# sec-bit/ckb-zkp

Hardware: AMD Instinct MI355X
Metric: Groth16 proofs/sec (2^20 constraints, BN256) (higher is better)
Workload: dtype u32 limbs (256-bit Montgomery integers); 1 GPU; Groth16 prove, MiMC-chain R1CS, 1048570 constraints (domain 2^20), 1258284 aux, bn254, G1 x4 + G2 x1 MSM + 4 NTT (7 in the reference: evaluation-form key); curve=bn254, log_domain=20, parallelism=independent proofs x1

## Files before the change

### ckb_zkp_amd/_lib.py

```python
from __future__ import annotations

import ctypes as C
import os
from pathlib import Path

LIB_PATH = Path(os.environ.get("ZKP_ACCEL_LIB") or Path(__file__).resolve().parent / "lib" / "libzkp_accel.so")

u64p = C.POINTER(C.c_uint64)
u32p = C.POINTER(C.c_uint32)
u8p = C.POINTER(C.c_uint8)
vp = C.c_void_p


class ZkpError(RuntimeError):
    def __init__(self, status: int, where: str, text: str):
        super().__init__(f"{where}: status {status} ({text})")
        self.status = status


class Csr(C.Structure):
    _fields_ = [("row_ptr", vp), ("col", vp), ("coeff", vp)]


class Groth16PkDesc(C.Structure):
# ... 106 lines not shown
    "zkp_bases_upload_g2": (C.c_int32, [vp, C.c_int, vp, vp, C.c_size_t, C.POINTER(C.c_uint64)]),
    "zkp_bases_share": (C.c_int32, [vp, vp, C.c_uint64, u64p]),
    "zkp_bases_free": (C.c_int32, [vp, C.c_uint64]),
    "zkp_bases_len": (C.c_int32, [vp, C.c_uint64, C.POINTER(C.c_size_t)]),
    "zkp_msm_g1": (C.c_int32, [vp, C.c_uint64, C.c_size_t, vp, C.c_size_t, vp]),
    "zkp_msm_g2": (C.c_int32, [vp, C.c_uint64, C.c_size_t, vp, C.c_size_t, vp]),
    "zkp_msm_g1_dev": (C.c_int32, [vp, C.c_uint64, C.c_size_t, vp, C.c_size_t, vp]),
    "zkp_msm_g2_dev": (C.c_int32, [vp, C.c_uint64, C.c_size_t, vp, C.c_size_t, vp]),
    "zkp_vartime_multiscalar_mul_g1": (C.c_int32, [vp, C.c_uint64, vp, C.c_size_t, vp]),
    "zkp_vartime_multiscalar_mul_g2": (C.c_int32, [vp, C.c_uint64, vp, C.c_size_t, vp]),
    "zkp_msm_g1_var": (C.c_int32, [vp, C.c_int, vp, vp, vp, C.c_size_t, C.c_int32, vp]),
    "zkp_msm_g2_var": (C.c_int32, [vp, C.c_int, vp, vp, vp, C.c_size_t, C.c_int32, vp]),
    "zkp_msm_g1_var_batch_dev": (C.c_int32, [vp, C.c_int, C.c_size_t, vp, vp, vp, vp, C.c_int32, vp]),
    "zkp_msm_g2_var_batch_dev": (C.c_int32, [vp, C.c_int, C.c_size_t, vp, vp, vp, vp, C.c_int32, vp]),
    "zkp_g1_ipa_fold_dev": (C.c_int32, [vp, C.c_int, vp, vp, vp, vp, C.c_size_t, vp, vp, vp, vp]),
    "zkp_fr_dot_batch_dev": (C.c_int32, [vp, C.c_int, C.c_size_t, vp, vp, vp, vp]),
    "zkp_msm_g1_mont_dev": (C.c_int32, [vp, C.c_uint64, C.c_size_t, vp, C.c_size_t, vp]),
    "zkp_msm_g2_mont_dev": (C.c_int32, [vp, C.c_uint64, C.c_size_t, vp, C.c_size_t, vp]),
    "zkp_msm_g1_mont_batch_dev": (C.c_int32, [vp, C.c_uint64, C.c_size_t, vp, vp, vp, vp]),
    "zkp_msm_mont_multi_dev": (C.c_int32, [vp, C.c_size_t, vp, vp, vp, vp, vp, C.c_size_t]),
    "zkp_fr_vec_op_dev": (C.c_int32, [vp, C.c_int, C.c_int32, vp, vp, vp, vp, C.c_size_t]),
    "zkp_fr_spmv_dev": (C.c_int32, [vp, C.c_int, vp, vp, vp, C.c_size_t, vp, vp]),
    "zkp_fr_gather_dev": (C.c_int32, [vp, vp, vp, C.c_size_t, vp]),
    "zkp_poly_divide_by_vanishing_dev": (C.c_int32, [vp, C.c_int, vp, C.c_size_t, C.c_size_t, vp, vp]),
    "zkp_d2d": (C.c_int32, [vp, vp, vp, C.c_size_t]),
    "zkp_dev_zero": (C.c_int32, [vp, vp, C.c_size_t]),
    "zkp_fr_batch_inverse_dev": (C.c_int32, [vp, C.c_int, vp, C.c_size_t]),
    "zkp_poly_evaluate_dev": (C.c_int32, [vp, C.c_int, vp, C.c_size_t, vp, vp]),
    "zkp_poly_div_linear_dev": (C.c_int32, [vp, C.c_int, vp, C.c_size_t, vp, vp, vp]),
    "zkp_g1_fold": (C.c_int32, [vp, C.c_int, vp, C.c_size_t, vp]),
    "zkp_g2_fold": (C.c_int32, [vp, C.c_int, vp, C.c_size_t, vp]),
    "zkp_g1_into_affine": (C.c_int32, [vp, C.c_int, vp, vp, vp]),
    "zkp_g1_decompress": (C.c_int32, [vp, C.c_int, vp, C.c_size_t, vp, vp, C.POINTER(C.c_size_t)]),
    "zkp_g2_decompress": (C.c_int32, [vp, C.c_int, vp, C.c_size_t, vp, vp, C.POINTER(C.c_size_t)]),
    "zkp_g1_compress": (C.c_int32, [vp, C.c_int, vp, vp, C.c_size_t, vp]),
    "zkp_g2_compress": (C.c_int32, [vp, C.c_int, vp, vp, C.c_size_t, vp]),
    "zkp_g1_subgroup_check": (C.c_int32, [vp, C.c_int, vp, vp, C.c_size_t, C.POINTER(C.c_size_t)]),
    "zkp_g2_subgroup_check": (C.c_int32, [vp, C.c_int, vp, vp, C.c_size_t, C.POINTER(C.c_size_t)]),
    "zkp_g2_into_affine": (C.c_int32, [vp, C.c_int, vp, vp, vp]),
    "zkp_groth16_points_into_affine": (C.c_int32, [C.c_int, vp, vp, vp, vp, vp]),
    "zkp_fixed_base_mul_g1": (C.c_int32, [vp, C.c_int, vp, vp, C.c_size_t, vp, vp]),
    "zkp_fixed_base_mul_g2": (C.c_int32, [vp, C.c_int, vp, vp, C.c_size_t, vp, vp]),
    "zkp_groth16_pk_upload": (C.c_int32, [vp, C.POINTER(Groth16PkDesc), C.POINTER(vp)]),
    "zkp_groth16_pk_upload_ex": (C.c_int32, [vp, C.POINTER(Groth16PkDesc), C.c_uint32, C.POINTER(vp)]),
    "zkp_groth16_pk_upload_shard": (C.c_int32, [vp, C.POINTER(Groth16PkDesc), C.c_int32, C.c_int32, C.POINTER(vp)]),
    "zkp_groth16_partials_bytes": (C.c_int32, [C.c_int, C.POINTER(C.c_size_t)]),
    "zkp_groth16_prove_partials_dev": (C.c_int32, [vp, vp, vp, vp, vp, vp]),
    "zkp_groth16_fold_assemble_dev": (C.c_int32, [vp, C.c_int, vp, C.c_int32, vp, vp, vp, vp]),
    "zkp_groth16_pk_free": (C.c_int32, [vp, vp]),
    "zkp_groth16_witness_map": (C.c_int32, [vp, vp, vp, vp]),
    "zkp_groth16_witness_map_dev": (C.c_int32, [vp, vp, vp, vp]),
    "zkp_groth16_domain_size": (C.c_int32, [vp, C.POINTER(C.c_uint64)]),
    "zkp_groth16_pk_info": (C.c_int32, [vp, vp, C.POINTER(C.c_uint64)]),
    "zkp_groth16_prove": (C.c_int32, [vp, vp, vp, vp, vp, vp, vp]),
    "zkp_groth16_prove_dev": (C.c_int32, [vp, vp, vp, vp, vp, vp, vp]),
    "zkp_groth16_prove_batch_dev": (C.c_int32, [vp, vp, C.c_size_t, vp, vp, vp, vp, vp]),
    "zkp_groth16_prove_batch": (C.c_int32, [vp, vp, C.c_size_t, vp, vp, vp, vp, vp]),
    "zkp_groth16_assemble": (C.c_int32, [vp, C.c_int, vp, vp, vp, vp, vp]),
    "zkp_groth16_last_timing": (C.c_int32, [vp, C.POINTER(Groth16Timing)]),
    "zkp_marlin_last_timing": (C.c_int32, [vp, C.POINTER(MarlinTiming)]),
    "zkp_set_profiling": (C.c_int32, [vp, C.c_int32]),
    "zkp_marlin_index_upload": (C.c_int32, [vp, C.POINTER(MarlinIndexDesc), C.POINTER(vp)]),
    "zkp_marlin_index_free": (C.c_int32, [vp, vp]),
    "zkp_marlin_index_info": (C.c_int32, [vp, u64p]),
    "zkp_marlin_index_commit": (C.c_int32, [vp, vp, C.c_uint64, vp, vp]),
    "zkp_marlin_prove": (C.c_int32, [vp, vp, C.c_uint64, C.c_uint64, vp, C.c_size_t, vp, vp, C.c_size_t,
                                     C.POINTER(MarlinRand), vp, C.POINTER(MarlinProof)]),
    "zkp_fs_rng_new": (C.c_int32, [vp, C.c_size_t, C.POINTER(vp)]),
    "zkp_fs_rng_free": (C.c_int32, [vp]),
    "zkp_fs_rng_absorb": (C.c_int32, [vp, vp, C.c_size_t]),
    "zkp_fs_rng_seed": (C.c_int32, [vp, vp]),
    "zkp_fs_rng_next_u64": (C.c_int32, [vp, u64p]),
    "zkp_fs_rng_rand_u128": (C.c_int32, [vp, vp]),
    "zkp_fs_rng_rand_fr": (C.c_int32, [vp, C.c_int, vp]),
    "zkp_fs_rng_sample_outside_domain": (C.c_int32, [vp, C.c_int, C.c_uint32, vp]),
    "zkp_merlin_oneshot": (C.c_int32, [vp, C.c_size_t, vp, C.c_size_t, vp, C.c_size_t, vp, C.c_size_t, vp, C.c_size_t]),
    "zkp_bench_mulmod": (C.c_int32, [vp, C.c_int, C.c_int32, C.c_int32, C.POINTER(C.c_double)]),
    "zkp_bench_hbm_copy": (C.c_int32, [vp, C.c_size_t, C.POINTER(C.c_double)]),
}

_lib = None


def load(path: os.PathLike | None = None) -> C.CDLL:
    global _lib
    if _lib is not None and path is None:
        return _lib
    p = Path(path) if path else LIB_PATH
    if not p.exists():
        raise ImportError(f"{p} not found — build it with `python -m ckb_zkp_amd.build` "
                          "(hipcc --offload-arch=gfx950); there is no CPU fallback")
    lib = C.CDLL(str(p))
    for name, (res, args) in SIGNATURES.items():
        fn = getattr(lib, name)
        fn.restype, fn.argtypes = res, args
    if path is None:
        _lib = lib
    return lib


ZKP_ERR_INVALID_POINT = -7


def check(status: int, where: str) -> None:
    if status != 0:
        raise ZkpError(status, where, load().zkp_status_string(status).decode())
# ... 1 lines not shown
```

### ckb_zkp_amd/csrc/capi.hip

```cpp
#include <cstdint>
#include <cstdlib>
#include <cstring>

#include "ctx.hpp"
#include "host_field.hpp"
#include "internal.hpp"
#include "ipa.hpp"

using namespace zkp;

namespace {

template <class Fn>
int32_t guarded(zkp_ctx* ctx, Fn&& fn) {
  if (!ctx) return ZKP_ERR_BAD_ARG;
  std::lock_guard<std::recursive_mutex> lk(ctx->mu);
  try {
    ZKP_HIP(hipSetDevice(ctx->device));
    fn();
    return ZKP_OK;
  } catch (const StatusError& e) {
    return e.status;
  } catch (const HipError& e) {
    ctx->last_error = std::string(e.what) + ": " + hipGetErrorString(e.e);
// ... 568 lines not shown
  if (!desc || !out || (flags & ~(uint32_t)ZKP_PK_KEEP_FORM)) return ZKP_ERR_BAD_ARG;
  return guarded(ctx, [&] { *out = groth16_pk_upload(ctx, desc, 0, 0, (int)flags); });
}
int32_t zkp_groth16_pk_upload_shard(zkp_ctx* ctx, const zkp_groth16_pk_desc* desc, int32_t rank, int32_t world,
                                    zkp_groth16_pk** out) {
  if (!desc || !out || world < 1 || rank < 0 || rank >= world) return ZKP_ERR_BAD_ARG;
  return guarded(ctx, [&] { *out = groth16_pk_upload(ctx, desc, rank, world); });
}
int32_t zkp_groth16_partials_bytes(zkp_curve_t curve, size_t* bytes) {
  if (!bytes || (curve != ZKP_BN254 && curve != ZKP_BLS12_381)) return ZKP_ERR_BAD_ARG;
  *bytes = groth16_partials_bytes(curve);
  return ZKP_OK;
}
int32_t zkp_groth16_prove_partials_dev(zkp_ctx* ctx, zkp_groth16_pk* pk, const uint64_t* z_dev, const uint64_t* r,
                                       const uint64_t* s, void* partials_dev) {
  if (!pk || !z_dev || !r || !s || !partials_dev) return ZKP_ERR_BAD_ARG;
  return guarded(ctx, [&] { groth16_prove_partials(ctx, pk, z_dev, r, s, partials_dev); });
}
int32_t zkp_groth16_fold_assemble_dev(zkp_ctx* ctx, zkp_curve_t curve, const void* gathered_dev, int32_t world,
                                      const uint64_t* r, const uint64_t* s, uint64_t* proof, uint8_t* inf) {
  if (!gathered_dev || world < 1 || !r || !s || !proof || !inf) return ZKP_ERR_BAD_ARG;
  return guarded(ctx, [&] { groth16_fold_assemble(ctx, curve, gathered_dev, world, r, s, proof, inf); });
}
int32_t zkp_groth16_pk_upload_multi(zkp_ctx* ctx, const zkp_groth16_pk_desc* desc, int32_t mode, zkp_groth16_pk_multi** out) {
  if (!ctx || !desc || !out || ctx->devs.empty() || (mode != ZKP_MULTI_SHARD && mode != ZKP_MULTI_REPLICATE)) return ZKP_ERR_BAD_ARG;
  return guarded_multi(ctx, [&] { *out = groth16_pk_upload_multi(ctx, desc, mode); });
}
int32_t zkp_groth16_pk_multi_free(zkp_ctx* ctx, zkp_groth16_pk_multi* pk) {
  if (!ctx || !pk || ctx->devs.empty()) return ZKP_ERR_BAD_ARG;
  return guarded_multi(ctx, [&] { groth16_pk_multi_free(ctx, pk); });
}
int32_t zkp_groth16_multi_info(zkp_ctx* ctx, zkp_groth16_pk_multi* pk, uint64_t info[6]) {
  if (!ctx || !pk || !info || ctx->devs.empty()) return ZKP_ERR_BAD_ARG;
  return guarded(ctx, [&] { groth16_multi_info(ctx, pk, info); });
}
int32_t zkp_groth16_prove_multi(zkp_ctx* ctx, zkp_groth16_pk_multi* pk, const uint64_t* const* z, int32_t z_on_device,
                                const uint64_t* r, const uint64_t* s, uint64_t* proof, uint8_t* inf) {
  if (!ctx || !pk || !z || !z[0] || !r || !s || !proof || !inf || ctx->devs.empty()) return ZKP_ERR_BAD_ARG;
  if (z_on_device)
    for (size_t k = 0; k < ctx->devs.size(); k++)
      if (!z[k]) return ZKP_ERR_BAD_ARG;
  return guarded_multi(ctx, [&] { groth16_prove_multi(ctx, pk, z, z_on_device != 0, r, s, proof, inf); });
}
int32_t zkp_groth16_prove_batch_multi(zkp_ctx* ctx, zkp_groth16_pk_multi* pk, size_t count, const uint64_t* const* z,
                                      int32_t z_on_device, const uint64_t* r, const uint64_t* s, uint64_t* proofs,
                                      uint8_t* inf) {
  if (!ctx || !pk || ctx->devs.empty() || (count && (!z || !r || !s || !proofs || !inf))) return ZKP_ERR_BAD_ARG;
  return guarded_multi(ctx, [&] { groth16_prove_batch_multi(ctx, pk, count, z, z_on_device != 0, r, s, proofs, inf); });
}
int32_t zkp_groth16_pk_free(zkp_ctx* ctx, zkp_groth16_pk* pk) {
  if (!pk) return ZKP_ERR_BAD_ARG;
  return guarded(ctx, [&] { groth16_pk_free(ctx, pk); });
}
int32_t zkp_groth16_pk_info(zkp_ctx* ctx, zkp_groth16_pk* pk, uint64_t info[8]) {
  if (!ctx || !pk || !info) return ZKP_ERR_BAD_ARG;
  return guarded(ctx, [&] { groth16_pk_info(ctx, pk, info); });
}
int32_t zkp_groth16_domain_size(zkp_groth16_pk* pk, uint64_t* n) {
  if (!pk || !n) return ZKP_ERR_BAD_ARG;
  *n = groth16_domain_size(pk);
  return ZKP_OK;
}
int32_t zkp_groth16_witness_map(zkp_ctx* ctx, zkp_groth16_pk* pk, const uint64_t* z, uint64_t* h) {
  if (!pk || !z || !h) return ZKP_ERR_BAD_ARG;
  return guarded(ctx, [&] { groth16_witness_map(ctx, pk, z, h, false); });
}
int32_t zkp_groth16_witness_map_dev(zkp_ctx* ctx, zkp_groth16_pk* pk, const uint64_t* z, uint64_t* h) {
  if (!pk || !z || !h) return ZKP_ERR_BAD_ARG;
  return guarded(ctx, [&] { groth16_witness_map(ctx, pk, z, h, true); });
}
int32_t zkp_groth16_prove(zkp_ctx* ctx, zkp_groth16_pk* pk, const uint64_t* z, const uint64_t* r, const uint64_t* s,
                          uint64_t* proof, uint8_t* inf) {
  if (!pk || !z || !r || !s || !proof || !inf) return ZKP_ERR_BAD_ARG;
  return guarded(ctx, [&] { groth16_prove(ctx, pk, z, false, r, s, proof, inf); });
}
int32_t zkp_groth16_prove_dev(zkp_ctx* ctx, zkp_groth16_pk* pk, const uint64_t* z, const uint64_t* r,
                              const uint64_t* s, uint64_t* proof, uint8_t* inf) {
  if (!pk || !z || !r || !s || !proof || !inf) return ZKP_ERR_BAD_ARG;
  return guarded(ctx, [&] { groth16_prove(ctx, pk, z, true, r, s, proof, inf); });
}
int32_t zkp_groth16_prove_batch_dev(zkp_ctx* ctx, zkp_groth16_pk* pk, size_t n, const uint64_t* const* z_dev,
                                    const uint64_t* r, const uint64_t* s, uint64_t* proofs, uint8_t* inf) {
  if (!pk || (n && (!z_dev || !r || !s || !proofs || !inf))) return ZKP_ERR_BAD_ARG;
  return guarded(ctx, [&] { groth16_prove_batch(ctx, pk, n, z_dev, r, s, proofs, inf); });
}
int32_t zkp_groth16_prove_batch(zkp_ctx* ctx, zkp_groth16_pk* pk, size_t n, const uint64_t* const* z_host,
                                const uint64_t* r, const uint64_t* s, uint64_t* proofs, uint8_t* inf) {
  if (!pk || (n && (!z_host || !r || !s || !proofs || !inf))) return ZKP_ERR_BAD_ARG;
  return guarded(ctx, [&] { groth16_prove_batch(ctx, pk, n, z_host, r, s, proofs, inf, false); });
}
int32_t zkp_groth16_assemble(zkp_ctx* ctx, zkp_curve_t curve, const uint64_t* sums, const uint64_t* r,
                             const uint64_t* s, uint64_t* proof, uint8_t* inf) {
  if (!sums || !r || !s || !proof || !inf) return ZKP_ERR_BAD_ARG;
  return guarded(ctx, [&] { groth16_assemble(ctx, curve, sums, r, s, proof, inf); });
}
int32_t zkp_marlin_index_upload(zkp_ctx* ctx, const zkp_marlin_index_desc* desc, zkp_marlin_index** out) {
  if (!desc || !out) return ZKP_ERR_BAD_ARG;
  return guarded(ctx, [&] { *out = marlin_index_upload(ctx, desc); });
}
int32_t zkp_marlin_index_free(zkp_ctx* ctx, zkp_marlin_index* index) {
  if (!index) return ZKP_ERR_BAD_ARG;
  return guarded(ctx, [&] { marlin_index_free(ctx, index); });
}
int32_t zkp_marlin_index_info(const zkp_marlin_index* index, uint64_t info[6]) {
  if (!index || !info) return ZKP_ERR_BAD_ARG;
  marlin_index_info(index, info);
// ... 37 lines not shown
```

### ckb_zkp_amd/csrc/ctx.hpp

```cpp
#pragma once
#include <hip/hip_runtime.h>
#include <stdint.h>

#include <map>
#include <mutex>
#include <memory>
#include <string>
#include <unordered_map>
#include <vector>

#include "../../include/zkp_accel.h"

namespace zkp {

struct HipError {
  hipError_t e;
  const char* what;
  int line;
};

#define ZKP_HIP(call)                                                   \
  do {                                                                  \
    hipError_t _e = (call);                                             \
    if (_e != hipSuccess) throw ::zkp::HipError{_e, #call, __LINE__};   \
  } while (0)

struct StatusError {
  int32_t status;
};
#define ZKP_REQUIRE(cond, status) \
  do {                            \
    if (!(cond)) throw ::zkp::StatusError{(status)}; \
  } while (0)

struct DevBuf {
  void* p = nullptr;
  size_t cap = 0;
  void* get(size_t bytes) {
    if (bytes > cap) {
      if (p) (void)hipFree(p);
      p = nullptr;
      cap = 0;
      size_t want = bytes + (bytes >> 3) + 256;
      hipError_t e = hipMalloc(&p, want);
      if (e != hipSuccess) throw StatusError{ZKP_ERR_OOM};
      cap = want;
    }
    return p;
  }
  template <class T>
  T* as(size_t count) { return reinterpret_cast<T*>(get(count * sizeof(T))); }
  ~DevBuf() {
    if (p) (void)hipFree(p);
  }
  DevBuf() = default;
  DevBuf(const DevBuf&) = delete;
  DevBuf& operator=(const DevBuf&) = delete;
};

struct NttTables {
  int log_n = 0, h = 0;
  uint32_t* w_lo = nullptr;
  uint32_t* w_hi = nullptr;
  uint32_t* wi_lo = nullptr;
  uint32_t* wi_hi = nullptr;
  uint32_t* g_lo = nullptr;
  uint32_t* g_hi = nullptr;
  uint32_t* gi_lo = nullptr;
  uint32_t* gi_hi = nullptr;
  uint32_t* sub_fwd = nullptr;
  uint32_t* sub_inv = nullptr;
  uint32_t* n_inv = nullptr;
  void* block = nullptr;
  uint32_t* full_fwd[8] = {};
  uint32_t* full_inv[8] = {};
  uint32_t* full_g = nullptr;
  uint32_t* full_gi = nullptr;
  uint32_t* g_hi_n = nullptr;
  uint32_t* full_g_n = nullptr;
  std::vector<void*> extra;
};

struct BasesEntry;

struct MsmWorkspace {
  hipStream_t stream = nullptr;
  bool own_stream = false;
  hipEvent_t done = nullptr;
  hipEvent_t sorted = nullptr;
  hipEvent_t l1_done = nullptr;
  uint32_t chain_nb = 0;
  size_t chain_xb = 0;
  hipEvent_t acc_done = nullptr;
  DevBuf keys, vals, keys2, vals2, sort_tmp, offsets, buckets, tmp, out, sched, scan_tmp, scan_tmp2, partial, redo;
};
struct Groth16Timing {
  zkp_groth16_timing t{};
};

}

struct zkp_lane {
  hipStream_t stream = nullptr;
  bool own_stream = true;
  static constexpr int N_WS = 4;
  static constexpr int N_WS_MSM = N_WS;
  zkp::MsmWorkspace ws[N_WS];
  zkp::DevBuf ntt_scratch;
  hipEvent_t ev_fork = nullptr, ev_a = nullptr, ev_b1 = nullptr;
  uint32_t* host_proof = nullptr;
  bool host_tail = false;
  bool busy = false;
};

struct zkp_cfg {
  int lanes = 0;
  int msm_batch_lanes = 1;
  int msm_c = 0, msm_c_g2 = 0;
  long long msm_chunk = (long long)3 << 19;
  double table_budget_gb = 0;
  bool h_lagrange = true, c_fold = true, host_affine = true;
  long long lfold_heavy_cost = 0;
  int multi_exchange = 0;
  int multi_exchange_timeout_ms = 30000;
  int multi_wm_split = -1;
};

struct zkp_ctx {
  int device = 0;
  zkp_cfg cfg;
  std::recursive_mutex mu;
  static constexpr int N_LANES = 8;
  static constexpr int N_WS = zkp_lane::N_WS;
  zkp_lane lanes[N_LANES];
  zkp_lane* cur = &lanes[0];
  int cur_idx = 0;
  hipEvent_t ev0 = nullptr, ev1 = nullptr;
  hipEvent_t ev2 = nullptr, ev3 = nullptr;
  bool profiling = false;
  size_t table_bytes = 0;
  bool msm_defer_reduce = false;
  int msm_acc_into = -1;
  int msm_bucket_ws = -1;
  bool dbg_skip_k8 = false;
  bool batch_mode = false;
  std::map<std::pair<int, int>, zkp::NttTables> ntt_tables;
  zkp::DevBuf ntt_io, poly_tmp, poly_consts, spmv_list;
  zkp::DevBuf msm_scalars, msm_misc, var_bases;
  uint32_t* pinned = nullptr;
  size_t pinned_cap = 0;
  std::unordered_map<uint64_t, std::shared_ptr<zkp::BasesEntry>> bases;
  uint64_t next_handle = 1;
  zkp_groth16_timing last_timing{};
  zkp_marlin_timing last_marlin_timing{};
  std::string last_error;
  std::vector<zkp_ctx*> devs;
  std::map<std::pair<int, int>, std::shared_ptr<void>> var_plans;
  bool tl_on = false;
  std::string tl_tag;
  std::vector<std::pair<std::string, hipEvent_t>> tl;
  void mark(hipStream_t st, const char* what) {
// ... 8 lines not shown
```

### ckb_zkp_amd/csrc/groth16.hip

```cpp
#include <algorithm>
#include <cstdlib>
#include <cstring>
#include <memory>
#include <string>
#include <vector>

#include "field_dev.hpp"
#include "host_field.hpp"
#include "internal.hpp"
#include "msm_vtbl.hpp"

using namespace zkp;

struct DevCsr {
  uint32_t* row_ptr = nullptr;
  uint32_t* col = nullptr;
  uint32_t* coeff = nullptr;
  size_t nnz = 0;
};

struct zkp_groth16_pk {
  int curve = 0;
  uint32_t num_inputs = 0, num_aux = 0, num_constraints = 0;
  int log_n = 0;
  size_t N = 0, nz = 0;
  DevCsr m[3];
  uint64_t hA = 0, hB1 = 0, hB2 = 0, hH = 0, hL = 0;
  bool share_b_sort = false;
  bool chain_lh = false;
  bool share_al_sort = false;
  bool share_l1 = false;
  bool b_in_l1 = false;
  bool c_folded = false;
  bool h_lagrange = false;
  int shard_rank = 0, shard_world = 0;
  size_t q_lo[5] = {0, 0, 0, 0, 0}, q_n[5] = {0, 0, 0, 0, 0};
  struct PerLane {
    DevBuf abc;
    DevBuf S;
    DevBuf results;
    DevBuf proof;
    bool warmed = false;
    int graph_state = 0;
    hipGraphExec_t graph_exec = nullptr;
    hipGraph_t graph = nullptr;
    std::vector<const void*> sig;
  } lane[zkp_ctx::N_LANES];
  DevBuf consts;
};

namespace zkp {

template <class P>
__global__ __launch_bounds__(256) void csr_eval_kernel(const uint32_t* __restrict__ row_ptr,
                                                       const uint32_t* __restrict__ col,
                                                       const uint32_t* __restrict__ coeff,
                                                       const uint32_t* __restrict__ z, uint32_t nc, uint32_t N,
                                                       uint32_t num_inputs, int is_a, uint32_t* __restrict__ out) {
  using F = Fp<P>;
  uint32_t i = blockIdx.x * blockDim.x + threadIdx.x;
  if (i >= N) return;
  F acc = F::zero();
  if (i < nc) {
    const F one = F::one();
    for (uint32_t k = row_ptr[i]; k < row_ptr[i + 1]; k++) {
      F v = F::load(z + (size_t)col[k] * 8);
      F cf = F::load(coeff + (size_t)k * 8);
      if (cf == one) acc = acc + v;
      else acc = acc + v * cf;
    }
  } else if (is_a && i - nc < num_inputs) {
    acc = F::load(z + (size_t)(i - nc) * 8);
  }
  acc.store(out + (size_t)i * 8);
}

template <class P>
__global__ __launch_bounds__(256) void qap_pointwise_kernel(uint32_t* __restrict__ a, const uint32_t* __restrict__ b,
                                                            const uint32_t* __restrict__ c,
                                                            const uint32_t* __restrict__ zinv, uint32_t N) {
  using F = Fp<P>;
  uint32_t i = blockIdx.x * blockDim.x + threadIdx.x;
  if (i >= N) return;
  F x = F::load(a + (size_t)i * 8) * F::load(b + (size_t)i * 8) - F::load(c + (size_t)i * 8);
  (x * F::load(zinv)).store(a + (size_t)i * 8);
}

template <class P>
__global__ __launch_bounds__(256) void qap_pointwise_ab_kernel(uint32_t* __restrict__ a, const uint32_t* __restrict__ b,
                                                               const uint32_t* __restrict__ zinv, uint32_t N) {
  using F = Fp<P>;
  uint32_t i = blockIdx.x * blockDim.x + threadIdx.x;
  if (i >= N) return;
  (F::load(a + (size_t)i * 8) * F::load(b + (size_t)i * 8) * F::load(zinv)).store(a + (size_t)i * 8);
}

template <class P>
__global__ __launch_bounds__(256) void pow_canon_kernel(uint32_t* __restrict__ out, const uint32_t* __restrict__ base,
                                                        const uint32_t* __restrict__ mult, uint32_t count) {
  using F = Fp<P>;
  const uint32_t i = blockIdx.x * blockDim.x + threadIdx.x;
// ... 240 lines not shown
  char* o = (char*)b_o.get(nz * ab);
  uint8_t* oi = (uint8_t*)b_oi.get(nz);
  v1->lfold(st, dl, dli, nz, dcp, drows, dkind, dcoeff, dg, dgi, o, oi);
  ZKP_HIP(hipGetLastError());
  l_xy->resize(nz * 2 * fq);
  l_inf->resize(nz);
  ZKP_HIP(hipMemcpyAsync(l_xy->data(), o, nz * ab, hipMemcpyDeviceToHost, st));
  ZKP_HIP(hipMemcpyAsync(l_inf->data(), oi, nz, hipMemcpyDeviceToHost, st));
  ZKP_HIP(hipStreamSynchronize(st));
  if (!heavy_cols.empty()) {
    const HostField Q = fq_field(d->curve);
    const size_t fw = 2 * fq;
    std::vector<HostJac> res(heavy_cols.size());
    std::vector<uint64_t> xyz(3 * fq);
    std::vector<uint64_t> cxy, csc;
    std::vector<uint8_t> cinf;
    for (size_t i = 0; i < heavy_cols.size(); i++) {
      const uint32_t m = heavy_cols[i];
      const size_t cn = hv[i].size();
      cxy.resize(cn * fw);
      csc.resize(cn * 4);
      cinf.resize(cn);
      for (size_t j = 0; j < cn; j++) {
        const uint32_t k = hv[i][j].first, e = hv[i][j].second;
        memcpy(&cxy[j * fw], &g_xy[(size_t)k * fw], 8 * fw);
        cinf[j] = g_inf[k];
        memcpy(&csc[j * 4], d->ct.coeff + (size_t)e * 4, 32);
      }
      std::vector<std::pair<uint32_t, uint32_t>>().swap(hv[i]);
      msm_var_run(ctx, d->curve, 1, cxy.data(), cinf.data(), csc.data(), cn, true, xyz.data());
      HostJac D = host_jac_load(Q, xyz.data());
      D.y = Q.neg(D.y);
      HostJac Lm{};
      if ((*l_inf)[m]) {
        Lm.x = Q.one_();
        Lm.y = Q.one_();
      } else {
        memcpy(Lm.x.data(), l_xy->data() + (size_t)m * fw, 8 * fq);
        memcpy(Lm.y.data(), l_xy->data() + (size_t)m * fw + fq, 8 * fq);
        Lm.z = Q.one_();
      }
      res[i] = host_jac_add(Q, Lm, D);
    }
    std::vector<uint64_t> axy(heavy_cols.size() * fw);
    std::vector<uint8_t> ainf(heavy_cols.size());
    host_into_affine(Q, res, axy.data(), fw, ainf.data());
    for (size_t i = 0; i < heavy_cols.size(); i++) {
      memcpy(l_xy->data() + (size_t)heavy_cols[i] * fw, axy.data() + i * fw, 8 * fw);
      (*l_inf)[heavy_cols[i]] = ainf[i];
    }
  }
}

zkp_groth16_pk* groth16_pk_upload(zkp_ctx* ctx, const zkp_groth16_pk_desc* d, int rank, int world, int flags) {
  ZKP_REQUIRE(d->curve == ZKP_BN254 || d->curve == ZKP_BLS12_381, ZKP_ERR_UNSUPPORTED_CURVE);
  ZKP_REQUIRE(d->num_inputs >= 1, ZKP_ERR_BAD_ARG);
  ZKP_REQUIRE(world >= 0 && (world == 0 ? rank == 0 : (rank >= 0 && rank < world)), ZKP_ERR_BAD_ARG);
  std::unique_ptr<zkp_groth16_pk> pk(new zkp_groth16_pk());
  pk->shard_rank = rank;
  pk->shard_world = world;
  pk->curve = d->curve;
  pk->num_inputs = d->num_inputs;
  pk->num_aux = d->num_aux;
  pk->num_constraints = d->num_constraints;
  pk->nz = (size_t)d->num_inputs + d->num_aux;
  size_t dom = (size_t)d->num_constraints + d->num_inputs;
  int lg = 0;
  while (((size_t)1 << lg) < dom) lg++;
  ZKP_REQUIRE(lg <= (d->curve == ZKP_BN254 ? 28 : 32) && lg <= 30, ZKP_ERR_DOMAIN_TOO_LARGE);
  pk->log_n = lg;
  pk->N = (size_t)1 << lg;
  const bool matrices_only = d->a_query == nullptr;
  if (!matrices_only) {
    ZKP_REQUIRE(d->a_len == pk->nz && d->b_g1_len == pk->nz && d->b_g2_len == pk->nz, ZKP_ERR_BAD_ARG);
    ZKP_REQUIRE(d->l_len == d->num_aux, ZKP_ERR_BAD_ARG);
  }
  const size_t fq = d->curve == ZKP_BN254 ? 4 : 6;
  const uint64_t* tA[4] = {d->alpha_g1, d->delta_g1, nullptr, nullptr};
  const uint64_t* tB1[4] = {d->beta_g1, nullptr, d->delta_g1, nullptr};
  const uint64_t* tB2[4] = {d->beta_g2, nullptr, d->delta_g2, nullptr};
  const uint64_t* tL[4] = {nullptr, nullptr, nullptr, d->delta_g1};
  pk->m[0] = upload_csr(ctx, d->at, d->num_constraints);
  pk->m[1] = upload_csr(ctx, d->bt, d->num_constraints);
  pk->m[2] = upload_csr(ctx, d->ct, d->num_constraints);
  ZKP_REQUIRE(!(matrices_only && world > 0), ZKP_ERR_BAD_ARG);
  if (!matrices_only) {
    for (auto p : {d->alpha_g1, d->beta_g1, d->delta_g1, d->beta_g2, d->delta_g2}) ZKP_REQUIRE(p, ZKP_ERR_BAD_ARG);
    const size_t h_used = std::min<size_t>(d->h_len, pk->N);
    shard_bounds(pk->nz + 4, rank, world, &pk->q_lo[0], &pk->q_n[0]);
    pk->q_lo[1] = pk->q_lo[2] = pk->q_lo[0];
    pk->q_n[1] = pk->q_n[2] = pk->q_n[0];
    shard_bounds(h_used, rank, world, &pk->q_lo[3], &pk->q_n[3]);
    pk->q_lo[4] = pk->q_lo[0];
    pk->q_n[4] = pk->q_n[0];
    const bool lagrange_on = ctx->cfg.h_lagrange && !(flags & 1) && d->h_query && h_used > 0 && pk->log_n >= 1;
    int lgk = 0;
    {
      const int groups[5] = {1, 1, 2, 1, 1};
      size_t hq_lo = 0, hq_n = pk->q_n[3];
      if (lagrange_on) shard_bounds(pk->N, rank, world, &hq_lo, &hq_n);
      const size_t ns[5] = {pk->q_n[0], pk->q_n[1], pk->q_n[2], lagrange_on ? hq_n : (world > 0 ? pk->q_n[3] : (size_t)d->h_len), pk->q_n[4]};
      lgk = bases_plan_lgk(ctx, d->curve, groups, ns, 5);
      if (lgk > 0 && getenv("ZKP_DEBUG_MSM")) fprintf(stderr, "[groth16] window tables do not fit: window groups of %d\n", 1 << lgk);
    }
    std::vector<uint8_t> fA, fB1, fB2, fL;
    pk->hA = upload_ext(ctx, d->curve, 1, d->a_query, d->a_inf, d->a_len, 2 * fq, tA, pk->q_lo[0], pk->q_n[0], 0, &fA, 0, 0, lgk);
// ... 50 lines not shown
      }
      fold_c_into_l(ctx, d, pk->nz, gc.xy, gc.inf, &lxy, &linf);
      if (!lagrange_keep_cache) gc.clear();
      pk->hL = upload_ext(ctx, d->curve, 1, lxy.data(), linf.data(), pk->nz, 2 * fq, tL, pk->q_lo[4], pk->q_n[4], 0, &fL, 0, 0, lgk);
      pk->c_folded = true;
    } else
    pk->hL = upload_ext(ctx, d->curve, 1, d->l_query, d->l_inf, d->l_len, 2 * fq, tL, pk->q_lo[4], pk->q_n[4],
                        d->num_inputs, &fL, 0, 0, lgk);
    {
      static const bool on = !(getenv("ZKP_SHARE_AL_SORT") && atoi(getenv("ZKP_SHARE_AL_SORT")) == 0);
      bool same = fA.size() == fL.size() && pk->q_lo[0] == pk->q_lo[4];
      size_t differ = 0;
      std::vector<uint8_t> both(fA.size());
      for (size_t k = 0; same && k < fA.size(); k++) {
        both[k] = fA[k] & fL[k];
        differ += fA[k] != fL[k];
      }
      pk->share_al_sort = on && same && differ <= fA.size() / 16 && bases_same_shape(ctx, pk->hL, pk->hA) && pk->q_n[0] > 0;
      if (pk->share_al_sort && differ) bases_set_sort_flags(ctx, pk->hA, both.data(), both.size());
      static const bool on_l1 = !(getenv("ZKP_SHARE_L1") && atoi(getenv("ZKP_SHARE_L1")) == 0);
      const bool aligned = fA.size() == fL.size() && fA.size() == fB2.size() && pk->q_lo[0] == pk->q_lo[4] &&
                           pk->q_lo[0] == pk->q_lo[2] && pk->q_n[0] > 0;
      if (on_l1 && aligned && !pk->share_al_sort && bases_same_shape(ctx, pk->hL, pk->hA)) {
        const bool with_b = pk->share_b_sort && bases_same_shape(ctx, pk->hB1, pk->hA);
        std::vector<uint8_t> all(fA.size()), member(fA.size());
        for (size_t k = 0; k < fA.size(); k++) {
          all[k] = fA[k] & fL[k] & (with_b ? fB2[k] : (uint8_t)1);
          member[k] = all[k] ? 0 : (uint8_t)((fA[k] ? 1 : 0) | (with_b && fB2[k] ? 2 : 0) | (fL[k] ? 4 : 0));
        }
        bases_set_sort_flags(ctx, pk->hA, all.data(), all.size());
        bases_set_group(ctx, pk->hA, member.data(), member.size());
        bases_set_filter_bit(ctx, pk->hA, 0);
        if (with_b) bases_set_filter_bit(ctx, pk->hB2, 1);
        bases_set_filter_bit(ctx, pk->hL, 2);
        pk->share_l1 = true;
        pk->b_in_l1 = with_b;
      }
      {
        static const bool on_chain = !(getenv("ZKP_CHAIN_LH") && atoi(getenv("ZKP_CHAIN_LH")) == 0);
        uint64_t iL[5], iH[5];
        bases_info(ctx, pk->hL, iL);
        bases_info(ctx, pk->hH, iH);
        pk->chain_lh = on_chain && iL[0] == iH[0] && iL[2] == 1 && iH[2] == 1 && pk->q_n[3] > 0 && pk->q_n[4] > 0;
      }
      if (getenv("ZKP_DEBUG_MSM"))
        fprintf(stderr, "[groth16] A/L sort sharing: %d (flags differ at %zu of %zu bases), B1/B2: %d, shared level 1: %d\n",
                (int)pk->share_al_sort, differ, fA.size(), (int)pk->share_b_sort, (int)pk->share_l1);
    }
  }
  uint32_t* consts = pk->consts.as<uint32_t>(64);
  if (d->curve == ZKP_BN254) hipLaunchKernelGGL(qap_consts_kernel<Bn254Fr>, dim3(1), dim3(64), 0, ctx->cur->stream, consts, lg);
  else hipLaunchKernelGGL(qap_consts_kernel<Bls381Fr>, dim3(1), dim3(64), 0, ctx->cur->stream, consts, lg);
  ZKP_HIP(hipGetLastError());
  for (int l = 0; l < 2; l++) {
    auto& L = pk->lane[l];
    L.abc.get(3 * pk->N * 32);
    L.S.get((pk->nz + 4) * 32);
    L.results.get(6 * 16 * 24 * 4 + 64);
    L.proof.get(4096);
  }
  ZKP_HIP(hipStreamSynchronize(ctx->cur->stream));
  return pk.release();
}

void groth16_pk_free(zkp_ctx* ctx, zkp_groth16_pk* pk) {
  (void)hipDeviceSynchronize();
  for (auto& PL : pk->lane) {
    if (PL.graph_exec) (void)hipGraphExecDestroy(PL.graph_exec);
    if (PL.graph) (void)hipGraphDestroy(PL.graph);
  }
  for (uint64_t h : {pk->hA, pk->hB1, pk->hB2, pk->hH, pk->hL})
    if (h) bases_drop(ctx, h);
  for (auto& m : pk->m) {
    if (m.row_ptr) (void)hipFree(m.row_ptr);
    if (m.col) (void)hipFree(m.col);
    if (m.coeff) (void)hipFree(m.coeff);
  }
  delete pk;
}

uint64_t groth16_domain_size(zkp_groth16_pk* pk) { return pk->N; }
void groth16_pk_info(zkp_ctx* ctx, zkp_groth16_pk* pk, uint64_t info[8]) {
  for (int i = 0; i < 8; i++) info[i] = 0;
  if (!pk->hA) return;
  uint64_t a[5], b[5];
  bases_info(ctx, pk->hA, a);
  bases_info(ctx, pk->hB2, b);
  info[0] = a[2];
  for (uint64_t h : {pk->hA, pk->hB1, pk->hB2, pk->hH, pk->hL}) {
    uint64_t t[5];
    bases_info(ctx, h, t);
    info[1] += t[4];
  }
  info[2] = a[0];
  info[3] = a[1];
  info[4] = a[3];
  info[5] = b[0];
  info[6] = (pk->share_b_sort ? 1 : 0) | (pk->share_al_sort ? 2 : 0) | (pk->share_l1 ? 4 : 0);
  info[7] = (pk->h_lagrange ? 1 : 0) | (pk->c_folded ? 2 : 0) | (pk->chain_lh ? 4 : 0);
}

template <class P>
static uint32_t* witness_map_dev(zkp_ctx* ctx, zkp_groth16_pk* pk, const uint32_t* z_dev, bool coeffs = true) {
  const uint32_t N = (uint32_t)pk->N;
  uint32_t* a = pk->lane[ctx->cur_idx].abc.as<uint32_t>(3 * pk->N * 8);
  uint32_t* b = a + pk->N * 8;
  uint32_t* c = b + pk->N * 8;
  uint32_t* bufs[3] = {a, b, c};
  hipStream_t st = ctx->cur->stream;
  const int nchain = (!coeffs && pk->c_folded) ? 2 : 3;
  for (int k = 0; k < nchain; k++)
    hipLaunchKernelGGL(csr_eval_kernel<P>, dim3((N + 255) / 256), dim3(256), 0, st, pk->m[k].row_ptr, pk->m[k].col,
                       pk->m[k].coeff, z_dev, pk->num_constraints, N, pk->num_inputs, k == 0 ? 1 : 0, bufs[k]);
  static const bool batch = getenv("ZKP_NTT_BATCH") && atoi(getenv("ZKP_NTT_BATCH")) != 0;
  if (batch) {
    ntt_run_batch(ctx, pk->curve, bufs, nchain, pk->log_n, ZKP_NTT_IFFT);
    ntt_run_batch(ctx, pk->curve, bufs, nchain, pk->log_n, ZKP_NTT_COSET_FFT);
  } else {
    for (int k = 0; k < nchain; k++) {
// ... 175 lines not shown
  }
  tm.ms_msm_accumulate = acc_ms;
  tm.msm_points = ent;
  tm.ms_msm_scan = scan_ms;
  tm.msm_scan_bytes = scan_bytes;
  tm.msm_scan_launches = scan_runs;
  if (partial_out) {
    ZKP_HIP(hipMemcpyAsync(partial_out, res, 5 * slot, hipMemcpyDeviceToDevice, st));
    ZKP_HIP(hipGetLastError());
    if (prof) {
      ZKP_HIP(hipEventRecord(eT1, st));
      ZKP_HIP(hipStreamSynchronize(st));
      ZKP_HIP(hipEventElapsedTime(&tm.ms_total, eT0, eT1));
      ctx->last_timing = tm;
    }
    return;
  }

  tic();
  if (!fan) v1->assemble_g1_part1(st, res, slot, rs, host_tail ? nullptr : proof_dev, flags_dev);
  v1->assemble_g1_part2(st, res, slot, host_tail ? nullptr : proof_dev, flags_dev, 2 * v1->fN + 2 * v2->fN);
  if (!g2_done_in_fan && !host_tail) v2->assemble_g2(st, res, slot, proof_dev, flags_dev, 2 * v1->fN);
  ZKP_HIP(hipGetLastError());
  toc(&tm.ms_assemble);
  const size_t proof_words = 4 * (size_t)v1->fN + 2 * (size_t)v2->fN;
  if (host_tail) {
    uint32_t* hp = ctx->cur->host_proof;
    ZKP_HIP(hipMemcpyAsync(hp, res, 16 * (size_t)v1->fN, hipMemcpyDeviceToHost, st));
    ZKP_HIP(hipMemcpyAsync(hp + 4 * v1->fN, res + 2 * slot, 16 * (size_t)v2->fN, hipMemcpyDeviceToHost, st));
    ZKP_HIP(hipMemcpyAsync(hp + 4 * v1->fN + 4 * v2->fN, res + 5 * slot, 16 * (size_t)v1->fN, hipMemcpyDeviceToHost, st));
  } else {
    ZKP_HIP(hipMemcpyAsync(ctx->cur->host_proof, proof_dev, proof_words * 4, hipMemcpyDeviceToHost, st));
    ZKP_HIP(hipMemcpyAsync(ctx->cur->host_proof + 256, flags_dev, 12, hipMemcpyDeviceToHost, st));
  }
  ctx->tl_tag.clear();
  ctx->mark(st, "copied");
  ctx->cur->host_tail = host_tail;
  ctx->cur->busy = true;
  if (prof) {
    ZKP_HIP(hipEventRecord(eT1, st));
    ZKP_HIP(hipStreamSynchronize(st));
    ZKP_HIP(hipEventElapsedTime(&tm.ms_total, eT0, eT1));
    ctx->last_timing = tm;
  }
}

static std::vector<const void*> lane_signature(zkp_ctx* ctx, zkp_groth16_pk* pk) {
  std::vector<const void*> sig;
  zkp_lane* L = ctx->cur;
  zkp_groth16_pk::PerLane& PL = pk->lane[ctx->cur_idx];
  for (DevBuf* b : {&PL.abc, &PL.S, &PL.results, &PL.proof, &L->ntt_scratch}) sig.push_back(b->p);
  for (int w = 0; w < zkp_lane::N_WS; w++) {
    MsmWorkspace& ws = L->ws[w];
    for (DevBuf* b : {&ws.keys, &ws.vals, &ws.keys2, &ws.vals2, &ws.sort_tmp, &ws.offsets, &ws.buckets, &ws.tmp, &ws.out,
                      &ws.sched, &ws.scan_tmp, &ws.scan_tmp2, &ws.partial, &ws.redo})
      sig.push_back(b->p);
  }
  sig.push_back(pk);
  return sig;
}

template <class FrP>
static void prove_enqueue(zkp_ctx* ctx, zkp_groth16_pk* pk, const uint64_t* z, bool z_on_device, const uint64_t* r,
                          const uint64_t* s, bool latency_plan = false) {
  static const bool graph_on = getenv("ZKP_GRAPH") && atoi(getenv("ZKP_GRAPH")) != 0;
  static const bool single_stream = getenv("ZKP_SINGLE_STREAM") && atoi(getenv("ZKP_SINGLE_STREAM")) != 0;
  if (!graph_on || ctx->profiling || single_stream) {
    prove_enqueue_part<FrP>(ctx, pk, z, z_on_device, r, s, 3, nullptr, latency_plan);
    return;
  }
  zkp_groth16_pk::PerLane& PL = pk->lane[ctx->cur_idx];
  hipStream_t st = ctx->cur->stream;
  if (PL.graph_state == 2 && PL.sig == lane_signature(ctx, pk)) {
    prove_enqueue_part<FrP>(ctx, pk, z, z_on_device, r, s, 1);
    ZKP_HIP(hipGraphLaunch(PL.graph_exec, st));
    ctx->cur->busy = true;
    return;
  }
  if (PL.graph_state == 2) {
    (void)hipGraphExecDestroy(PL.graph_exec);
    (void)hipGraphDestroy(PL.graph);
    PL.graph_exec = nullptr;
    PL.graph = nullptr;
    PL.graph_state = 0;
  }
  if (PL.graph_state == 1 && PL.sig == lane_signature(ctx, pk)) {
    prove_enqueue_part<FrP>(ctx, pk, z, z_on_device, r, s, 1);
    ZKP_HIP(hipStreamBeginCapture(st, hipStreamCaptureModeRelaxed));
    try {
      prove_enqueue_part<FrP>(ctx, pk, z, z_on_device, r, s, 2);
    } catch (...) {
      hipGraph_t g = nullptr;
      (void)hipStreamEndCapture(st, &g);
      if (g) (void)hipGraphDestroy(g);
      throw;
    }
    ZKP_HIP(hipStreamEndCapture(st, &PL.graph));
    ZKP_HIP(hipGraphInstantiate(&PL.graph_exec, PL.graph, nullptr, nullptr, 0));
    PL.graph_state = 2;
    ZKP_HIP(hipGraphLaunch(PL.graph_exec, st));
    ctx->cur->busy = true;
    return;
  }
  prove_enqueue_part<FrP>(ctx, pk, z, z_on_device, r, s, 3);
  PL.sig = lane_signature(ctx, pk);
  PL.graph_state = 1;
}

static void prove_finish(zkp_ctx* ctx, zkp_groth16_pk* pk, uint64_t* proof_out, uint8_t* inf_out) {
  const MsmVtbl* v1 = msm_vtbl(pk->curve, 1);
  const MsmVtbl* v2 = msm_vtbl(pk->curve, 2);
  const size_t proof_words = 4 * (size_t)v1->fN + 2 * (size_t)v2->fN;
  ZKP_HIP(hipStreamSynchronize(ctx->cur->stream));
  if (!ctx->tl.empty()) {
    std::string line = "[zkp timeline ms]";
    for (auto& m : ctx->tl) {
      float ms = 0.f;
      (void)hipEventSynchronize(m.second);
      (void)hipEventElapsedTime(&ms, ctx->tl[0].second, m.second);
// ... 60 lines not shown
  else prove_enqueue_part<Bls381Fr>(ctx, pk, z_dev, true, r, s, 3, (char*)out_dev, true);
  ZKP_HIP(hipStreamSynchronize(ctx->cur->stream));
}

void groth16_fold_assemble(zkp_ctx* ctx, int curve, const void* gathered_dev, int world, const uint64_t* r,
                           const uint64_t* s, uint64_t* proof_out, uint8_t* inf_out) {
  ZKP_REQUIRE(world >= 1, ZKP_ERR_BAD_ARG);
  const MsmVtbl* v1 = msm_vtbl(curve, 1);
  const MsmVtbl* v2 = msm_vtbl(curve, 2);
  hipStream_t st = ctx->cur->stream;
  const size_t slot = v2->xyzz_bytes;
  uint32_t* buf = ctx->msm_misc.as<uint32_t>(16 + 6 * slot / 4 + 256 + 16);
  uint32_t* rs = buf;
  char* res = reinterpret_cast<char*>(rs + 16);
  uint32_t* proof_dev = reinterpret_cast<uint32_t*>(res + 6 * slot);
  uint32_t* flags_dev = proof_dev + 240;
  ZKP_HIP(hipMemcpyAsync(rs, r, 32, hipMemcpyHostToDevice, st));
  ZKP_HIP(hipMemcpyAsync(rs + 8, s, 32, hipMemcpyHostToDevice, st));
  v1->fold_slots(st, (const char*)gathered_dev, 5 * slot, world, slot, 0x1b, res);
  v2->fold_slots(st, (const char*)gathered_dev, 5 * slot, world, slot, 0x04, res);
  v1->assemble_g1_part1(st, res, slot, rs, proof_dev, flags_dev);
  v1->assemble_g1_part2(st, res, slot, proof_dev, flags_dev, 2 * v1->fN + 2 * v2->fN);
  v2->assemble_g2(st, res, slot, proof_dev, flags_dev, 2 * v1->fN);
  ZKP_HIP(hipGetLastError());
  const size_t proof_words = 4 * (size_t)v1->fN + 2 * (size_t)v2->fN;
  uint32_t flags_host[4] = {0, 0, 0, 0};
  ZKP_HIP(hipMemcpyAsync(proof_out, proof_dev, proof_words * 4, hipMemcpyDeviceToHost, st));
  ZKP_HIP(hipMemcpyAsync(flags_host, flags_dev, 12, hipMemcpyDeviceToHost, st));
  ZKP_HIP(hipStreamSynchronize(st));
  for (int i = 0; i < 3; i++) inf_out[i] = (uint8_t)flags_host[i];
}

void groth16_prove(zkp_ctx* ctx, zkp_groth16_pk* pk, const uint64_t* z, bool z_on_device, const uint64_t* r,
                   const uint64_t* s, uint64_t* proof_out, uint8_t* inf_out) {
  ZKP_REQUIRE(pk->shard_world == 0, ZKP_ERR_BAD_ARG);
  ctx->cur = &ctx->lanes[0];
  ctx->cur_idx = 0;
  static const bool timeline = getenv("ZKP_TIMELINE") && atoi(getenv("ZKP_TIMELINE")) != 0;
  ctx->tl_on = timeline && !ctx->profiling;
  if (pk->curve == ZKP_BN254) prove_enqueue<Bn254Fr>(ctx, pk, z, z_on_device, r, s, true);
  else prove_enqueue<Bls381Fr>(ctx, pk, z, z_on_device, r, s, true);
  ctx->tl_on = false;
  prove_finish(ctx, pk, proof_out, inf_out);
}

void groth16_prove_batch(zkp_ctx* ctx, zkp_groth16_pk* pk, size_t n, const uint64_t* const* z_dev, const uint64_t* r,
                         const uint64_t* s, uint64_t* proofs_out, uint8_t* inf_out, bool z_on_device) {
  const MsmVtbl* v1 = msm_vtbl(pk->curve, 1);
  const MsmVtbl* v2 = msm_vtbl(pk->curve, 2);
  const size_t pw64 = (4 * (size_t)v1->fN + 2 * (size_t)v2->fN) / 2;
  const bool prof = ctx->profiling;
  ZKP_REQUIRE(pk->shard_world == 0, ZKP_ERR_BAD_ARG);
  size_t pending[zkp_ctx::N_LANES] = {};
  const int lanes_default = pk->log_n <= 22 ? 8 : 4;
  const int nl = std::max(1, std::min(ctx->cfg.lanes > 0 ? ctx->cfg.lanes : lanes_default, (int)zkp_ctx::N_LANES));
  auto select = [&](int l) {
    ctx->cur = &ctx->lanes[l];
    ctx->cur_idx = l;
  };
  struct BatchMode {
    zkp_ctx* c;
    ~BatchMode() { c->batch_mode = false; }
  } batch_mode{ctx};
  ctx->batch_mode = n > 1 && !prof;
  try {
    if (ctx->batch_mode) {
      std::vector<uint64_t> scratch_proof(pw64 + 8);
      uint8_t scratch_inf[4];
      bool any = false;
      for (int l = 0; l < nl; l++) {
        if (pk->lane[l].warmed) continue;
        select(l);
        if (pk->curve == ZKP_BN254) prove_enqueue<Bn254Fr>(ctx, pk, z_dev[0], z_on_device, r, s);
        else prove_enqueue<Bls381Fr>(ctx, pk, z_dev[0], z_on_device, r, s);
        pk->lane[l].warmed = true;
        any = true;
      }
      if (any)
        for (int l = 0; l < nl; l++) {
          select(l);
          if (ctx->cur->busy) prove_finish(ctx, pk, scratch_proof.data(), scratch_inf);
        }
    }
    for (size_t i = 0; i < n; i++) {
      const int l = prof ? 0 : (int)(i % nl);
      select(l);
      if (ctx->cur->busy) prove_finish(ctx, pk, proofs_out + pending[l] * pw64, inf_out + pending[l] * 3);
      if (pk->curve == ZKP_BN254) prove_enqueue<Bn254Fr>(ctx, pk, z_dev[i], z_on_device, r + 4 * i, s + 4 * i);
      else prove_enqueue<Bls381Fr>(ctx, pk, z_dev[i], z_on_device, r + 4 * i, s + 4 * i);
      pending[l] = i;
    }
    for (int l = 0; l < zkp_ctx::N_LANES; l++) {
      select(l);
      if (ctx->cur->busy) prove_finish(ctx, pk, proofs_out + pending[l] * pw64, inf_out + pending[l] * 3);
    }
  } catch (...) {
    (void)hipDeviceSynchronize();
    for (auto& L : ctx->lanes) L.busy = false;
    select(0);
    throw;
  }
  select(0);
}

}
#include <dlfcn.h>

#include <chrono>
#include <condition_variable>
#include <mutex>
#include <string>

#include <thread>
struct zkp_groth16_pk_multi {
  int mode = 0, curve = 0;
  std::vector<zkp_groth16_pk*> pk;
  std::vector<hipEvent_t> ev_chain, ev_done, ev_h_read;
  hipEvent_t ev_h = nullptr;
  void* gathered = nullptr;
  std::vector<void*> gathered_all;
  std::vector<void*> partial;
  int exchange = 0;
  bool exchange_fallback = false;
  int rccl_ranks = 0;
  int split_choice = -1;
  int calls = 0;
  double ms_variant[2] = {0.0, 0.0};
};
namespace zkp {

namespace {
struct RcclApi {
  struct Fns {
    void* lib = nullptr;
    int (*CommInitAll)(void**, int, const int*) = nullptr;
    int (*CommDestroy)(void*) = nullptr;
// ... 463 lines not shown
```

### ckb_zkp_amd/csrc/internal.hpp

```cpp
#pragma once
#include "ctx.hpp"

namespace zkp {

void ntt_run(zkp_ctx* ctx, int curve, uint32_t* data_dev, int log_n, int op);
void ntt_run_batch(zkp_ctx* ctx, int curve, uint32_t* const* data_dev, int count, int log_n, int op);
bool ntt_ifft_coset_fft(zkp_ctx* ctx, int curve, uint32_t* data, int log_n);
uint32_t* ntt_qap_coset_ifft(zkp_ctx* ctx, int curve, uint32_t* a, uint32_t* b, uint32_t* c, const uint32_t* zinv, int log_n);
void ntt_free_tables(zkp_ctx* ctx);

void fr_vec_op(zkp_ctx* ctx, int curve, int op, const uint64_t* a, const uint64_t* b, const uint64_t* k_host,
               uint64_t* out, size_t n);
void fr_batch_inverse(zkp_ctx* ctx, int curve, uint64_t* v, size_t n);
void fr_dot_batch(zkp_ctx* ctx, int curve, size_t count, const uint64_t* const* a, const uint64_t* const* b, const size_t* ns,
                  uint64_t* out_host);
void fr_spmv(zkp_ctx* ctx, int curve, const uint32_t* row_ptr, const uint32_t* col, const uint64_t* coeff, size_t nrows,
             const uint64_t* x, uint64_t* out);
void fr_gather(zkp_ctx* ctx, const uint64_t* in, const int32_t* idx, size_t n, uint64_t* out);
void poly_vanishing_fold(zkp_ctx* ctx, int curve, const uint64_t* p, size_t len, size_t n, uint64_t* q, uint64_t* rem);
void poly_div_linear(zkp_ctx* ctx, int curve, const uint64_t* p, size_t n, const uint64_t* z_host, uint64_t* q,
                     uint64_t* eval_out_host);
void marlin_round2_prod(zkp_ctx* ctx, int curve, const uint64_t* ra, const uint64_t* za, const uint64_t* zb, const uint64_t* t,
                        const uint64_t* z, const uint64_t* k_host, uint64_t* out, size_t n);
void marlin_t3_evals(zkp_ctx* ctx, int curve, const uint64_t* const* on_k, const uint64_t* k_host, uint64_t* out, size_t n);
void marlin_h2_numerator(zkp_ctx* ctx, int curve, const uint64_t* const* on_b, const uint64_t* t, const uint64_t* k_host, uint64_t* out,
                         size_t n);
void poly_evaluate_batch(zkp_ctx* ctx, int curve, size_t count, const uint64_t* const* p, const size_t* n, const uint64_t* z_host,
                         uint64_t* out_host);

uint64_t bases_upload(zkp_ctx* ctx, int curve, int group, const uint64_t* xy_host, const uint8_t* inf_host, size_t n,
                      int c_hint = 0, int cap_hint = 0, int lgk_hint = -1);
size_t bases_table_bytes(zkp_ctx* ctx, int curve, int group, size_t n, int lgk);
int bases_plan_lgk(zkp_ctx* ctx, int curve, const int* groups, const size_t* ns, int count);
void bases_free(zkp_ctx* ctx, uint64_t handle);
uint64_t bases_share(zkp_ctx* dst, zkp_ctx* src, uint64_t handle);
size_t bases_len(zkp_ctx* ctx, uint64_t handle);
int bases_group(zkp_ctx* ctx, uint64_t handle);
void msm_run(zkp_ctx* ctx, uint64_t handle, size_t offset, const uint64_t* scalars_dev, size_t n, bool montgomery,
             uint64_t* out_xyz_host, void* out_dev_xyzz = nullptr, float* ms_accumulate = nullptr,
             uint64_t* n_entries = nullptr, int ws = 0, int sort_src = -1, float* ms_scan = nullptr, int l1_src = -1);
double bench_mulmod(zkp_ctx* ctx, int curve, int field, bool unsaturated);
double bench_hbm_copy(zkp_ctx* ctx, size_t bytes);
bool bases_same_shape(zkp_ctx* ctx, uint64_t h1, uint64_t h2);
void bases_set_sort_flags(zkp_ctx* ctx, uint64_t handle, const uint8_t* flags_host, size_t n);
void bases_set_group(zkp_ctx* ctx, uint64_t owner, const uint8_t* member_flags_host, size_t n);
void bases_set_filter_bit(zkp_ctx* ctx, uint64_t handle, int bit);
void msm_run_batch(zkp_ctx* ctx, uint64_t handle, size_t count, const size_t* offsets, const uint64_t* const* scalars_dev,
                   const size_t* ns, bool montgomery, uint64_t* out_xyz_host);
void msm_run_multi(zkp_ctx* ctx, size_t count, const uint64_t* handles, const size_t* offsets,
                   const uint64_t* const* scalars_dev, const size_t* ns, bool montgomery, uint64_t* out_xyz_host,
                   size_t slot_words);
void msm_var_run(zkp_ctx* ctx, int curve, int group, const uint64_t* xy_host, const uint8_t* inf_host,
                 const uint64_t* scalars_host, size_t n, bool montgomery, uint64_t* out_xyz_host);
void msm_var_batch_run(zkp_ctx* ctx, int curve, int group, size_t count, const uint64_t* const* xy_dev,
                       const uint8_t* const* inf_dev, const uint64_t* const* scalars_dev, const size_t* ns, bool montgomery,
                       uint64_t* out_xyz_host);
void msm_free_all(zkp_ctx* ctx);
void bases_drop(zkp_ctx* ctx, uint64_t handle);
void point_fold(zkp_ctx* ctx, int curve, int group, const uint64_t* xyz_host, size_t k, uint64_t* out_xyz_host);
void point_into_affine(zkp_ctx* ctx, int curve, int group, const uint64_t* xyz_host, uint64_t* xy_out, uint8_t* inf_out);
size_t points_decompress(zkp_ctx* ctx, int curve, int group, const uint8_t* bytes, size_t n, uint64_t* xy_out, uint8_t* inf_out);
void points_compress(zkp_ctx* ctx, int curve, int group, const uint64_t* xy, const uint8_t* inf, size_t n, uint8_t* bytes_out);
size_t points_subgroup_check(zkp_ctx* ctx, int curve, int group, const uint64_t* xy, const uint8_t* inf, size_t n);
void points_fold_into_affine(zkp_ctx* ctx, int curve, int group, const uint64_t* a_xyz_host, const uint64_t* b_xyz_host,
                             const uint8_t* has_b, size_t k, uint64_t* xy_out, uint8_t* inf_out);
void fixed_base_mul(zkp_ctx* ctx, int curve, int group, const uint64_t* base_xy, const uint64_t* scalars_host, size_t n,
                    uint64_t* out_xy, uint8_t* out_inf);

zkp_groth16_pk* groth16_pk_upload(zkp_ctx* ctx, const zkp_groth16_pk_desc* d, int rank = 0, int world = 0, int flags = 0);
size_t groth16_partials_bytes(int curve);
void groth16_prove_partials(zkp_ctx* ctx, zkp_groth16_pk* pk, const uint64_t* z_dev, const uint64_t* r, const uint64_t* s,
                            void* out_dev);
void groth16_fold_assemble(zkp_ctx* ctx, int curve, const void* gathered_dev, int world, const uint64_t* r,
                           const uint64_t* s, uint64_t* proof_out, uint8_t* inf_out);
void groth16_pk_free(zkp_ctx* ctx, zkp_groth16_pk* pk);
uint64_t groth16_domain_size(zkp_groth16_pk* pk);
void groth16_pk_info(zkp_ctx* ctx, zkp_groth16_pk* pk, uint64_t info[8]);
void bases_info(zkp_ctx* ctx, uint64_t handle, uint64_t info[5]);
void groth16_witness_map(zkp_ctx* ctx, zkp_groth16_pk* pk, const uint64_t* z, uint64_t* h, bool on_device);
void groth16_prove(zkp_ctx* ctx, zkp_groth16_pk* pk, const uint64_t* z, bool z_on_device, const uint64_t* r,
                   const uint64_t* s, uint64_t* proof_out, uint8_t* inf_out);

void groth16_prove_batch(zkp_ctx* ctx, zkp_groth16_pk* pk, size_t n, const uint64_t* const* z_dev, const uint64_t* r,
                         const uint64_t* s, uint64_t* proofs_out, uint8_t* inf_out, bool z_on_device = true);
void groth16_assemble(zkp_ctx* ctx, int curve, const uint64_t* sums_xyz, const uint64_t* r, const uint64_t* s,
                      uint64_t* proof_out, uint8_t* inf_out);

zkp_groth16_pk_multi* groth16_pk_upload_multi(zkp_ctx* root, const zkp_groth16_pk_desc* d, int mode);
void groth16_pk_multi_free(zkp_ctx* root, zkp_groth16_pk_multi* pk);
void groth16_multi_info(zkp_ctx* root, zkp_groth16_pk_multi* pk, uint64_t info[6]);
void groth16_prove_multi(zkp_ctx* root, zkp_groth16_pk_multi* pk, const uint64_t* const* z, bool z_on_device, const uint64_t* r,
                         const uint64_t* s, uint64_t* proof_out, uint8_t* inf_out);
void groth16_prove_batch_multi(zkp_ctx* root, zkp_groth16_pk_multi* pk, size_t n, const uint64_t* const* z, bool z_on_device,
                               const uint64_t* r, const uint64_t* s, uint64_t* proofs_out, uint8_t* inf_out);

zkp_marlin_index* marlin_index_upload(zkp_ctx* ctx, const zkp_marlin_index_desc* d);
void marlin_index_free(zkp_ctx* ctx, zkp_marlin_index* ix);
void marlin_index_commit(zkp_ctx* ctx, zkp_marlin_index* ix, uint64_t powers_g, uint64_t* comms_xy, uint8_t* inf);
void marlin_index_info(const zkp_marlin_index* ix, uint64_t info[6]);
void marlin_prove(zkp_ctx* ctx, zkp_marlin_index* ix, uint64_t powers_g, uint64_t powers_gamma_g, const uint8_t* ivk_bytes,
                  size_t ivk_len, const uint64_t* x_mont, const uint64_t* w_mont, size_t n_w, const zkp_marlin_rand* rnd,
                  const uint64_t* fixed_challenges, zkp_marlin_proof* out);

}
```

### ckb_zkp_amd/csrc/msm.hip

```cpp
#include <algorithm>
#include <cstdlib>
#include <cstring>
#include <map>
#include <type_traits>
#include <memory>
#include <mutex>
#include <vector>

#include "field_dev.hpp"
#include "internal.hpp"
#include "msm_digits.hpp"
#include "msm_small.hpp"
#include "msm_vtbl.hpp"

namespace zkp {

#if defined(ZKP_NO_SORT_PRIO)
#define ZKP_SORT_PRIO() do { } while (0)
#else
#define ZKP_SORT_PRIO() __builtin_amdgcn_s_setprio(3)
#endif

const MsmVtbl* msm_vtbl_c01();
const MsmVtbl* msm_vtbl_c02();
// ... 166 lines not shown
  info[2] = (uint64_t)1 << e->lgk;
  info[3] = e->lgk ? (uint64_t)((e->W + (1 << e->lgk) - 1) >> e->lgk) : (uint64_t)e->W;
  info[4] = e->table_bytes;
}
void bases_drop(zkp_ctx* ctx, uint64_t handle) {
  auto it = ctx->bases.find(handle);
  if (it == ctx->bases.end()) return;
  if (it->second.use_count() == 1) ctx->table_bytes -= std::min(ctx->table_bytes, it->second->table_bytes);
  ctx->bases.erase(it);
}
void msm_free_all(zkp_ctx* ctx) {
  ctx->bases.clear();
  ctx->table_bytes = 0;
  ctx->var_plans.clear();
}
uint64_t bases_share(zkp_ctx* dst, zkp_ctx* src, uint64_t handle) {
  auto e = get_bases(src, handle);
  ZKP_REQUIRE(dst->device == src->device, ZKP_ERR_BAD_ARG);
  uint64_t h = dst->next_handle++;
  dst->bases[h] = e;
  return h;
}
void bases_set_sort_flags(zkp_ctx* ctx, uint64_t handle, const uint8_t* flags_host, size_t n) {
  auto e = get_bases(ctx, handle);
  ZKP_REQUIRE(n == e->n, ZKP_ERR_BAD_ARG);
  if (e->sort_inf) (void)hipFree(e->sort_inf);
  e->sort_inf = nullptr;
  if (!flags_host || n == 0) return;
  if (hipMalloc(&e->sort_inf, n) != hipSuccess) throw StatusError{ZKP_ERR_OOM};
  ZKP_HIP(hipMemcpyAsync(e->sort_inf, flags_host, n, hipMemcpyHostToDevice, ctx->cur->stream));
  ZKP_HIP(hipStreamSynchronize(ctx->cur->stream));
}
void bases_set_group(zkp_ctx* ctx, uint64_t owner, const uint8_t* member_flags_host, size_t n) {
  auto e = get_bases(ctx, owner);
  ZKP_REQUIRE(n == e->n, ZKP_ERR_BAD_ARG);
  if (e->group_flags) (void)hipFree(e->group_flags);
  e->group_flags = nullptr;
  if (!member_flags_host || n == 0) return;
  if (hipMalloc(&e->group_flags, n) != hipSuccess) throw StatusError{ZKP_ERR_OOM};
  ZKP_HIP(hipMemcpyAsync(e->group_flags, member_flags_host, n, hipMemcpyHostToDevice, ctx->cur->stream));
  ZKP_HIP(hipStreamSynchronize(ctx->cur->stream));
}
void bases_set_filter_bit(zkp_ctx* ctx, uint64_t handle, int bit) {
  ZKP_REQUIRE(bit >= -1 && bit < 3, ZKP_ERR_BAD_ARG);
  get_bases(ctx, handle)->filter_bit = bit;
}
bool bases_same_shape(zkp_ctx* ctx, uint64_t h1, uint64_t h2) {
  auto a = get_bases(ctx, h1), b = get_bases(ctx, h2);
  return a->curve == b->curve && a->n == b->n && a->c == b->c && a->W == b->W && a->wide == b->wide && a->cap == b->cap && a->lgk == b->lgk;
}


constexpr int SCAN_CHUNK = 2048;
__global__ __launch_bounds__(256) void scan_reduce_kernel(const uint32_t* __restrict__ in, size_t n,
                                                          uint32_t* __restrict__ sums) {
  ZKP_SORT_PRIO();
  __shared__ uint32_t red[256];
  size_t base = (size_t)blockIdx.x * SCAN_CHUNK;
  uint32_t acc = 0;
  for (int k = 0; k < SCAN_CHUNK / 256; k++) {
    size_t i = base + (size_t)k * 256 + threadIdx.x;
    if (i < n) acc += in[i];
  }
  red[threadIdx.x] = acc;
  __syncthreads();
  for (int s = 128; s > 0; s >>= 1) {
    if ((int)threadIdx.x < s) red[threadIdx.x] += red[threadIdx.x + s];
    __syncthreads();
  }
  if (threadIdx.x == 0) sums[blockIdx.x] = red[0];
}
__global__ __launch_bounds__(1024) void scan_sums_kernel(uint32_t* __restrict__ sums, size_t m) {
  ZKP_SORT_PRIO();
  __shared__ uint32_t buf[1024];
  uint32_t carry = 0;
  for (size_t t0 = 0; t0 < m; t0 += 1024) {
    size_t i = t0 + threadIdx.x;
    uint32_t v = i < m ? sums[i] : 0;
    buf[threadIdx.x] = v;
    __syncthreads();
    for (int d = 1; d < 1024; d <<= 1) {
      uint32_t add = (int)threadIdx.x >= d ? buf[threadIdx.x - d] : 0;
      __syncthreads();
      buf[threadIdx.x] += add;
      __syncthreads();
    }
    if (i < m) sums[i] = carry + buf[threadIdx.x] - v;
    uint32_t total = buf[1023];
    __syncthreads();
    carry += total;
  }
}
__global__ __launch_bounds__(256) void scan_apply_kernel(const uint32_t* __restrict__ in, size_t n,
                                                         const uint32_t* __restrict__ sums,
                                                         uint32_t* __restrict__ out) {
  ZKP_SORT_PRIO();
  __shared__ uint32_t part[256];
  size_t base = (size_t)blockIdx.x * SCAN_CHUNK;
  constexpr int PER = SCAN_CHUNK / 256;
  uint32_t v[PER];
  uint32_t acc = 0;
  for (int k = 0; k < PER; k++) {
    size_t i = base + (size_t)threadIdx.x * PER + k;
    v[k] = i < n ? in[i] : 0;
    acc += v[k];
  }
  part[threadIdx.x] = acc;
  __syncthreads();
  for (int d = 1; d < 256; d <<= 1) {
    uint32_t add = (int)threadIdx.x >= d ? part[threadIdx.x - d] : 0;
    __syncthreads();
    part[threadIdx.x] += add;
    __syncthreads();
  }
  uint32_t run = sums[blockIdx.x] + part[threadIdx.x] - acc;
  for (int k = 0; k < PER; k++) {
    size_t i = base + (size_t)threadIdx.x * PER + k;
    if (i < n) out[i] = run;
    run += v[k];
  }
}
static void exclusive_scan_u32(hipStream_t st, const uint32_t* in, uint32_t* out, size_t n, DevBuf& tmp) {
  if (n == 0) return;
  size_t chunks = (n + SCAN_CHUNK - 1) / SCAN_CHUNK;
  uint32_t* sums = tmp.as<uint32_t>(chunks + 1);
  hipLaunchKernelGGL(scan_reduce_kernel, dim3(chunks), dim3(256), 0, st, in, n, sums);
  hipLaunchKernelGGL(scan_sums_kernel, dim3(1), dim3(1024), 0, st, sums, chunks);
  hipLaunchKernelGGL(scan_apply_kernel, dim3(chunks), dim3(256), 0, st, in, n, sums, out);
}

constexpr int SORT_H1_MAX = 13;
constexpr uint32_t SORT_BIN_TARGET = 16384;
constexpr int SORT_L_MAX = 13;
constexpr int SORT_SCALARS = 2048;
constexpr int SORT_SCALARS_UNUSED_ = 0;
template <class FrP, int NT>
__global__ __launch_bounds__(NT) void sort_hist_kernel(const uint32_t* __restrict__ scalars, size_t n, size_t offset,
                                                        const uint8_t* __restrict__ inf, int montgomery, int c, int W, int wide,
                                                        uint32_t nb, int L, uint32_t nbins1,
                                                        uint32_t* __restrict__ hist, uint32_t nblocks, uint32_t tile,
                                                        int lgk) {
  ZKP_SORT_PRIO();
  const uint32_t gmask = (1u << lgk) - 1;
  __shared__ uint32_t cnt[(1 << SORT_H1_MAX) + 1];
  for (uint32_t i = threadIdx.x; i <= nbins1; i += NT) cnt[i] = 0;
  __syncthreads();
  for (uint32_t j = threadIdx.x; j < tile; j += NT) {
    size_t i = (size_t)blockIdx.x * tile + j;
    if (i < n && !(inf && inf[offset + i])) {
      DigitIter it = load_scalar<FrP>(scalars, i, montgomery);
      for (int w = 0; w < W; w++) {
        uint32_t key, neg;
        it.next(w, c, wide, nb, key, neg);
        if (key < nb) atomicAdd(&cnt[((((uint32_t)w & gmask) << (c - 1)) | key) >> L], 1u);
      }
    }
  }
  __syncthreads();
  for (uint32_t i = threadIdx.x; i < nbins1; i += NT) hist[(size_t)i * nblocks + blockIdx.x] = cnt[i];
}
template <class FrP>
__global__ __launch_bounds__(256) void sort_scatter_kernel(const uint32_t* __restrict__ scalars, size_t n,
                                                           size_t offset, const uint8_t* __restrict__ inf,
                                                           int montgomery, size_t ntab, int c, int W, int wide, uint32_t nb,
                                                           int L, uint32_t nbins1, const uint32_t* __restrict__ offs,
                                                           uint32_t nblocks, uint32_t tile,
                                                           uint64_t* __restrict__ kv, int lgk,
                                                           const uint8_t* __restrict__ group_flags) {
  ZKP_SORT_PRIO();
  const uint32_t gmask = (1u << lgk) - 1;
  __shared__ uint32_t cur[(1 << SORT_H1_MAX) + 1];
  for (uint32_t i = threadIdx.x; i < nbins1; i += 256) cur[i] = offs[(size_t)i * nblocks + blockIdx.x];
  __syncthreads();
  const uint32_t lmask = (1u << L) - 1;
  for (uint32_t rep = 0; rep < tile / 256; rep++) {
    size_t i = (size_t)blockIdx.x * tile + rep * 256 + threadIdx.x;
    if (i < n && !(inf && inf[offset + i])) {
      DigitIter it = load_scalar<FrP>(scalars, i, montgomery);
// ... 259 lines not shown
    if (hist[i]) atomicAdd(&tmeta[TM_HIST + i], hist[i]);
}

__global__ void task_cursor_kernel(uint32_t* tmeta) {
  ZKP_SORT_PRIO();
  if (threadIdx.x || blockIdx.x) return;
  uint32_t acc = 0;
  for (int l = MSM_TASK_CAP; l >= 0; l--) {
    tmeta[TM_CUR + l] = acc;
    acc += tmeta[TM_HIST + l];
  }
}

__global__ __launch_bounds__(1024) void task_order_kernel(const uint32_t* __restrict__ task_start,
                                                         const uint32_t* __restrict__ task_len,
                                                         const uint32_t* __restrict__ task_dst,
                                                         const uint32_t* __restrict__ n_tasks_dev,
                                                         uint32_t* __restrict__ tmeta, uint4* __restrict__ desc) {
  ZKP_SORT_PRIO();
  __shared__ uint32_t cnt[MSM_TASK_CAP + 1];
  __shared__ uint32_t base[MSM_TASK_CAP + 1];
  for (int i = threadIdx.x; i <= (int)MSM_TASK_CAP; i += blockDim.x) cnt[i] = 0;
  __syncthreads();
  uint32_t t = blockIdx.x * blockDim.x + threadIdx.x;
  const bool live = t < *n_tasks_dev;
  uint32_t l = 0, rank = 0;
  if (live) {
    l = task_len[t];
    rank = atomicAdd(&cnt[l], 1u);
  }
  __syncthreads();
  for (int i = threadIdx.x; i <= (int)MSM_TASK_CAP; i += blockDim.x)
    if (cnt[i]) base[i] = atomicAdd(&tmeta[TM_CUR + i], cnt[i]);
  __syncthreads();
  if (live) desc[base[l] + rank] = make_uint4(task_start[t], l, task_dst[t], t);
}

__global__ void sched_check_kernel(const uint32_t* toff, const uint32_t* long_list, const uint32_t* tmeta, uint32_t nb,
                                   uint32_t max_tasks, uint32_t* rep) {
  const uint32_t n_long = tmeta[TM_NLONG], n_tasks = toff[nb];
  for (uint32_t b = blockIdx.x * blockDim.x + threadIdx.x; b < nb; b += gridDim.x * blockDim.x) {
    if (toff[b + 1] < toff[b]) atomicAdd(&rep[0], 1u);
    atomicMax(&rep[1], toff[b + 1] - toff[b]);
  }
  for (uint32_t w = blockIdx.x * blockDim.x + threadIdx.x; w < n_long; w += gridDim.x * blockDim.x)
    if (long_list[w] >= nb) atomicAdd(&rep[2], 1u);
  if (blockIdx.x == 0 && threadIdx.x == 0) {
    rep[3] = n_long;
    rep[4] = n_tasks;
    rep[5] = n_tasks > max_tasks;
  }
}

static void msm_run_entry(zkp_ctx* ctx, const BasesEntry* be, size_t offset, const uint64_t* scalars_dev, size_t n,
                          bool montgomery, uint64_t* out_xyz_host, void* out_dev_xyzz, float* ms_accumulate,
                          uint64_t* n_entries, int ws_idx, int sort_src, float* ms_scan, int l1_src = -1);
void msm_run(zkp_ctx* ctx, uint64_t handle, size_t offset, const uint64_t* scalars_dev, size_t n, bool montgomery,
             uint64_t* out_xyz_host, void* out_dev_xyzz, float* ms_accumulate, uint64_t* n_entries, int ws_idx,
             int sort_src, float* ms_scan, int l1_src) {
  struct ChainReset {
    zkp_ctx* c;
    ~ChainReset() {
      c->msm_defer_reduce = false;
      c->msm_acc_into = -1;
    }
  } chain_reset{ctx};
  auto be = get_bases(ctx, handle);
  const size_t chunk_pts = (size_t)std::max<long long>(0, ctx->cfg.msm_chunk);
  const bool chunkable = chunk_pts >= 1024 && n >= 2 * chunk_pts && be->group == 1 && !be->var && sort_src < 0 && l1_src < 0 &&
                         !be->group_flags && !ctx->profiling && !ms_accumulate && !ms_scan && !n_entries &&
                         !ctx->msm_defer_reduce && ctx->msm_acc_into < 0 && ctx->msm_bucket_ws < 0 && !ctx->batch_mode;
  if (!chunkable) {
    msm_run_entry(ctx, be.get(), offset, scalars_dev, n, montgomery, out_xyz_host, out_dev_xyzz, ms_accumulate, n_entries,
                  ws_idx, sort_src, ms_scan, l1_src);
    return;
  }
  const size_t nch0 = (n + chunk_pts - 1) / chunk_pts, per = ((n + nch0 - 1) / nch0 + 255) & ~(size_t)255;
  static const size_t first_div = [] { const char* e = getenv("ZKP_MSM_CHUNK_FIRST"); long v = e ? atol(e) : 2; return (size_t)(v < 1 ? 1 : v); }();
  const size_t first = first_div > 1 ? std::max<size_t>(((per / first_div) + 255) & ~(size_t)255, 1024) : 0;
  const size_t rest = first && first < n ? n - first : n;
  const size_t nrest = (rest + per - 1) / per, per_rest = ((rest + nrest - 1) / nrest + 255) & ~(size_t)255;
  const size_t nch = (first && first < n ? 1 : 0) + (rest + per_rest - 1) / per_rest;
  const int wa = ws_idx, wb = ws_idx ^ 2;
  hipStream_t sa = wa == 0 ? ctx->cur->stream : ctx->cur->ws[wa].stream, sb = wb == 0 ? ctx->cur->stream : ctx->cur->ws[wb].stream;
  ZKP_HIP(hipEventRecord(ctx->cur->ws[wa].l1_done, sa));
  ZKP_HIP(hipStreamWaitEvent(sb, ctx->cur->ws[wa].l1_done, 0));
  size_t done = 0;
  for (size_t k = 0; k < nch; k++) {
    const size_t len = std::min((k == 0 && first && first < n) ? first : per_rest, n - done);
    const bool last = k + 1 == nch;
    const int w = ((nch - 1 - k) & 1) ? wb : wa;
    ctx->msm_defer_reduce = !last;
    ctx->msm_acc_into = k > 0 ? wa : -1;
    ctx->msm_bucket_ws = wa;
    msm_run_entry(ctx, be.get(), offset + done, scalars_dev + 4 * done, len, montgomery, last ? out_xyz_host : nullptr,
                  last ? out_dev_xyzz : nullptr, nullptr, nullptr, w, -1, nullptr, -1);
    done += len;
  }
}

struct VarPlan {
  DevBuf d1, d2;
  uint32_t n1 = 0, n2 = 0;
};
static VarPlan& var_plan(zkp_ctx* ctx, int c, int W, hipStream_t st) {
  auto key = std::make_pair(c, W);
  auto it = ctx->var_plans.find(key);
  if (it != ctx->var_plans.end()) return *static_cast<VarPlan*>(it->second.get());
  const uint32_t nb_w = 1u << (c - 1);
  std::vector<SegDesc> s1, s2(256);
  uint32_t lvl_off = 0, cnt = (uint32_t)W * nb_w;
  for (auto& d : s2) d = SegDesc{0, 1, 0, 0};
  for (int l = 0; l < c - 1; l++) {
    const uint32_t pw = nb_w >> (l + 1);
    const uint32_t ch = std::min<uint32_t>((uint32_t)SEG_CHUNK, pw);
    for (int w = 0; w < W; w++) {
      const uint32_t first = (uint32_t)s1.size();
      for (uint32_t j = 0; j < pw / ch; j++)
        s1.push_back(SegDesc{lvl_off + (uint32_t)w * (nb_w >> l) + 1 + 2 * j * ch, 2, ch, (uint32_t)s1.size()});
      const int t = c * w + l;
      if (t < 256) s2[t] = SegDesc{first, 1, (uint32_t)s1.size() - first, (uint32_t)t};
    }
    lvl_off += cnt;
    cnt >>= 1;
  }
  for (int t = 0; t < 256; t++) s2[t].out = (uint32_t)t;
  auto vp = std::make_shared<VarPlan>();
  vp->n1 = (uint32_t)s1.size();
  vp->n2 = 256;
  ZKP_HIP(hipMemcpyAsync(vp->d1.as<SegDesc>(s1.size()), s1.data(), s1.size() * sizeof(SegDesc), hipMemcpyHostToDevice, st));
  ZKP_HIP(hipMemcpyAsync(vp->d2.as<SegDesc>(256), s2.data(), 256 * sizeof(SegDesc), hipMemcpyHostToDevice, st));
  ZKP_HIP(hipStreamSynchronize(st));
  ctx->var_plans[key] = vp;
  return *vp;
}

static void msm_run_entry(zkp_ctx* ctx, const BasesEntry* be, size_t offset, const uint64_t* scalars_dev, size_t n,
                          bool montgomery, uint64_t* out_xyz_host, void* out_dev_xyzz, float* ms_accumulate,
                          uint64_t* n_entries, int ws_idx, int sort_src, float* ms_scan, int l1_src) {
  const MsmVtbl* vt = be->vt;
  MsmWorkspace& ws = ctx->cur->ws[ws_idx];
  const bool defer = ctx->msm_defer_reduce;
  const int into = ctx->msm_acc_into;
  const int bucket_ws = into >= 0 ? into : ctx->msm_bucket_ws;
  ctx->msm_defer_reduce = false;
  ctx->msm_acc_into = -1;
  ctx->msm_bucket_ws = -1;
  ZKP_REQUIRE(!(defer || into >= 0) || (n > 0 && !be->var && be->group == 1), ZKP_ERR_BAD_ARG);
  const bool reuse = sort_src >= 0;
  MsmWorkspace& sw = reuse ? ctx->cur->ws[sort_src] : ws;
  hipStream_t st = ws_idx == 0 ? ctx->cur->stream : ws.stream;
  const size_t XB = vt->bucket_bytes;
  const size_t jac_words = 3 * (size_t)vt->fN;
  uint32_t* out_jac = ws.out.as<uint32_t>(64 * 4);
  if (ms_accumulate) *ms_accumulate = 0.f;
  if (ms_scan) *ms_scan = 0.f;
  if (n_entries) *n_entries = 0;
  if (n == 0) {
    vt->write_identity(st, (char*)out_dev_xyzz, out_jac);
  } else {
    const int c = be->c, W = be->W, wide = be->wide;
    const int var = be->var ? 1 : 0;
    const int lgk = be->lgk, K = 1 << lgk;
    ZKP_REQUIRE(var == (lgk > 0), ZKP_ERR_BAD_ARG);
    const uint32_t nb_w = 1u << (c - 1);
    const int kbits = (c - 1) + lgk;
    const uint32_t nb = 1u << kbits;
    const size_t E = n * (size_t)W;
    ZKP_REQUIRE(E < 2147483000ull, ZKP_ERR_BAD_ARG);
    const bool l1_reuse = !reuse && l1_src >= 0;
    MsmWorkspace& lw = l1_reuse ? ctx->cur->ws[l1_src] : sw;
    uint32_t* vals = sw.vals.as<uint32_t>(E + 8);
    uint64_t* kv = lw.keys2.as<uint64_t>(E);
    const uint32_t* sc = reinterpret_cast<const uint32_t*>(scalars_dev);
    const int mont = montgomery ? 1 : 0;
    static const int h1_env = [] { const char* e = getenv("ZKP_SORT_H1"); return e ? atoi(e) : 0; }();
    int H1 = 10;
    while (H1 < SORT_H1_MAX && (E >> H1) > SORT_BIN_TARGET) H1++;
    if (h1_env > 0) H1 = std::min(SORT_H1_MAX, h1_env);
    H1 = std::min(H1, kbits);
    if (kbits - H1 > SORT_L_MAX) H1 = kbits - SORT_L_MAX;
    const int LB = kbits - H1;
    const uint32_t nbins1 = 1u << H1;
    uint32_t tile = SORT_SCALARS;
    while ((n + tile - 1) / tile > 1536) tile += 256;
    const uint32_t nblocks = (uint32_t)((n + tile - 1) / tile);
    const size_t hist_n = (size_t)nbins1 * nblocks + 1;
    uint32_t* hist = lw.sort_tmp.as<uint32_t>(2 * hist_n);
    uint32_t* offs = hist + hist_n;
    uint32_t* start = sw.offsets.as<uint32_t>(2 * (size_t)nb);
    uint32_t* end = start + nb;
    const uint8_t* scan_inf = be->sort_inf && !ctx->profiling ? be->sort_inf : be->inf;
    if (reuse) {
      if (sort_src != ws_idx) ZKP_HIP(hipStreamWaitEvent(st, sw.sorted, 0));
    } else if (l1_reuse) {
      if (l1_src != ws_idx) ZKP_HIP(hipStreamWaitEvent(st, lw.l1_done, 0));
    } else {
      ZKP_HIP(hipMemsetAsync(hist + hist_n - 1, 0, 4, st));
    }
    const uint8_t* grp = scan_inf == be->sort_inf ? be->group_flags : nullptr;
    static const bool staged_on = !(getenv("ZKP_SORT_STAGED") && atoi(getenv("ZKP_SORT_STAGED")) == 0);
    uint32_t staged_sub = 0;
    size_t staged_lds = 0;
    if (staged_on && nbins1 <= 2048 && (size_t)256 * W * 8 <= SORT_STAGE_BYTES) {
      staged_sub = (uint32_t)(SORT_STAGE_BYTES / ((size_t)W * 8)) / 256 * 256;
      staged_sub = std::min<uint32_t>(staged_sub, tile);
      staged_lds = ((size_t)nbins1 + ((nbins1 + 3) & ~3u)) * 4 + (size_t)staged_sub * W * 8;
    }
    const bool timed_scan = ms_scan && ctx->profiling && !reuse && !l1_reuse;
    if (timed_scan) ZKP_HIP(hipEventRecord(ctx->ev2, st));
    if (reuse || l1_reuse) {
    } else {
      static const int nt_hist = [] { const char* e = getenv("ZKP_SORT_NT_HIST"); return e ? atoi(e) : 1024; }();
      static const int nt_scat = [] { const char* e = getenv("ZKP_SORT_NT_SCATTER"); return e ? atoi(e) : 512; }();
      auto level1 = [&](auto tag) {
        using FrP = decltype(tag);
        auto hist_l = [&](auto nt) {
          constexpr int NT = decltype(nt)::value;
          hipLaunchKernelGGL((sort_hist_kernel<FrP, NT>), dim3(nblocks), dim3(NT), 0, st, sc, n, offset, scan_inf, mont, c, W, wide, nb_w,
                             LB, nbins1, hist, nblocks, tile, lgk);
        };
        if (nt_hist >= 1024) hist_l(std::integral_constant<int, 1024>{});
        else if (nt_hist >= 512) hist_l(std::integral_constant<int, 512>{});
        else hist_l(std::integral_constant<int, 256>{});
        exclusive_scan_u32(st, hist, offs, hist_n, ws.scan_tmp);
        if (staged_sub) {
          auto scat_l = [&](auto nt) {
            constexpr int NT = decltype(nt)::value;
            hipLaunchKernelGGL((sort_scatter_staged_kernel<FrP, NT>), dim3(nblocks), dim3(NT), staged_lds, st, sc, n, offset,
                               scan_inf, mont, be->n, c, W, wide, nb_w, LB, nbins1, offs, nblocks, tile, kv, lgk, grp, staged_sub);
          };
          if (nt_scat >= 1024) scat_l(std::integral_constant<int, 1024>{});
          else if (nt_scat >= 512) scat_l(std::integral_constant<int, 512>{});
          else scat_l(std::integral_constant<int, 256>{});
        } else {
          hipLaunchKernelGGL(sort_scatter_kernel<FrP>, dim3(nblocks), dim3(256), 0, st, sc, n, offset, scan_inf, mont, be->n, c, W, wide,
                             nb_w, LB, nbins1, offs, nblocks, tile, kv, lgk, grp);
        }
      };
      if (be->curve == ZKP_BN254) level1(Bn254Fr{});
      else level1(Bls381Fr{});
    }
    if (timed_scan) {
      ZKP_HIP(hipEventRecord(ctx->ev3, st));
      ZKP_HIP(hipEventSynchronize(ctx->ev3));
      ZKP_HIP(hipEventElapsedTime(ms_scan, ctx->ev2, ctx->ev3));
    }
    if (!reuse && !l1_reuse) ZKP_HIP(hipEventRecord(ws.l1_done, st));
    if (!reuse && !l1_reuse) ctx->mark(st, ":l1");
    if (!reuse)
      hipLaunchKernelGGL(sort_bin_kernel, dim3(nbins1), dim3(SORT_BIN_THREADS), ((size_t)4 << LB) + 4 * (size_t)SORT_BIN_STAGE, st,
                         kv, offs, nblocks, LB, vals, start, end, (l1_reuse || grp) ? be->filter_bit : -1);
    uint32_t* const sorted_vals = vals;
    const uint32_t max_tasks = nb + (uint32_t)(E / be->cap) + 1;
    uint32_t* sched = sw.sched.as<uint32_t>((size_t)2 * (nb + 2) + (size_t)8 * max_tasks + TM_WORDS + 8);
    uint32_t* tcount = sched;
    uint32_t* toff = tcount + (nb + 2);
    uint32_t* task_start = toff + (nb + 2);
    uint32_t* task_len = task_start + max_tasks;
    uint32_t* task_dst = task_len + max_tasks;
    uint32_t* long_list = task_dst + max_tasks;
    uint32_t* tmeta = long_list + max_tasks;
    uint4* desc = reinterpret_cast<uint4*>((reinterpret_cast<uintptr_t>(tmeta + TM_WORDS) + 15) & ~(uintptr_t)15);
    if (!reuse) {
      ZKP_HIP(hipMemsetAsync(tmeta, 0, TM_WORDS * 4, st));
      hipLaunchKernelGGL(task_count_kernel, dim3((nb + 256) / 256), dim3(256), 0, st, start, end, nb, tcount, be->cap);
      exclusive_scan_u32(st, tcount, toff, (size_t)nb + 1, ws.scan_tmp2);
      static const uint32_t tnt = [] { const char* e = getenv("ZKP_TASK_NT"); const int v = e ? atoi(e) : 1024; return (uint32_t)(v >= 1024 ? 1024 : v >= 512 ? 512 : 256); }();
      hipLaunchKernelGGL(task_fill_kernel, dim3((nb + tnt - 1) / tnt), dim3(tnt), 0, st, start, end, toff, nb, task_start,
                         task_len, task_dst, long_list, tmeta, be->cap);
      hipLaunchKernelGGL(task_cursor_kernel, dim3(1), dim3(64), 0, st, tmeta);
      hipLaunchKernelGGL(task_order_kernel, dim3((max_tasks + tnt - 1) / tnt), dim3(tnt), 0, st, task_start, task_len, task_dst,
                         toff + nb, tmeta, desc);
      ZKP_HIP(hipEventRecord(ws.sorted, st));
      ctx->mark(st, ":sorted");
    }
    MsmWorkspace& bws = bucket_ws >= 0 ? ctx->cur->ws[bucket_ws] : ws;
    char* buckets = reinterpret_cast<char*>(bws.buckets.get((size_t)2 * nb * XB + XB));
    char* task_partial = reinterpret_cast<char*>(ws.partial.get((size_t)max_tasks * XB));
    static const bool zero_all = getenv("ZKP_MEMSET_BUCKETS") && atoi(getenv("ZKP_MEMSET_BUCKETS")) != 0;
    const uint32_t init = into >= 0 ? 1u : 0u;
    if (init) {
      ZKP_REQUIRE(bws.chain_nb == nb && bws.chain_xb == XB, ZKP_ERR_BAD_ARG);
      ZKP_HIP(hipStreamWaitEvent(st, bws.acc_done, 0));
    } else if (zero_all) ZKP_HIP(hipMemsetAsync(buckets, 0, (size_t)nb * XB, st));
    else hipLaunchKernelGGL(zero_empty_buckets_kernel, dim3((nb + 255) / 256), dim3(256), 0, st, start, end, nb, buckets, (uint32_t)XB);
    bws.chain_nb = 0;
    const bool timed = ms_accumulate && ctx->profiling;
    if (timed) ZKP_HIP(hipEventRecord(ctx->ev2, st));
    static const uint32_t force_redo = getenv("ZKP_DEBUG_FORCE_REDO") && atoi(getenv("ZKP_DEBUG_FORCE_REDO")) != 0 ? 2u : 0u;
    ctx->mark(st, ":acc0");
    vt->accumulate(st, be->table, sorted_vals, desc, toff + nb, max_tasks, buckets, task_partial,
                   ws.redo.as<uint32_t>((size_t)max_tasks + 1), init | force_redo);
    ctx->mark(st, ":acc1");
    if (timed) {
      ZKP_HIP(hipEventRecord(ctx->ev3, st));
      ZKP_HIP(hipEventSynchronize(ctx->ev3));
      ZKP_HIP(hipEventElapsedTime(ms_accumulate, ctx->ev2, ctx->ev3));
    }
    static const int dbg = [] { const char* e = getenv("ZKP_DEBUG_MSM"); return e ? atoi(e) : 0; }();
    if (dbg) {
      uint32_t* rep = ws.redo.as<uint32_t>((size_t)max_tasks + 1);
      ZKP_HIP(hipStreamSynchronize(st));
      ZKP_HIP(hipMemsetAsync(rep, 0, 32, st));
      hipLaunchKernelGGL(sched_check_kernel, dim3(256), dim3(256), 0, st, toff, long_list, tmeta, nb, max_tasks, rep);
      uint32_t h[8];
      ZKP_HIP(hipMemcpyAsync(h, rep, 32, hipMemcpyDeviceToHost, st));
      ZKP_HIP(hipStreamSynchronize(st));
      printf("[msm] group=%d n=%zu nb=%u max_tasks=%u: toff inversions=%u max tasks/bucket=%u bad long_list=%u n_long=%u n_tasks=%u overflow=%u\n",
             be->group, n, nb, max_tasks, h[0], h[1], h[2], h[3], h[4], h[5]);
      fflush(stdout);
    }
#ifdef ZKP_ABLATION
    if (dbg != 2)
#endif
      vt->combine(st, long_list, tmeta + TM_NLONG, toff, task_partial, buckets, init);
    if (dbg) {
      hipError_t e = hipStreamSynchronize(st);
      printf("[msm] combine: %s\n", hipGetErrorString(e));
      fflush(stdout);
    }
    if (n_entries) {
      *n_entries = E;
      if (ctx->profiling) {
        uint32_t emitted = 0;
        ZKP_HIP(hipMemcpyAsync(&emitted, offs + hist_n - 1, 4, hipMemcpyDeviceToHost, st));
        ZKP_HIP(hipStreamSynchronize(st));
        *n_entries = emitted;
      }
    }
    if (var) {
      VarPlan& vp = var_plan(ctx, c, K, st);
      uint32_t lvl_off = 0, cnt = nb;
      for (int l = 0; l < c - 1; l++) {
        vt->pair(st, buckets + (size_t)lvl_off * XB, buckets + (size_t)(lvl_off + cnt) * XB, cnt / 2);
        lvl_off += cnt;
        cnt /= 2;
      }
      const char* roots = buckets + (size_t)lvl_off * XB;
      char* partial = reinterpret_cast<char*>(ws.tmp.get(((size_t)vp.n1 + 256 + 8) * XB));
      char* R = partial + (size_t)vp.n1 * XB;
      vt->segsum_desc(st, buckets, vp.d1.as<SegDesc>(vp.n1), vp.n1, partial);
      vt->segsum_desc(st, partial, vp.d2.as<SegDesc>(256), 256, R);
      vt->final_var(st, R, roots, c, K, (char*)out_dev_xyzz, out_jac);
      ZKP_HIP(hipGetLastError());
      if (out_xyz_host) {
        ZKP_HIP(hipMemcpyAsync(out_xyz_host, out_jac, jac_words * 4, hipMemcpyDeviceToHost, st));
        ZKP_HIP(hipStreamSynchronize(st));
      }
      return;
    }
    if (defer) {
      bws.chain_nb = nb;
      bws.chain_xb = XB;
      ZKP_HIP(hipEventRecord(bws.acc_done, st));
      vt->write_identity(st, (char*)out_dev_xyzz, out_jac);
      ZKP_HIP(hipGetLastError());
      ZKP_REQUIRE(!out_xyz_host, ZKP_ERR_BAD_ARG);
      return;
    }
#ifdef ZKP_ABLATION
    if (ctx->dbg_skip_k8) return;
#endif
    const int L = c - 1;
    SegPlan plan{};
    plan.L = L;
    const uint32_t chunk = ctx->batch_mode ? SEG_CHUNK_BATCH : SEG_CHUNK;
    plan.chunk = chunk;
    uint32_t lvl_off = 0, cnt = nb, blocks = 0;
    static const bool fuse_seg = !(getenv("ZKP_PAIR_TOP_FUSE_SEG") && atoi(getenv("ZKP_PAIR_TOP_FUSE_SEG")) == 0);
    int l_top = -1;
    char* top_base = nullptr;
    uint32_t top_cnt = 0;
    for (int l = 0; l < L; l++) {
      uint32_t next_off = lvl_off + cnt;
      static const bool top_fused = !(getenv("ZKP_PAIR_TOP") && atoi(getenv("ZKP_PAIR_TOP")) == 0);
      static const uint32_t top_max = [] {
        const char* e = getenv("ZKP_PAIR_TOP_MAX");
        uint32_t v = e ? (uint32_t)atoi(e) : PAIR_TOP_MAX;
        if (v < 2) v = PAIR_TOP_MAX;
        while (v & (v - 1)) v &= v - 1;
        return v;
      }();
      if (!top_fused || cnt > top_max) vt->pair(st, buckets + (size_t)lvl_off * XB, buckets + (size_t)next_off * XB, cnt / 2);
      else if (cnt == top_max || l == 0) {
        if (fuse_seg && cnt / 2 <= chunk) {
          l_top = l;
          top_base = buckets + (size_t)lvl_off * XB;
          top_cnt = cnt;
        } else {
          vt->pair_top(st, buckets + (size_t)lvl_off * XB, cnt);
        }
      }
      plan.first_block[l] = blocks;
      plan.off[l] = lvl_off + 1;
      plan.stride[l] = 2;
      plan.count[l] = cnt / 2;
      blocks += (cnt / 2 + chunk - 1) / chunk;
      lvl_off = next_off;
      cnt /= 2;
    }
    plan.first_block[L] = blocks;
    const char* root = buckets + (size_t)lvl_off * XB;
    char* partial = reinterpret_cast<char*>(ws.tmp.get(((size_t)blocks + 64) * XB));
    char* Obuf = partial + (size_t)blocks * XB;
    if (L > 0 && l_top >= 0) {
      SegPlan low = plan;
      low.L = l_top;
      const uint32_t blocks_low = plan.first_block[l_top];
      vt->pair_top_segsum(st, top_base, top_cnt, buckets, &low, partial, blocks_low);
      SegPlan p2{};
      p2.L = L;
      p2.chunk = chunk;
      for (int l = 0; l < L; l++) {
        p2.first_block[l] = l;
        if (l < l_top) {
          p2.off[l] = plan.first_block[l];
          p2.stride[l] = 1;
          p2.count[l] = plan.first_block[l + 1] - plan.first_block[l];
        } else {
          p2.off[l] = plan.off[l];
          p2.stride[l] = plan.stride[l];
          p2.count[l] = plan.count[l];
        }
        ZKP_REQUIRE(p2.count[l] <= chunk, ZKP_ERR_BAD_ARG);
      }
      p2.first_block[L] = L;
      vt->segsum(st, partial, &p2, Obuf, L, buckets, l_top);
    } else if (L > 0) {
      vt->segsum(st, buckets, &plan, partial, blocks, nullptr, 1 << 30);
      SegPlan p2{};
      p2.L = L;
      p2.chunk = chunk;
      for (int l = 0; l < L; l++) {
        p2.first_block[l] = l;
        p2.off[l] = plan.first_block[l];
        p2.stride[l] = 1;
        p2.count[l] = plan.first_block[l + 1] - plan.first_block[l];
        ZKP_REQUIRE(p2.count[l] <= chunk, ZKP_ERR_BAD_ARG);
      }
      p2.first_block[L] = L;
      vt->segsum(st, partial, &p2, Obuf, L, nullptr, 1 << 30);
    }
    vt->final(st, Obuf, L, root, (char*)out_dev_xyzz, out_jac);
    ctx->mark(st, ":reduced");
  }
  ZKP_HIP(hipGetLastError());
  if (out_xyz_host) {
    ZKP_HIP(hipMemcpyAsync(out_xyz_host, out_jac, jac_words * 4, hipMemcpyDeviceToHost, st));
    ZKP_HIP(hipStreamSynchronize(st));
  }
}

void msm_run_multi(zkp_ctx* ctx, size_t count, const uint64_t* handles, const size_t* offsets,
                   const uint64_t* const* scalars_dev, const size_t* ns, bool montgomery, uint64_t* out_xyz_host,
                   size_t slot_words) {
  if (count == 0) return;
// ... 300 lines not shown
```

### ckb_zkp_amd/csrc/ntt.hip

```cpp
#include <algorithm>
#include <cstdlib>

#include "ctx.hpp"
#include "field_dev.hpp"
#include "unsat_dev.hpp"

namespace zkp {

constexpr int NTT_SMAX = 9;
static int ntt_smax() {
  static const int v = [] {
    const char* e = getenv("ZKP_NTT_SMAX");
    int s = e ? atoi(e) : NTT_SMAX;
    return s < 4 ? 4 : (s > 10 ? 10 : s);
  }();
  return v;
}
#ifndef ZKP_NTT_TILE_LOG
#define ZKP_NTT_TILE_LOG 10
#endif
#ifndef ZKP_NTT_THREADS
#define ZKP_NTT_THREADS 256
#endif
constexpr int NTT_TILE_LOG = ZKP_NTT_TILE_LOG;
// ... 476 lines not shown
    F r;
    x.to_words(r.v);
    F::reduce_once(r).store(out + (size_t)oidx * 8);
  }
}
static bool ntt_v2() {
  static const bool on = !(getenv("ZKP_NTT_V2") && atoi(getenv("ZKP_NTT_V2")) == 0);
  return on;
}
template <class P>
static void ntt_launch(hipStream_t st, const NttPassArgs& a, uint32_t grid, int count) {
  const size_t tile = (size_t)1 << (a.S + a.logC);
  const size_t tw_bytes = ((size_t)1 << a.S) / 2 * 4 * Fu<P>::L + 32;
  if (ntt_v2() && tile == ((size_t)1 << NTT_TILE_LOG))
    hipLaunchKernelGGL((ntt_pass2_kernel<P, (1 << NTT_TILE_LOG)>), dim3(grid, count), dim3(NTT_THREADS),
                       NTT2_PLANE(tile) * 4 * Fu<P>::L + tw_bytes, st, a);
  else if (ntt_v2())
    hipLaunchKernelGGL((ntt_pass2_kernel<P, 0>), dim3(grid, count), dim3(NTT_THREADS), NTT2_PLANE(tile) * 4 * Fu<P>::L + tw_bytes, st, a);
  else
    hipLaunchKernelGGL(ntt_pass_kernel<P>, dim3(grid, count), dim3(NTT_THREADS), tile * 32 + tw_bytes, st, a);
}

static void ntt_plan(int log_n, int* S, int* P) {
  if (log_n == 0) {
    *P = 0;
    return;
  }
  const int smax = ntt_smax();
  int p = (log_n + smax - 1) / smax;
  int base = log_n / p, rem = log_n % p;
  for (int i = 0; i < p; i++) S[i] = base + (i < rem ? 1 : 0);
  *P = p;
}

template <class P>
static uint32_t* full_table(zkp_ctx* ctx, NttTables& t, uint32_t** slot, const uint32_t* lo, const uint32_t* hi, int S,
                            int logB, int twiddle) {
  static const bool enabled = !(getenv("ZKP_NTT_FULL") && atoi(getenv("ZKP_NTT_FULL")) == 0);
  if (!enabled || t.log_n > NTT_FULL_MAX_LOG || t.log_n < 2) return nullptr;
  if (*slot) return *slot;
  const size_t N = (size_t)1 << t.log_n;
  uint32_t* blk;
  if (hipMalloc(&blk, N * 32) != hipSuccess) return nullptr;
  hipStream_t s = ctx->cur->stream;
  hipLaunchKernelGGL(ntt_full_table_kernel<P>, dim3((N + 255) / 256), dim3(256), 0, s, blk, lo, hi, t.h, (uint32_t)N, S,
                     logB, twiddle, ntt_v2() ? 1 : 0);
  ZKP_HIP(hipGetLastError());
  ZKP_HIP(hipStreamSynchronize(s));
  t.extra.push_back(blk);
  *slot = blk;
  return blk;
}

template <class P>
void ntt_run_t(zkp_ctx* ctx, int curve, uint32_t* const* data, int count, int log_n, int op) {
  ZKP_REQUIRE(log_n <= P::TWO_ADICITY, ZKP_ERR_DOMAIN_TOO_LARGE);
  ZKP_REQUIRE(count >= 1 && count <= NTT_MAX_BATCH, ZKP_ERR_BAD_ARG);
  if (log_n == 0) return;
  NttTables& t = get_tables<P>(ctx, curve, log_n);
  const size_t N = (size_t)1 << log_n;
  int S[8], np;
  ntt_plan(log_n, S, &np);
  const bool odd = (np & 1) && np > 1;
  uint32_t* scratch = ctx->cur->ntt_scratch.as<uint32_t>((size_t)count * N * 8 * (odd ? 2 : 1));
  uint32_t* scratch2 = scratch + (size_t)count * N * 8;
  const bool inverse = (op == ZKP_NTT_IFFT || op == ZKP_NTT_COSET_IFFT);
  bool in_scratch = false;
  int logB = 0;
  const uint32_t* src_base = nullptr;
  for (int p = 0; p < np; p++) {
    uint32_t* dst_base;
    if (np == 1) dst_base = scratch;
    else if (p == np - 1) dst_base = nullptr;
    else if (!odd) dst_base = ((np - 1 - p) & 1) ? scratch : nullptr;
    else dst_base = (p & 1) ? scratch2 : scratch;
    NttPassArgs a{};
    for (int k = 0; k < count; k++) {
      a.in[k] = src_base ? src_base + (size_t)k * N * 8 : data[k];
      a.out[k] = dst_base ? dst_base + (size_t)k * N * 8 : data[k];
    }
    in_scratch = dst_base != nullptr;
    a.log_n = log_n;
    a.S = S[p];
    a.logB = logB;
    int logC = std::min(NTT_TILE_LOG - S[p], log_n - S[p]);
    a.logC = logC;
    a.sub_log = std::min(log_n, NTT_SUB_LOG);
    a.last = (p == np - 1);
    a.h = t.h;
    a.tw_sub = inverse ? t.sub_inv : t.sub_fwd;
    a.tw_lo = inverse ? t.wi_lo : t.w_lo;
    a.tw_hi = inverse ? t.wi_hi : t.w_hi;
    if (!a.last)
      a.tw_full = full_table<P>(ctx, t, inverse ? &t.full_inv[p] : &t.full_fwd[p], a.tw_lo, a.tw_hi, S[p], logB, 1);
    if (p == 0 && op == ZKP_NTT_COSET_FFT) {
      a.pre_lo = t.g_lo;
      a.pre_hi = t.g_hi;
      a.pre_full = full_table<P>(ctx, t, &t.full_g, t.g_lo, t.g_hi, 0, 0, 0);
    }
    if (p == np - 1) {
      if (op == ZKP_NTT_COSET_IFFT) {
        a.post_lo = t.gi_lo;
        a.post_hi = t.gi_hi;
        a.post_full = full_table<P>(ctx, t, &t.full_gi, t.gi_lo, t.gi_hi, 0, 0, 0);
      } else if (op == ZKP_NTT_IFFT) {
        a.post_const = t.n_inv;
      }
    }
    ntt_launch<P>(ctx->cur->stream, a, (uint32_t)(N >> (S[p] + logC)), count);
    src_base = dst_base;
    logB += S[p];
  }
  ZKP_HIP(hipGetLastError());
  if (in_scratch)
    for (int k = 0; k < count; k++)
      ZKP_HIP(hipMemcpyAsync(data[k], scratch + (size_t)k * N * 8, N * 32, hipMemcpyDeviceToDevice, ctx->cur->stream));
}

template <class P>
static void launch_pass(zkp_ctx* ctx, NttTables& t, int log_n, const int* S, int np, int p, int logB, bool inverse,
                        const uint32_t* in, uint32_t* out, NttPassArgs a) {
  a.in[0] = in;
  a.out[0] = out;
  a.log_n = log_n;
  a.S = S[p];
  a.logB = logB;
  const int logC = std::min(NTT_TILE_LOG - S[p], log_n - S[p]);
  a.logC = logC;
  a.sub_log = std::min(log_n, NTT_SUB_LOG);
  a.last = (p == np - 1);
  a.h = t.h;
  a.tw_sub = inverse ? t.sub_inv : t.sub_fwd;
  a.tw_lo = inverse ? t.wi_lo : t.w_lo;
  a.tw_hi = inverse ? t.wi_hi : t.w_hi;
  if (!a.last) a.tw_full = full_table<P>(ctx, t, inverse ? &t.full_inv[p] : &t.full_fwd[p], a.tw_lo, a.tw_hi, S[p], logB, 1);
  ntt_launch<P>(ctx->cur->stream, a, (uint32_t)(((size_t)1 << log_n) >> (S[p] + logC)), 1);
}

template <class P>
static bool ntt_ifft_coset_fft_t(zkp_ctx* ctx, int curve, uint32_t* data, int log_n) {
  if (log_n < 2 || log_n > NTT_FULL_MAX_LOG) return false;
  NttTables& t = get_tables<P>(ctx, curve, log_n);
  uint32_t* pre = full_table<P>(ctx, t, &t.full_g_n, t.g_lo, t.g_hi_n, 0, 0, 0);
  if (!pre) return false;
  const size_t N = (size_t)1 << log_n;
  uint32_t* scratch = ctx->cur->ntt_scratch.as<uint32_t>(N * 8);
  int S[8], np;
  ntt_plan(log_n, S, &np);
  uint32_t* buf[2] = {data, scratch};
  int cur = 0;
  for (int half = 0; half < 2; half++) {
    int logB = 0;
    for (int p = 0; p < np; p++) {
      NttPassArgs a{};
      if (half == 1 && p == 0) a.pre_full = pre;
      launch_pass<P>(ctx, t, log_n, S, np, p, logB, half == 0, buf[cur], buf[cur ^ 1], a);
      cur ^= 1;
      logB += S[p];
    }
  }
  ZKP_HIP(hipGetLastError());
  return true;
}

template <class P>
static uint32_t* ntt_qap_coset_ifft_t(zkp_ctx* ctx, int curve, uint32_t* a_, uint32_t* b_, uint32_t* c_, const uint32_t* zinv,
                                      int log_n) {
  if (log_n < 2 || log_n > NTT_FULL_MAX_LOG) return nullptr;
  NttTables& t = get_tables<P>(ctx, curve, log_n);
  uint32_t* post = full_table<P>(ctx, t, &t.full_gi, t.gi_lo, t.gi_hi, 0, 0, 0);
  if (!post) return nullptr;
  const size_t N = (size_t)1 << log_n;
  uint32_t* scratch = ctx->cur->ntt_scratch.as<uint32_t>(N * 8);
  int S[8], np;
  ntt_plan(log_n, S, &np);
  if (np < 2) return nullptr;
  const uint32_t* in = a_;
  uint32_t* out = scratch;
  int logB = 0;
  for (int p = 0; p < np; p++) {
    NttPassArgs a{};
    if (p == 0) {
      a.fuse_b = b_;
      a.fuse_c = c_;
      a.fuse_k = zinv;
    }
    if (p == np - 1) {
      a.post_lo = t.gi_lo;
      a.post_hi = t.gi_hi;
      a.post_full = post;
      if (out == scratch) out = b_;
    }
    launch_pass<P>(ctx, t, log_n, S, np, p, logB, true, in, out, a);
    in = out;
    out = (out == scratch) ? a_ : scratch;
    logB += S[p];
  }
  ZKP_HIP(hipGetLastError());
  return const_cast<uint32_t*>(in);
}

bool ntt_ifft_coset_fft(zkp_ctx* ctx, int curve, uint32_t* data, int log_n) {
  static const bool on = !(getenv("ZKP_NTT_FUSE") && atoi(getenv("ZKP_NTT_FUSE")) == 0);
  if (!on) return false;
  if (curve == ZKP_BN254) return ntt_ifft_coset_fft_t<Bn254Fr>(ctx, curve, data, log_n);
  if (curve == ZKP_BLS12_381) return ntt_ifft_coset_fft_t<Bls381Fr>(ctx, curve, data, log_n);
  throw StatusError{ZKP_ERR_UNSUPPORTED_CURVE};
}
uint32_t* ntt_qap_coset_ifft(zkp_ctx* ctx, int curve, uint32_t* a, uint32_t* b, uint32_t* c, const uint32_t* zinv, int log_n) {
  static const bool on = !(getenv("ZKP_NTT_FUSE") && atoi(getenv("ZKP_NTT_FUSE")) == 0);
  if (!on) return nullptr;
  if (curve == ZKP_BN254) return ntt_qap_coset_ifft_t<Bn254Fr>(ctx, curve, a, b, c, zinv, log_n);
  if (curve == ZKP_BLS12_381) return ntt_qap_coset_ifft_t<Bls381Fr>(ctx, curve, a, b, c, zinv, log_n);
  throw StatusError{ZKP_ERR_UNSUPPORTED_CURVE};
}

void ntt_run_batch(zkp_ctx* ctx, int curve, uint32_t* const* data, int count, int log_n, int op) {
  ZKP_REQUIRE(op >= 0 && op <= 3, ZKP_ERR_BAD_ARG);
  if (curve == ZKP_BN254) ntt_run_t<Bn254Fr>(ctx, curve, data, count, log_n, op);
  else if (curve == ZKP_BLS12_381) ntt_run_t<Bls381Fr>(ctx, curve, data, count, log_n, op);
  else throw StatusError{ZKP_ERR_UNSUPPORTED_CURVE};
}

void ntt_run(zkp_ctx* ctx, int curve, uint32_t* data, int log_n, int op) {
  uint32_t* one[1] = {data};
  ntt_run_batch(ctx, curve, one, 1, log_n, op);
// ... 12 lines not shown
```

### ckb_zkp_amd/groth16.py

```python
from __future__ import annotations

import ctypes as C
import secrets
from dataclasses import dataclass, field

import numpy as np

from . import _lib
from .api import Context, _ptr
from .codec import fr_canonical, fr_to_mont, g1_from_mont, g1_to_mont, g2_from_mont, g2_to_mont, ints_to_limbs
from .params import CurveParams, get_curve
from .r1cs import ConstraintSystem, PolynomialDegreeTooLarge, R1csInstance


@dataclass
class Proof:
    a: tuple
    b: tuple
    c: tuple


@dataclass
class Parameters:
    curve: CurveParams
# ... 274 lines not shown
    def __init__(self, ctx: Context, params: Parameters, circuit, matrices_only: bool = False, shard=None, keep_form: bool = False):
        self.ctx, self.params, self.curve = ctx, params, params.curve
        self.shard = shard
        if shard is not None and keep_form:
            raise ValueError("keep_form applies to unsharded keys (zkp_groth16_pk_upload_ex); for a sharded key create the "
                             "context with dict(h_evaluation_form=False, c_fold=False)")
        inst = _as_instance(self.curve, circuit, assign=False)
        assert (inst.num_inputs, inst.num_aux, inst.num_constraints()) == \
            (params.num_inputs, params.num_aux, params.num_constraints)
        d = _lib.Groth16PkDesc()
        d.curve, d.num_inputs, d.num_aux, d.num_constraints = self.curve.cid, inst.num_inputs, inst.num_aux, \
            inst.num_constraints()
        keep = []

        def P(a):
            a = np.ascontiguousarray(a)
            keep.append(a)
            return a.ctypes.data

        for name, which in (("at", "a"), ("bt", "b"), ("ct", "c")):
            rp, col, cf = inst.csr(which)
            m = getattr(d, name)
            m.row_ptr, m.col, m.coeff = P(rp.astype(np.uint32)), P(col.astype(np.uint32)), P(cf.astype(np.uint64))
        for name in ("alpha_g1", "beta_g1", "delta_g1", "beta_g2", "delta_g2"):
            setattr(d, name, P(getattr(params, name).astype(np.uint64)))
        for name, fld in (() if matrices_only else (("a", "a_query"), ("b_g1", "b_g1_query"), ("b_g2", "b_g2_query"),
                                                    ("h", "h_query"), ("l", "l_query"))):
            xy, inf = getattr(params, fld)
            setattr(d, f"{name}_query", P(xy.astype(np.uint64)))
            setattr(d, f"{name}_inf", P(inf.astype(np.uint8)) if len(inf) else None)
            setattr(d, f"{name}_len", len(inf))
        h = C.c_void_p()
        if shard is None and keep_form:
            _lib.check(ctx.lib.zkp_groth16_pk_upload_ex(ctx.h, C.byref(d), 1, C.byref(h)), "zkp_groth16_pk_upload_ex")
        elif shard is None:
            _lib.check(ctx.lib.zkp_groth16_pk_upload(ctx.h, C.byref(d), C.byref(h)), "zkp_groth16_pk_upload")
        else:
            _lib.check(ctx.lib.zkp_groth16_pk_upload_shard(ctx.h, C.byref(d), shard[0], shard[1], C.byref(h)),
                       "zkp_groth16_pk_upload_shard")
        self.h = h
        n = C.c_uint64()
        _lib.check(ctx.lib.zkp_groth16_domain_size(self.h, C.byref(n)), "zkp_groth16_domain_size")
        self.domain_size = n.value
        self.nz = inst.num_inputs + inst.num_aux

    def table_plan(self) -> dict:
        info = (C.c_uint64 * 8)()
        _lib.check(self.ctx.lib.zkp_groth16_pk_info(self.ctx.h, self.h, info), "zkp_groth16_pk_info")
        return {"window_group": int(info[0]), "table_bytes": int(info[1]), "window_bits": int(info[2]), "windows": int(info[3]),
                "table_copies": int(info[4]), "window_bits_b": int(info[5]), "b1_reuses_b2_sort": bool(info[6] & 1),
                "l_reuses_a_sort": bool(info[6] & 2), "shared_level1_pass": bool(info[6] & 4),
                "h_evaluation_form": bool(info[7] & 1), "c_folded_into_l": bool(info[7] & 2), "l_h_bucket_chained": bool(info[7] & 4)}

    def free(self):
        if self.h:
            _lib.check(self.ctx.lib.zkp_groth16_pk_free(self.ctx.h, self.h), "zkp_groth16_pk_free")
            self.h = None

    def witness_map(self, z_mont: np.ndarray) -> np.ndarray:
        z = np.ascontiguousarray(z_mont, dtype=np.uint64)
        assert z.shape == (self.nz, 4)
        h = np.zeros((self.domain_size, 4), dtype=np.uint64)
        _lib.check(self.ctx.lib.zkp_groth16_witness_map(self.ctx.h, self.h, _ptr(z), _ptr(h)), "zkp_groth16_witness_map")
        return h

    def witness_map_dev(self, z_dev: int, h_dev: int):
        _lib.check(self.ctx.lib.zkp_groth16_witness_map_dev(self.ctx.h, self.h, C.c_void_p(z_dev), C.c_void_p(h_dev)),
                   "zkp_groth16_witness_map_dev")

    def partials_dev(self, z_dev: int, r: int, s: int, out_dev: int):
        c = self.curve
        rm, sm = fr_to_mont([r], c)[0], fr_to_mont([s], c)[0]
        _lib.check(self.ctx.lib.zkp_groth16_prove_partials_dev(self.ctx.h, self.h, C.c_void_p(z_dev), _ptr(rm), _ptr(sm),
                                                              C.c_void_p(out_dev)), "zkp_groth16_prove_partials_dev")

    def prove_raw(self, z, r_mont: np.ndarray, s_mont: np.ndarray, z_on_device: bool = False):
        c = self.curve
        words = 4 * c.fq_limbs + 4 * c.fq_limbs
        out = np.zeros(words, dtype=np.uint64)
        inf = np.zeros(3, dtype=np.uint8)
        r_mont = np.ascontiguousarray(r_mont, dtype=np.uint64)
        s_mont = np.ascontiguousarray(s_mont, dtype=np.uint64)
        if z_on_device:
            st = self.ctx.lib.zkp_groth16_prove_dev(self.ctx.h, self.h, C.c_void_p(z), _ptr(r_mont), _ptr(s_mont),
                                                    _ptr(out), _ptr(inf))
        else:
            z = np.ascontiguousarray(z, dtype=np.uint64)
            assert z.shape == (self.nz, 4)
            st = self.ctx.lib.zkp_groth16_prove(self.ctx.h, self.h, _ptr(z), _ptr(r_mont), _ptr(s_mont), _ptr(out),
                                                _ptr(inf))
        _lib.check(st, "zkp_groth16_prove")
        return out, inf

    def witness_map_host(self, z_mont: np.ndarray) -> np.ndarray:
        return self.witness_map(z_mont)

    def prove_batch_raw(self, z_devs, r_mont: np.ndarray, s_mont: np.ndarray, z_on_device: bool = True):
        n = len(z_devs)
        words = 8 * self.curve.fq_limbs
        out = np.zeros((n, words), dtype=np.uint64)
        inf = np.zeros((n, 3), dtype=np.uint8)
        zp = (C.c_void_p * n)(*[C.c_void_p(z) for z in z_devs])
        r_mont = np.ascontiguousarray(r_mont, dtype=np.uint64).reshape(n, 4)
        s_mont = np.ascontiguousarray(s_mont, dtype=np.uint64).reshape(n, 4)
        fn = self.ctx.lib.zkp_groth16_prove_batch_dev if z_on_device else self.ctx.lib.zkp_groth16_prove_batch
        _lib.check(fn(self.ctx.h, self.h, n, C.cast(zp, C.c_void_p), _ptr(r_mont), _ptr(s_mont), _ptr(out), _ptr(inf)),
# ... 122 lines not shown
```

### include/zkp_accel.h

```cpp
#ifndef ZKP_ACCEL_H
#define ZKP_ACCEL_H
#include <stddef.h>
#include <stdint.h>
#ifdef __cplusplus
extern "C" {
#endif

typedef enum { ZKP_BN254 = 0, ZKP_BLS12_381 = 1 } zkp_curve_t;

typedef enum {
  ZKP_OK = 0,
  ZKP_ERR_BAD_ARG = -1,
  ZKP_ERR_UNSUPPORTED_CURVE = -2,
  ZKP_ERR_DOMAIN_TOO_LARGE = -3,
  ZKP_ERR_OOM = -4,
  ZKP_ERR_DEVICE = -5,
  ZKP_ERR_BAD_HANDLE = -6,
  ZKP_ERR_INVALID_POINT = -7
} zkp_status;

typedef enum { ZKP_NTT_FFT = 0, ZKP_NTT_IFFT = 1, ZKP_NTT_COSET_FFT = 2, ZKP_NTT_COSET_IFFT = 3 } zkp_ntt_op;

typedef struct zkp_ctx zkp_ctx;

// ... 101 lines not shown
int32_t zkp_g1_into_affine(zkp_ctx* ctx, zkp_curve_t curve, const uint64_t* xyz_host, uint64_t* xy_out,
                           uint8_t* inf_out);
int32_t zkp_g2_into_affine(zkp_ctx* ctx, zkp_curve_t curve, const uint64_t* xyz_host, uint64_t* xy_out,
                           uint8_t* inf_out);
int32_t zkp_groth16_points_into_affine(zkp_curve_t curve, const uint64_t* a_xyzz, const uint64_t* b_xyzz, const uint64_t* c_xyzz,
                                       uint64_t* proof_out, uint8_t* inf_out);

int32_t zkp_g1_decompress(zkp_ctx* ctx, zkp_curve_t curve, const uint8_t* bytes, size_t n, uint64_t* xy_out, uint8_t* inf_out,
                          size_t* bad_index);
int32_t zkp_g2_decompress(zkp_ctx* ctx, zkp_curve_t curve, const uint8_t* bytes, size_t n, uint64_t* xy_out, uint8_t* inf_out,
                          size_t* bad_index);
int32_t zkp_g1_compress(zkp_ctx* ctx, zkp_curve_t curve, const uint64_t* xy, const uint8_t* inf, size_t n, uint8_t* bytes_out);
int32_t zkp_g2_compress(zkp_ctx* ctx, zkp_curve_t curve, const uint64_t* xy, const uint8_t* inf, size_t n, uint8_t* bytes_out);
int32_t zkp_g1_subgroup_check(zkp_ctx* ctx, zkp_curve_t curve, const uint64_t* xy, const uint8_t* inf, size_t n, size_t* bad_index);
int32_t zkp_g2_subgroup_check(zkp_ctx* ctx, zkp_curve_t curve, const uint64_t* xy, const uint8_t* inf, size_t n, size_t* bad_index);

int32_t zkp_fixed_base_mul_g1(zkp_ctx* ctx, zkp_curve_t curve, const uint64_t* base_xy, const uint64_t* scalars_host,
                              size_t n, uint64_t* out_xy, uint8_t* out_inf);
int32_t zkp_fixed_base_mul_g2(zkp_ctx* ctx, zkp_curve_t curve, const uint64_t* base_xy, const uint64_t* scalars_host,
                              size_t n, uint64_t* out_xy, uint8_t* out_inf);

typedef struct {
  const uint32_t* row_ptr;
  const uint32_t* col;
  const uint64_t* coeff;
} zkp_csr;

typedef struct {
  zkp_curve_t curve;
  uint32_t num_inputs;
  uint32_t num_aux;
  uint32_t num_constraints;
  zkp_csr at, bt, ct;
  const uint64_t* alpha_g1; const uint64_t* beta_g1; const uint64_t* delta_g1;
  const uint64_t* beta_g2; const uint64_t* delta_g2;
  const uint64_t* a_query; const uint8_t* a_inf; size_t a_len;
  const uint64_t* b_g1_query; const uint8_t* b_g1_inf; size_t b_g1_len;
  const uint64_t* b_g2_query; const uint8_t* b_g2_inf; size_t b_g2_len;
  const uint64_t* h_query; const uint8_t* h_inf; size_t h_len;
  const uint64_t* l_query; const uint8_t* l_inf; size_t l_len;
} zkp_groth16_pk_desc;

typedef struct zkp_groth16_pk zkp_groth16_pk;

int32_t zkp_groth16_pk_upload(zkp_ctx* ctx, const zkp_groth16_pk_desc* desc, zkp_groth16_pk** out);
#define ZKP_PK_KEEP_FORM 1u
int32_t zkp_groth16_pk_upload_ex(zkp_ctx* ctx, const zkp_groth16_pk_desc* desc, uint32_t flags, zkp_groth16_pk** out);
int32_t zkp_groth16_pk_free(zkp_ctx* ctx, zkp_groth16_pk* pk);

int32_t zkp_groth16_witness_map(zkp_ctx* ctx, zkp_groth16_pk* pk, const uint64_t* z_host, uint64_t* h_host);
int32_t zkp_groth16_witness_map_dev(zkp_ctx* ctx, zkp_groth16_pk* pk, const uint64_t* z_dev, uint64_t* h_dev);
int32_t zkp_groth16_domain_size(zkp_groth16_pk* pk, uint64_t* n);
int32_t zkp_groth16_pk_info(zkp_ctx* ctx, zkp_groth16_pk* pk, uint64_t info[8]);

int32_t zkp_groth16_prove(zkp_ctx* ctx, zkp_groth16_pk* pk, const uint64_t* z_host, const uint64_t* r,
                          const uint64_t* s, uint64_t* proof_out, uint8_t* inf_out);
int32_t zkp_groth16_prove_dev(zkp_ctx* ctx, zkp_groth16_pk* pk, const uint64_t* z_dev, const uint64_t* r,
                              const uint64_t* s, uint64_t* proof_out, uint8_t* inf_out);

int32_t zkp_groth16_prove_batch_dev(zkp_ctx* ctx, zkp_groth16_pk* pk, size_t n, const uint64_t* const* z_dev,
                                    const uint64_t* r, const uint64_t* s, uint64_t* proofs_out, uint8_t* inf_out);

int32_t zkp_groth16_prove_batch(zkp_ctx* ctx, zkp_groth16_pk* pk, size_t n, const uint64_t* const* z_host,
                                const uint64_t* r, const uint64_t* s, uint64_t* proofs_out, uint8_t* inf_out);

int32_t zkp_groth16_assemble(zkp_ctx* ctx, zkp_curve_t curve, const uint64_t* sums_xyz, const uint64_t* r,
                             const uint64_t* s, uint64_t* proof_out, uint8_t* inf_out);

int32_t zkp_groth16_pk_upload_shard(zkp_ctx* ctx, const zkp_groth16_pk_desc* desc, int32_t rank, int32_t world,
                                    zkp_groth16_pk** out);
int32_t zkp_groth16_partials_bytes(zkp_curve_t curve, size_t* bytes);
int32_t zkp_groth16_prove_partials_dev(zkp_ctx* ctx, zkp_groth16_pk* pk, const uint64_t* z_dev, const uint64_t* r,
                                       const uint64_t* s, void* partials_dev);
int32_t zkp_groth16_fold_assemble_dev(zkp_ctx* ctx, zkp_curve_t curve, const void* gathered_dev, int32_t world,
                                      const uint64_t* r, const uint64_t* s, uint64_t* proof_out, uint8_t* inf_out);

typedef struct zkp_groth16_pk_multi zkp_groth16_pk_multi;
typedef enum { ZKP_MULTI_SHARD = 0, ZKP_MULTI_REPLICATE = 1 } zkp_multi_mode;
int32_t zkp_ctx_create_multi(zkp_ctx** out, const int* device_ids, int n_devices);
int32_t zkp_ctx_create_multi_ex(zkp_ctx** out, const int* device_ids, int n_devices, const zkp_ctx_config* cfg);
int32_t zkp_ctx_num_devices(zkp_ctx* ctx, int32_t* n);
int32_t zkp_ctx_device(zkp_ctx* ctx, int32_t rank, zkp_ctx** member);
int32_t zkp_groth16_pk_upload_multi(zkp_ctx* ctx, const zkp_groth16_pk_desc* desc, int32_t mode,
                                    zkp_groth16_pk_multi** out);
int32_t zkp_groth16_pk_multi_free(zkp_ctx* ctx, zkp_groth16_pk_multi* pk);
int32_t zkp_groth16_multi_info(zkp_ctx* ctx, zkp_groth16_pk_multi* pk, uint64_t info[6]);
int32_t zkp_groth16_prove_multi(zkp_ctx* ctx, zkp_groth16_pk_multi* pk, const uint64_t* const* z, int32_t z_on_device,
                                const uint64_t* r, const uint64_t* s, uint64_t* proof_out, uint8_t* inf_out);
int32_t zkp_groth16_prove_batch_multi(zkp_ctx* ctx, zkp_groth16_pk_multi* pk, size_t count, const uint64_t* const* z,
                                      int32_t z_on_device, const uint64_t* r, const uint64_t* s, uint64_t* proofs_out,
                                      uint8_t* inf_out);

typedef struct zkp_fs_rng zkp_fs_rng;
int32_t zkp_fs_rng_new(const uint8_t* seed_material, size_t len, zkp_fs_rng** out);
int32_t zkp_fs_rng_free(zkp_fs_rng* rng);
int32_t zkp_fs_rng_absorb(zkp_fs_rng* rng, const uint8_t* material, size_t len);
int32_t zkp_fs_rng_seed(const zkp_fs_rng* rng, uint8_t out32[32]);
int32_t zkp_fs_rng_next_u64(zkp_fs_rng* rng, uint64_t* out);
int32_t zkp_fs_rng_rand_u128(zkp_fs_rng* rng, uint64_t out[2]);
int32_t zkp_fs_rng_rand_fr(zkp_fs_rng* rng, zkp_curve_t curve, uint64_t* out_mont);
int32_t zkp_fs_rng_sample_outside_domain(zkp_fs_rng* rng, zkp_curve_t curve, uint32_t log_domain, uint64_t* out_mont);
int32_t zkp_merlin_oneshot(const uint8_t* label, size_t label_len, const uint8_t* msg_label, size_t msg_label_len,
                           const uint8_t* msg, size_t msg_len, const uint8_t* chal_label, size_t chal_label_len,
                           uint8_t* out, size_t out_len);

typedef struct zkp_marlin_index zkp_marlin_index;
// ... 78 lines not shown
```

### rust/zkp-accel/src/ffi.rs

```rust
#![allow(non_camel_case_types, clippy::too_many_arguments)]
use std::os::raw::{c_char, c_int, c_void};

#[repr(C)]
pub struct zkp_ctx {
    _p: [u8; 0],
}
#[repr(C)]
pub struct zkp_groth16_pk {
    _p: [u8; 0],
}
#[repr(C)]
pub struct zkp_groth16_pk_multi {
    _p: [u8; 0],
}
#[repr(C)]
pub struct zkp_fs_rng {
    _p: [u8; 0],
}
#[repr(C)]
pub struct zkp_marlin_index {
    _p: [u8; 0],
}

pub const ZKP_BN254: c_int = 0;
// ... 174 lines not shown
    pub fn zkp_timer_stop_ms(ctx: *mut zkp_ctx, ms: *mut f32) -> i32;
    pub fn zkp_ntt(ctx: *mut zkp_ctx, curve: c_int, data_host: *mut u64, log_n: u32, op: i32) -> i32;
    pub fn zkp_ntt_dev(ctx: *mut zkp_ctx, curve: c_int, data_dev: *mut u64, log_n: u32, op: i32) -> i32;
    pub fn zkp_fr_vec_op_dev(ctx: *mut zkp_ctx, curve: c_int, op: i32, a: *const u64, b: *const u64, k_host: *const u64, out: *mut u64, n: usize) -> i32;
    pub fn zkp_fr_spmv_dev(ctx: *mut zkp_ctx, curve: c_int, row_ptr_dev: *const u32, col_dev: *const u32, coeff_dev: *const u64, nrows: usize, x_dev: *const u64, out_dev: *mut u64) -> i32;
    pub fn zkp_fr_gather_dev(ctx: *mut zkp_ctx, in_dev: *const u64, idx_dev: *const i32, n: usize, out_dev: *mut u64) -> i32;
    pub fn zkp_poly_divide_by_vanishing_dev(ctx: *mut zkp_ctx, curve: c_int, p_dev: *const u64, len: usize, n: usize, q_dev: *mut u64, rem_dev: *mut u64) -> i32;
    pub fn zkp_d2d(ctx: *mut zkp_ctx, dst_dev: *mut c_void, src_dev: *const c_void, bytes: usize) -> i32;
    pub fn zkp_dev_zero(ctx: *mut zkp_ctx, dst_dev: *mut c_void, bytes: usize) -> i32;
    pub fn zkp_fr_batch_inverse_dev(ctx: *mut zkp_ctx, curve: c_int, v: *mut u64, n: usize) -> i32;
    pub fn zkp_poly_evaluate_dev(ctx: *mut zkp_ctx, curve: c_int, p: *const u64, n: usize, z_host: *const u64, eval_out_host: *mut u64) -> i32;
    pub fn zkp_poly_div_linear_dev(ctx: *mut zkp_ctx, curve: c_int, p: *const u64, n: usize, z_host: *const u64, q_dev: *mut u64, eval_out_host: *mut u64) -> i32;
    pub fn zkp_bases_upload_g1(ctx: *mut zkp_ctx, curve: c_int, xy: *const u64, inf: *const u8, n: usize, handle: *mut u64) -> i32;
    pub fn zkp_bases_upload_g2(ctx: *mut zkp_ctx, curve: c_int, xy: *const u64, inf: *const u8, n: usize, handle: *mut u64) -> i32;
    pub fn zkp_bases_free(ctx: *mut zkp_ctx, handle: u64) -> i32;
    pub fn zkp_bases_share(dst: *mut zkp_ctx, src: *mut zkp_ctx, src_handle: u64, dst_handle: *mut u64) -> i32;
    pub fn zkp_bases_len(ctx: *mut zkp_ctx, handle: u64, n: *mut usize) -> i32;
    pub fn zkp_msm_g1(ctx: *mut zkp_ctx, handle: u64, offset: usize, scalars_host: *const u64, n: usize, out_xyz: *mut u64) -> i32;
    pub fn zkp_msm_g2(ctx: *mut zkp_ctx, handle: u64, offset: usize, scalars_host: *const u64, n: usize, out_xyz: *mut u64) -> i32;
    pub fn zkp_msm_g1_dev(ctx: *mut zkp_ctx, handle: u64, offset: usize, scalars_dev: *const u64, n: usize, out_xyz_host: *mut u64) -> i32;
    pub fn zkp_msm_g2_dev(ctx: *mut zkp_ctx, handle: u64, offset: usize, scalars_dev: *const u64, n: usize, out_xyz_host: *mut u64) -> i32;
    pub fn zkp_vartime_multiscalar_mul_g1(ctx: *mut zkp_ctx, handle: u64, fr_scalars_host: *const u64, n: usize, out_xyz: *mut u64) -> i32;
    pub fn zkp_vartime_multiscalar_mul_g2(ctx: *mut zkp_ctx, handle: u64, fr_scalars_host: *const u64, n: usize, out_xyz: *mut u64) -> i32;
    pub fn zkp_msm_g1_var(ctx: *mut zkp_ctx, curve: c_int, xy_host: *const u64, inf_host: *const u8, scalars_host: *const u64, n: usize, montgomery: i32, out_xyz: *mut u64) -> i32;
    pub fn zkp_msm_g2_var(ctx: *mut zkp_ctx, curve: c_int, xy_host: *const u64, inf_host: *const u8, scalars_host: *const u64, n: usize, montgomery: i32, out_xyz: *mut u64) -> i32;
    pub fn zkp_msm_g1_var_batch_dev(ctx: *mut zkp_ctx, curve: c_int, count: usize, xy_dev: *const *const u64, inf_dev: *const *const u8, scalars_dev: *const *const u64, ns: *const usize, montgomery: i32, out_xyz: *mut u64) -> i32;
    pub fn zkp_msm_g2_var_batch_dev(ctx: *mut zkp_ctx, curve: c_int, count: usize, xy_dev: *const *const u64, inf_dev: *const *const u8, scalars_dev: *const *const u64, ns: *const usize, montgomery: i32, out_xyz: *mut u64) -> i32;
    pub fn zkp_g1_ipa_fold_dev(ctx: *mut zkp_ctx, curve: c_int, l_xy: *const u64, l_inf: *const u8, r_xy: *const u64, r_inf: *const u8, n: usize, a_host: *const u64, b_host: *const u64, out_xy: *mut u64, out_inf: *mut u8) -> i32;
    pub fn zkp_fr_dot_batch_dev(ctx: *mut zkp_ctx, curve: c_int, count: usize, a_dev: *const *const u64, b_dev: *const *const u64, ns: *const usize, out_host: *mut u64) -> i32;
    pub fn zkp_msm_g1_mont_dev(ctx: *mut zkp_ctx, handle: u64, offset: usize, fr_scalars_dev: *const u64, n: usize, out_xyz_host: *mut u64) -> i32;
    pub fn zkp_msm_g2_mont_dev(ctx: *mut zkp_ctx, handle: u64, offset: usize, fr_scalars_dev: *const u64, n: usize, out_xyz_host: *mut u64) -> i32;
    pub fn zkp_msm_g1_mont_batch_dev(ctx: *mut zkp_ctx, bases_handle: u64, count: usize, offsets: *const usize, scalars_dev: *const *const u64, ns: *const usize, out_xyz: *mut u64) -> i32;
    pub fn zkp_msm_mont_multi_dev(ctx: *mut zkp_ctx, count: usize, bases_handles: *const u64, offsets: *const usize, scalars_dev: *const *const u64, ns: *const usize, out_xyz: *mut u64, slot_u64: usize) -> i32;
    pub fn zkp_g1_fold(ctx: *mut zkp_ctx, curve: c_int, xyz_host: *const u64, k: usize, out_xyz: *mut u64) -> i32;
    pub fn zkp_g2_fold(ctx: *mut zkp_ctx, curve: c_int, xyz_host: *const u64, k: usize, out_xyz: *mut u64) -> i32;
    pub fn zkp_g1_into_affine(ctx: *mut zkp_ctx, curve: c_int, xyz_host: *const u64, xy_out: *mut u64, inf_out: *mut u8) -> i32;
    pub fn zkp_g2_into_affine(ctx: *mut zkp_ctx, curve: c_int, xyz_host: *const u64, xy_out: *mut u64, inf_out: *mut u8) -> i32;
    pub fn zkp_groth16_points_into_affine(curve: c_int, a_xyzz: *const u64, b_xyzz: *const u64, c_xyzz: *const u64, proof_out: *mut u64, inf_out: *mut u8) -> i32;
    pub fn zkp_g1_decompress(ctx: *mut zkp_ctx, curve: c_int, bytes: *const u8, n: usize, xy_out: *mut u64, inf_out: *mut u8, bad_index: *mut usize) -> i32;
    pub fn zkp_g2_decompress(ctx: *mut zkp_ctx, curve: c_int, bytes: *const u8, n: usize, xy_out: *mut u64, inf_out: *mut u8, bad_index: *mut usize) -> i32;
    pub fn zkp_g1_compress(ctx: *mut zkp_ctx, curve: c_int, xy: *const u64, inf: *const u8, n: usize, bytes_out: *mut u8) -> i32;
    pub fn zkp_g2_compress(ctx: *mut zkp_ctx, curve: c_int, xy: *const u64, inf: *const u8, n: usize, bytes_out: *mut u8) -> i32;
    pub fn zkp_g1_subgroup_check(ctx: *mut zkp_ctx, curve: c_int, xy: *const u64, inf: *const u8, n: usize, bad_index: *mut usize) -> i32;
    pub fn zkp_g2_subgroup_check(ctx: *mut zkp_ctx, curve: c_int, xy: *const u64, inf: *const u8, n: usize, bad_index: *mut usize) -> i32;
    pub fn zkp_fixed_base_mul_g1(ctx: *mut zkp_ctx, curve: c_int, base_xy: *const u64, scalars_host: *const u64, n: usize, out_xy: *mut u64, out_inf: *mut u8) -> i32;
    pub fn zkp_fixed_base_mul_g2(ctx: *mut zkp_ctx, curve: c_int, base_xy: *const u64, scalars_host: *const u64, n: usize, out_xy: *mut u64, out_inf: *mut u8) -> i32;
    pub fn zkp_groth16_pk_upload(ctx: *mut zkp_ctx, desc: *const zkp_groth16_pk_desc, out: *mut *mut zkp_groth16_pk) -> i32;
    pub fn zkp_groth16_pk_upload_ex(ctx: *mut zkp_ctx, desc: *const zkp_groth16_pk_desc, flags: u32, out: *mut *mut zkp_groth16_pk) -> i32;
    pub fn zkp_groth16_pk_free(ctx: *mut zkp_ctx, pk: *mut zkp_groth16_pk) -> i32;
    pub fn zkp_groth16_witness_map(ctx: *mut zkp_ctx, pk: *mut zkp_groth16_pk, z_host: *const u64, h_host: *mut u64) -> i32;
    pub fn zkp_groth16_witness_map_dev(ctx: *mut zkp_ctx, pk: *mut zkp_groth16_pk, z_dev: *const u64, h_dev: *mut u64) -> i32;
    pub fn zkp_groth16_domain_size(pk: *mut zkp_groth16_pk, n: *mut u64) -> i32;
    pub fn zkp_groth16_pk_info(ctx: *mut zkp_ctx, pk: *mut zkp_groth16_pk, info: *mut u64) -> i32;
    pub fn zkp_groth16_prove(ctx: *mut zkp_ctx, pk: *mut zkp_groth16_pk, z_host: *const u64, r: *const u64, s: *const u64, proof_out: *mut u64, inf_out: *mut u8) -> i32;
    pub fn zkp_groth16_prove_dev(ctx: *mut zkp_ctx, pk: *mut zkp_groth16_pk, z_dev: *const u64, r: *const u64, s: *const u64, proof_out: *mut u64, inf_out: *mut u8) -> i32;
    pub fn zkp_groth16_prove_batch_dev(ctx: *mut zkp_ctx, pk: *mut zkp_groth16_pk, n: usize, z_dev: *const *const u64, r: *const u64, s: *const u64, proofs_out: *mut u64, inf_out: *mut u8) -> i32;
    pub fn zkp_groth16_prove_batch(ctx: *mut zkp_ctx, pk: *mut zkp_groth16_pk, n: usize, z_host: *const *const u64, r: *const u64, s: *const u64, proofs_out: *mut u64, inf_out: *mut u8) -> i32;
    pub fn zkp_groth16_assemble(ctx: *mut zkp_ctx, curve: c_int, sums_xyz: *const u64, r: *const u64, s: *const u64, proof_out: *mut u64, inf_out: *mut u8) -> i32;
    pub fn zkp_groth16_pk_upload_shard(ctx: *mut zkp_ctx, desc: *const zkp_groth16_pk_desc, rank: i32, world: i32, out: *mut *mut zkp_groth16_pk) -> i32;
    pub fn zkp_groth16_partials_bytes(curve: c_int, bytes: *mut usize) -> i32;
    pub fn zkp_groth16_prove_partials_dev(ctx: *mut zkp_ctx, pk: *mut zkp_groth16_pk, z_dev: *const u64, r: *const u64, s: *const u64, partials_dev: *mut c_void) -> i32;
    pub fn zkp_groth16_fold_assemble_dev(ctx: *mut zkp_ctx, curve: c_int, gathered_dev: *const c_void, world: i32, r: *const u64, s: *const u64, proof_out: *mut u64, inf_out: *mut u8) -> i32;
    pub fn zkp_ctx_create_multi(out: *mut *mut zkp_ctx, device_ids: *const c_int, n_devices: c_int) -> i32;
    pub fn zkp_ctx_create_multi_ex(out: *mut *mut zkp_ctx, device_ids: *const c_int, n_devices: c_int, cfg: *const zkp_ctx_config) -> i32;
    pub fn zkp_ctx_num_devices(ctx: *mut zkp_ctx, n: *mut i32) -> i32;
    pub fn zkp_ctx_device(ctx: *mut zkp_ctx, rank: i32, member: *mut *mut zkp_ctx) -> i32;
    pub fn zkp_groth16_pk_upload_multi(ctx: *mut zkp_ctx, desc: *const zkp_groth16_pk_desc, mode: i32, out: *mut *mut zkp_groth16_pk_multi) -> i32;
    pub fn zkp_groth16_pk_multi_free(ctx: *mut zkp_ctx, pk: *mut zkp_groth16_pk_multi) -> i32;
    pub fn zkp_groth16_multi_info(ctx: *mut zkp_ctx, pk: *mut zkp_groth16_pk_multi, info: *mut u64) -> i32;
    pub fn zkp_groth16_prove_multi(ctx: *mut zkp_ctx, pk: *mut zkp_groth16_pk_multi, z: *const *const u64, z_on_device: i32, r: *const u64, s: *const u64, proof_out: *mut u64, inf_out: *mut u8) -> i32;
    pub fn zkp_groth16_prove_batch_multi(ctx: *mut zkp_ctx, pk: *mut zkp_groth16_pk_multi, count: usize, z: *const *const u64, z_on_device: i32, r: *const u64, s: *const u64, proofs_out: *mut u64, inf_out: *mut u8) -> i32;
    pub fn zkp_fs_rng_new(seed_material: *const u8, len: usize, out: *mut *mut zkp_fs_rng) -> i32;
    pub fn zkp_fs_rng_free(rng: *mut zkp_fs_rng) -> i32;
    pub fn zkp_fs_rng_absorb(rng: *mut zkp_fs_rng, material: *const u8, len: usize) -> i32;
    pub fn zkp_fs_rng_seed(rng: *const zkp_fs_rng, out32: *mut u8) -> i32;
    pub fn zkp_fs_rng_next_u64(rng: *mut zkp_fs_rng, out: *mut u64) -> i32;
    pub fn zkp_fs_rng_rand_u128(rng: *mut zkp_fs_rng, out: *mut u64) -> i32;
    pub fn zkp_fs_rng_rand_fr(rng: *mut zkp_fs_rng, curve: c_int, out_mont: *mut u64) -> i32;
    pub fn zkp_fs_rng_sample_outside_domain(rng: *mut zkp_fs_rng, curve: c_int, log_domain: u32, out_mont: *mut u64) -> i32;
    pub fn zkp_merlin_oneshot(label: *const u8, label_len: usize, msg_label: *const u8, msg_label_len: usize, msg: *const u8, msg_len: usize, chal_label: *const u8, chal_label_len: usize, out: *mut u8, out_len: usize) -> i32;
    pub fn zkp_marlin_index_upload(ctx: *mut zkp_ctx, desc: *const zkp_marlin_index_desc, out: *mut *mut zkp_marlin_index) -> i32;
    pub fn zkp_marlin_index_free(ctx: *mut zkp_ctx, index: *mut zkp_marlin_index) -> i32;
    pub fn zkp_marlin_index_info(index: *const zkp_marlin_index, info: *mut u64) -> i32;
    pub fn zkp_marlin_index_commit(ctx: *mut zkp_ctx, index: *mut zkp_marlin_index, powers_of_g: u64, comms_xy: *mut u64, inf: *mut u8) -> i32;
    pub fn zkp_marlin_prove(ctx: *mut zkp_ctx, index: *mut zkp_marlin_index, powers_of_g: u64, powers_of_gamma_g: u64, ivk_bytes: *const u8, ivk_len: usize, x: *const u64, w: *const u64, n_w: usize, rnd: *const zkp_marlin_rand, fixed_challenges: *const u64, out: *mut zkp_marlin_proof) -> i32;
    pub fn zkp_groth16_last_timing(ctx: *mut zkp_ctx, out: *mut zkp_groth16_timing) -> i32;
    pub fn zkp_marlin_last_timing(ctx: *mut zkp_ctx, out: *mut zkp_marlin_timing) -> i32;
    pub fn zkp_set_profiling(ctx: *mut zkp_ctx, enable: i32) -> i32;
    pub fn zkp_bench_mulmod(ctx: *mut zkp_ctx, curve: c_int, field: i32, unsaturated: i32, gmulmod_per_s: *mut f64) -> i32;
    pub fn zkp_bench_hbm_copy(ctx: *mut zkp_ctx, bytes: usize, gbytes_per_s: *mut f64) -> i32;
}
```

Before: 140.0 proofs/s.

## Pre-plan and slab-reserve per-lane scratch instead of warm-up proofs

Adds a scratch planner that computes the MSM workspace and NTT buffer sizes for each lane. It carves them, together with the per-lane key buffers, out of a single hipMalloc slab, reserved at key upload or at batch start. This replaces the old warm-up path, which ran a throwaway proof on every lane to grow the buffers, and it removes reallocations in the middle of a batch. The cost is extra planning code, asserts that the planned sizes match the real run, and more device memory held per key.

```diff
diff --git a/ckb_zkp_amd/_lib.py b/ckb_zkp_amd/_lib.py
--- a/ckb_zkp_amd/_lib.py
+++ b/ckb_zkp_amd/_lib.py
@@ -182,6 +182,7 @@
     "zkp_groth16_witness_map_dev": (C.c_int32, [vp, vp, vp, vp]),
     "zkp_groth16_domain_size": (C.c_int32, [vp, C.POINTER(C.c_uint64)]),
     "zkp_groth16_pk_info": (C.c_int32, [vp, vp, C.POINTER(C.c_uint64)]),
+    "zkp_groth16_batch_stats": (C.c_int32, [vp, vp, C.POINTER(C.c_uint64)]),
     "zkp_groth16_prove": (C.c_int32, [vp, vp, vp, vp, vp, vp, vp]),
     "zkp_groth16_prove_dev": (C.c_int32, [vp, vp, vp, vp, vp, vp, vp]),
     "zkp_groth16_prove_batch_dev": (C.c_int32, [vp, vp, C.c_size_t, vp, vp, vp, vp, vp]),
diff --git a/ckb_zkp_amd/csrc/capi.hip b/ckb_zkp_amd/csrc/capi.hip
--- a/ckb_zkp_amd/csrc/capi.hip
+++ b/ckb_zkp_amd/csrc/capi.hip
@@ -644,6 +644,10 @@
   if (!pk) return ZKP_ERR_BAD_ARG;
   return guarded(ctx, [&] { groth16_pk_free(ctx, pk); });
 }
+int32_t zkp_groth16_batch_stats(zkp_ctx* ctx, zkp_groth16_pk* pk, uint64_t info[6]) {
+  if (!ctx || !pk || !info) return ZKP_ERR_BAD_ARG;
+  return guarded(ctx, [&] { groth16_batch_stats(ctx, pk, info); });
+}
 int32_t zkp_groth16_pk_info(zkp_ctx* ctx, zkp_groth16_pk* pk, uint64_t info[8]) {
   if (!ctx || !pk || !info) return ZKP_ERR_BAD_ARG;
   return guarded(ctx, [&] { groth16_pk_info(ctx, pk, info); });
diff --git a/ckb_zkp_amd/csrc/ctx.hpp b/ckb_zkp_amd/csrc/ctx.hpp
--- a/ckb_zkp_amd/csrc/ctx.hpp
+++ b/ckb_zkp_amd/csrc/ctx.hpp
@@ -2,6 +2,7 @@
 #include <hip/hip_runtime.h>
 #include <stdint.h>
 
+#include <atomic>
 #include <map>
 #include <mutex>
 #include <memory>
@@ -33,26 +34,54 @@
     if (!(cond)) throw ::zkp::StatusError{(status)}; \
   } while (0)
 
+struct DevSlab {
+  void* p = nullptr;
+  size_t bytes = 0;
+  size_t views = 0;
+};
+inline std::atomic<uint64_t> devbuf_allocs{0};
+
 struct DevBuf {
   void* p = nullptr;
   size_t cap = 0;
+  DevSlab* slab = nullptr;
+  void release() {
+    if (slab) {
+      if (--slab->views == 0) {
+        (void)hipFree(slab->p);
+        delete slab;
+      }
+      slab = nullptr;
+    } else if (p) {
+      (void)hipFree(p);
+    }
+    p = nullptr;
+    cap = 0;
+  }
+  void view(DevSlab* s, size_t offset, size_t bytes) {
+    release();
+    slab = s;
+    s->views++;
+    p = static_cast<char*>(s->p) + offset;
+    cap = bytes;
+  }
   void* get(size_t bytes) {
     if (bytes > cap) {
-      if (p) (void)hipFree(p);
-      p = nullptr;
-      cap = 0;
+      release();
       size_t want = bytes + (bytes >> 3) + 256;
       hipError_t e = hipMalloc(&p, want);
-      if (e != hipSuccess) throw StatusError{ZKP_ERR_OOM};
+      if (e != hipSuccess) {
+        p = nullptr;
+        throw StatusError{ZKP_ERR_OOM};
+      }
+      devbuf_allocs.fetch_add(1, std::memory_order_relaxed);
       cap = want;
     }
     return p;
   }
   template <class T>
   T* as(size_t count) { return reinterpret_cast<T*>(get(count * sizeof(T))); }
-  ~DevBuf() {
-    if (p) (void)hipFree(p);
-  }
+  ~DevBuf() { release(); }
   DevBuf() = default;
   DevBuf(const DevBuf&) = delete;
   DevBuf& operator=(const DevBuf&) = delete;
@@ -93,6 +122,19 @@
   size_t chain_xb = 0;
   hipEvent_t acc_done = nullptr;
   DevBuf keys, vals, keys2, vals2, sort_tmp, offsets, buckets, tmp, out, sched, scan_tmp, scan_tmp2, partial, redo;
+  static constexpr int N_BUF = 14;
+  enum { KEYS, VALS, KEYS2, VALS2, SORT_TMP, OFFSETS, BUCKETS, TMP, OUT, SCHED, SCAN_TMP, SCAN_TMP2, PARTIAL, REDO };
+  DevBuf* buf(int i) {
+    DevBuf* const all[N_BUF] = {&keys, &vals, &keys2, &vals2, &sort_tmp, &offsets, &buckets, &tmp, &out, &sched, &scan_tmp, &scan_tmp2, &partial, &redo};
+    return all[i];
+  }
+};
+struct LaneScratchPlan {
+  size_t ws[4][MsmWorkspace::N_BUF] = {};
+  size_t ntt = 0;
+  void want(int w, int i, size_t bytes) {
+    if (bytes > ws[w][i]) ws[w][i] = bytes;
+  }
 };
 struct Groth16Timing {
   zkp_groth16_timing t{};
@@ -107,6 +149,7 @@
   static constexpr int N_WS_MSM = N_WS;
   zkp::MsmWorkspace ws[N_WS];
   zkp::DevBuf ntt_scratch;
+  zkp_groth16_pk* slab_pk = nullptr;
   hipEvent_t ev_fork = nullptr, ev_a = nullptr, ev_b1 = nullptr;
   uint32_t* host_proof = nullptr;
   bool host_tail = false;
diff --git a/ckb_zkp_amd/csrc/groth16.hip b/ckb_zkp_amd/csrc/groth16.hip
--- a/ckb_zkp_amd/csrc/groth16.hip
+++ b/ckb_zkp_amd/csrc/groth16.hip
@@ -40,13 +40,16 @@
     DevBuf S;
     DevBuf results;
     DevBuf proof;
-    bool warmed = false;
+    size_t slab_bytes = 0;
     int graph_state = 0;
     hipGraphExec_t graph_exec = nullptr;
     hipGraph_t graph = nullptr;
     std::vector<const void*> sig;
   } lane[zkp_ctx::N_LANES];
   DevBuf consts;
+  uint64_t enqueued = 0;
+  uint64_t last_batch_allocs = 0;
+  int reserved_where = 0;
 };
 
 namespace zkp {
@@ -393,6 +396,169 @@
   }
 }
 
+static int batch_lanes(const zkp_ctx* ctx, const zkp_groth16_pk* pk) {
+  const int lanes_default = pk->log_n <= 22 ? 8 : 4;
+  return std::max(1, std::min(ctx->cfg.lanes > 0 ? ctx->cfg.lanes : lanes_default, (int)zkp_ctx::N_LANES));
+}
+
+static bool lane_plan(zkp_ctx* ctx, zkp_groth16_pk* pk, bool batch_mode, LaneScratchPlan* P) {
+  if (!pk->hA || pk->shard_world != 0) return false;
+  const bool single_stream = getenv("ZKP_SINGLE_STREAM") && atoi(getenv("ZKP_SINGLE_STREAM")) != 0;
+  if (getenv("ZKP_LATENCY_PLAN") && atoi(getenv("ZKP_LATENCY_PLAN")) == 0) return false;
+  const bool fan = !single_stream;
+  for (int mode = 0; mode <= (batch_mode ? 1 : 0); mode++) {
+    auto add = [&](uint64_t h, size_t n, int w, int sort_src = -1, int l1_src = -1, int acc_into = -1, bool defer = false) {
+      msm_plan_scratch(ctx, h, n, fan ? w : 0, fan ? sort_src : -1, fan ? l1_src : -1, fan ? acc_into : -1, fan && defer, true,
+                       mode == 1, P);
+    };
+    const int l1 = pk->share_l1 ? 1 : -1;
+    const bool b_l1 = pk->share_l1 && pk->b_in_l1;
+    add(pk->hB2, pk->q_n[2], 2, -1, b_l1 ? l1 : -1);
+    add(pk->hA, pk->q_n[0], 1);
+    add(pk->hB1, pk->q_n[1], 3, pk->share_b_sort ? 2 : -1);
+    add(pk->hL, pk->q_n[4], 1, pk->share_al_sort ? 1 : -1, l1, -1, pk->chain_lh);
+    add(pk->hH, pk->q_n[3], 0, -1, -1, pk->chain_lh ? 1 : -1);
+  }
+  const bool ntt_batch = getenv("ZKP_NTT_BATCH") && atoi(getenv("ZKP_NTT_BATCH")) != 0;
+  P->ntt = std::max(ntt_scratch_bytes(pk->log_n, 1, true), ntt_scratch_bytes(pk->log_n, ntt_batch ? 3 : 1, false));
+  return true;
+}
+
+static constexpr size_t VIEW_ALIGN = 256;
+static constexpr size_t SLAB_ALIGN = (size_t)2 << 20;
+static size_t align_up(size_t v, size_t a) { return (v + a - 1) / a * a; }
+
+static void key_lane_bytes(const zkp_groth16_pk* pk, size_t out[4]) {
+  out[0] = 3 * pk->N * 32;
+  out[1] = (pk->nz + 4) * 32;
+  out[2] = 6 * msm_vtbl(pk->curve, 2)->xyzz_bytes;
+  out[3] = 4096;
+}
+
+static void release_lane_scratch(zkp_lane& L) {
+  for (auto& ws : L.ws)
+    for (int i = 0; i < MsmWorkspace::N_BUF; i++) ws.buf(i)->release();
+  L.ntt_scratch.release();
+  L.slab_pk = nullptr;
+}
+static void release_key_lane(zkp_groth16_pk::PerLane& PL) {
+  for (DevBuf* b : {&PL.abc, &PL.S, &PL.results, &PL.proof}) b->release();
+  PL.slab_bytes = 0;
+}
+static bool lane_covers(zkp_lane& L, const LaneScratchPlan& P) {
+  for (int w = 0; w < zkp_lane::N_WS; w++)
+    for (int i = 0; i < MsmWorkspace::N_BUF; i++)
+      if (L.ws[w].buf(i)->cap < P.ws[w][i]) return false;
+  return L.ntt_scratch.cap >= P.ntt;
+}
+static bool key_lane_covers(zkp_groth16_pk::PerLane& PL, const size_t kb[4]) {
+  return PL.abc.cap >= kb[0] && PL.S.cap >= kb[1] && PL.results.cap >= kb[2] && PL.proof.cap >= kb[3];
+}
+
+static size_t lane_slab_bytes(const LaneScratchPlan& P, const size_t kb[4]) {
+  size_t total = align_up(P.ntt, VIEW_ALIGN);
+  for (int w = 0; w < zkp_lane::N_WS; w++)
+    for (int i = 0; i < MsmWorkspace::N_BUF; i++) total += align_up(P.ws[w][i], VIEW_ALIGN);
+  for (int k = 0; k < 4; k++) total += align_up(kb[k], VIEW_ALIGN);
+  return align_up(total, SLAB_ALIGN);
+}
+
+int groth16_reserve_lanes(zkp_ctx* ctx, zkp_groth16_pk* pk, int first, int count, bool batch_mode) {
+  LaneScratchPlan P;
+  if (!lane_plan(ctx, pk, batch_mode, &P)) return 0;
+  size_t kb[4];
+  key_lane_bytes(pk, kb);
+  std::vector<int> taken;
+  const int end = std::min(first + count, (int)zkp_ctx::N_LANES);
+  for (int l = std::max(first, 0); l < end; l++) {
+    zkp_lane& L = ctx->lanes[l];
+    zkp_groth16_pk::PerLane& PL = pk->lane[l];
+    const bool lane_ok = lane_covers(L, P), key_ok = key_lane_covers(PL, kb);
+    if (lane_ok && key_ok) continue;
+    (void)hipStreamSynchronize(L.stream);
+    for (int w = 1; w < zkp_lane::N_WS; w++) (void)hipStreamSynchronize(L.ws[w].stream);
+    LaneScratchPlan Q = P;
+    if (!lane_ok) {
+      for (int w = 0; w < zkp_lane::N_WS; w++)
+        for (int i = 0; i < MsmWorkspace::N_BUF; i++) Q.want(w, i, L.ws[w].buf(i)->cap);
+      Q.ntt = std::max(Q.ntt, L.ntt_scratch.cap);
+      if (L.slab_pk && L.slab_pk != pk) release_key_lane(L.slab_pk->lane[l]);
+      release_lane_scratch(L);
+    }
+    release_key_lane(PL);
+    size_t total = 0;
+    for (int k = 0; k < 4; k++) total += align_up(kb[k], VIEW_ALIGN);
+    if (!lane_ok) {
+      total += align_up(Q.ntt, VIEW_ALIGN);
+      for (int w = 0; w < zkp_lane::N_WS; w++)
+        for (int i = 0; i < MsmWorkspace::N_BUF; i++) total += align_up(Q.ws[w][i], VIEW_ALIGN);
+    }
+    total = align_up(total, SLAB_ALIGN);
+    void* base = nullptr;
+    if (hipMalloc(&base, total) != hipSuccess) {
+      (void)hipGetLastError();
+      for (int t : taken) {
+        if (ctx->lanes[t].slab_pk == pk) release_lane_scratch(ctx->lanes[t]);
+        release_key_lane(pk->lane[t]);
+      }
+      return 0;
+    }
+    devbuf_allocs.fetch_add(1, std::memory_order_relaxed);
+    DevSlab* slab = new DevSlab{base, total, 0};
+    size_t off = 0;
+    auto place = [&](DevBuf& b, size_t bytes) {
+      if (bytes == 0) return;
+      b.view(slab, off, align_up(bytes, VIEW_ALIGN));
+      off += align_up(bytes, VIEW_ALIGN);
+    };
+    place(PL.abc, kb[0]);
+    place(PL.S, kb[1]);
+    place(PL.results, kb[2]);
+    place(PL.proof, kb[3]);
+    if (!lane_ok) {
+      place(L.ntt_scratch, Q.ntt);
+      for (int w = 0; w < zkp_lane::N_WS; w++)
+        for (int i = 0; i < MsmWorkspace::N_BUF; i++) place(*L.ws[w].buf(i), Q.ws[w][i]);
+      L.slab_pk = pk;
+    }
+    PL.slab_bytes = total;
+    taken.push_back(l);
+  }
+  return (int)taken.size();
+}
+
+static bool reserve_at_upload(zkp_ctx* ctx, zkp_groth16_pk* pk) {
+  LaneScratchPlan P;
+  if (!lane_plan(ctx, pk, true, &P)) return false;
+  size_t kb[4];
+  key_lane_bytes(pk, kb);
+  const int nl = batch_lanes(ctx, pk);
+  const size_t need = (size_t)nl * lane_slab_bytes(P, kb);
+  size_t free_b = 0, total_b = 0;
+  if (hipMemGetInfo(&free_b, &total_b) != hipSuccess) {
+    (void)hipGetLastError();
+    return false;
+  }
+  if (need > total_b / 8 || need > free_b / 2) return false;
+  if (const char* e = getenv("ZKP_RESERVE_UPLOAD_MAX_MB"))
+    if (need > (size_t)std::max(0L, atol(e)) << 20) return false;
+  if (groth16_reserve_lanes(ctx, pk, 0, nl, true) == 0) return false;
+  pk->reserved_where = 1;
+  return true;
+}
+
+void groth16_batch_stats(zkp_ctx* ctx, zkp_groth16_pk* pk, uint64_t info[6]) {
+  (void)ctx;
+  for (int i = 0; i < 6; i++) info[i] = 0;
+  info[0] = pk->enqueued;
+  info[1] = pk->last_batch_allocs;
+  for (auto& PL : pk->lane) {
+    info[2] += PL.slab_bytes ? 1 : 0;
+    info[3] += PL.slab_bytes;
+  }
+  info[4] = info[2] ? (uint64_t)pk->reserved_where : 0;
+}
+
 zkp_groth16_pk* groth16_pk_upload(zkp_ctx* ctx, const zkp_groth16_pk_desc* d, int rank, int world, int flags) {
   ZKP_REQUIRE(d->curve == ZKP_BN254 || d->curve == ZKP_BLS12_381, ZKP_ERR_UNSUPPORTED_CURVE);
   ZKP_REQUIRE(d->num_inputs >= 1, ZKP_ERR_BAD_ARG);
@@ -549,19 +715,22 @@
   if (d->curve == ZKP_BN254) hipLaunchKernelGGL(qap_consts_kernel<Bn254Fr>, dim3(1), dim3(64), 0, ctx->cur->stream, consts, lg);
   else hipLaunchKernelGGL(qap_consts_kernel<Bls381Fr>, dim3(1), dim3(64), 0, ctx->cur->stream, consts, lg);
   ZKP_HIP(hipGetLastError());
-  for (int l = 0; l < 2; l++) {
-    auto& L = pk->lane[l];
-    L.abc.get(3 * pk->N * 32);
-    L.S.get((pk->nz + 4) * 32);
-    L.results.get(6 * 16 * 24 * 4 + 64);
-    L.proof.get(4096);
-  }
   ZKP_HIP(hipStreamSynchronize(ctx->cur->stream));
+  if (!reserve_at_upload(ctx, pk.get()))
+    for (int l = 0; l < 2; l++) {
+      auto& L = pk->lane[l];
+      L.abc.get(3 * pk->N * 32);
+      L.S.get((pk->nz + 4) * 32);
+      L.results.get(6 * 16 * 24 * 4 + 64);
+      L.proof.get(4096);
+    }
   return pk.release();
 }
 
 void groth16_pk_free(zkp_ctx* ctx, zkp_groth16_pk* pk) {
   (void)hipDeviceSynchronize();
+  for (auto& L : ctx->lanes)
+    if (L.slab_pk == pk) release_lane_scratch(L);
   for (auto& PL : pk->lane) {
     if (PL.graph_exec) (void)hipGraphExecDestroy(PL.graph_exec);
     if (PL.graph) (void)hipGraphDestroy(PL.graph);
@@ -843,9 +1012,7 @@
   for (DevBuf* b : {&PL.abc, &PL.S, &PL.results, &PL.proof, &L->ntt_scratch}) sig.push_back(b->p);
   for (int w = 0; w < zkp_lane::N_WS; w++) {
     MsmWorkspace& ws = L->ws[w];
-    for (DevBuf* b : {&ws.keys, &ws.vals, &ws.keys2, &ws.vals2, &ws.sort_tmp, &ws.offsets, &ws.buckets, &ws.tmp, &ws.out,
-                      &ws.sched, &ws.scan_tmp, &ws.scan_tmp2, &ws.partial, &ws.redo})
-      sig.push_back(b->p);
+    for (int i = 0; i < MsmWorkspace::N_BUF; i++) sig.push_back(ws.buf(i)->p);
   }
   sig.push_back(pk);
   return sig;
@@ -856,6 +1023,7 @@
                           const uint64_t* s, bool latency_plan = false) {
   static const bool graph_on = getenv("ZKP_GRAPH") && atoi(getenv("ZKP_GRAPH")) != 0;
   static const bool single_stream = getenv("ZKP_SINGLE_STREAM") && atoi(getenv("ZKP_SINGLE_STREAM")) != 0;
+  pk->enqueued++;
   if (!graph_on || ctx->profiling || single_stream) {
     prove_enqueue_part<FrP>(ctx, pk, z, z_on_device, r, s, 3, nullptr, latency_plan);
     return;
@@ -1022,8 +1190,7 @@
   const bool prof = ctx->profiling;
   ZKP_REQUIRE(pk->shard_world == 0, ZKP_ERR_BAD_ARG);
   size_t pending[zkp_ctx::N_LANES] = {};
-  const int lanes_default = pk->log_n <= 22 ? 8 : 4;
-  const int nl = std::max(1, std::min(ctx->cfg.lanes > 0 ? ctx->cfg.lanes : lanes_default, (int)zkp_ctx::N_LANES));
+  const int nl = batch_lanes(ctx, pk);
   auto select = [&](int l) {
     ctx->cur = &ctx->lanes[l];
     ctx->cur_idx = l;
@@ -1033,25 +1200,15 @@
     ~BatchMode() { c->batch_mode = false; }
   } batch_mode{ctx};
   ctx->batch_mode = n > 1 && !prof;
+  const uint64_t allocs0 = devbuf_allocs.load(std::memory_order_relaxed);
+  struct CountAllocs {
+    zkp_groth16_pk* pk;
+    uint64_t from;
+    ~CountAllocs() { pk->last_batch_allocs = devbuf_allocs.load(std::memory_order_relaxed) - from; }
+  } count_allocs{pk, allocs0};
   try {
-    if (ctx->batch_mode) {
-      std::vector<uint64_t> scratch_proof(pw64 + 8);
-      uint8_t scratch_inf[4];
-      bool any = false;
-      for (int l = 0; l < nl; l++) {
-        if (pk->lane[l].warmed) continue;
-        select(l);
-        if (pk->curve == ZKP_BN254) prove_enqueue<Bn254Fr>(ctx, pk, z_dev[0], z_on_device, r, s);
-        else prove_enqueue<Bls381Fr>(ctx, pk, z_dev[0], z_on_device, r, s);
-        pk->lane[l].warmed = true;
-        any = true;
-      }
-      if (any)
-        for (int l = 0; l < nl; l++) {
-          select(l);
-          if (ctx->cur->busy) prove_finish(ctx, pk, scratch_proof.data(), scratch_inf);
-        }
-    }
+    if (!prof && n > 0 && groth16_reserve_lanes(ctx, pk, 0, (int)std::min<size_t>(n, (size_t)nl), ctx->batch_mode) > 0)
+      pk->reserved_where = 2;
     for (size_t i = 0; i < n; i++) {
       const int l = prof ? 0 : (int)(i % nl);
       select(l);
diff --git a/ckb_zkp_amd/csrc/internal.hpp b/ckb_zkp_amd/csrc/internal.hpp
--- a/ckb_zkp_amd/csrc/internal.hpp
+++ b/ckb_zkp_amd/csrc/internal.hpp
@@ -8,6 +8,7 @@
 bool ntt_ifft_coset_fft(zkp_ctx* ctx, int curve, uint32_t* data, int log_n);
 uint32_t* ntt_qap_coset_ifft(zkp_ctx* ctx, int curve, uint32_t* a, uint32_t* b, uint32_t* c, const uint32_t* zinv, int log_n);
 void ntt_free_tables(zkp_ctx* ctx);
+size_t ntt_scratch_bytes(int log_n, int count, bool fused);
 
 void fr_vec_op(zkp_ctx* ctx, int curve, int op, const uint64_t* a, const uint64_t* b, const uint64_t* k_host,
                uint64_t* out, size_t n);
@@ -45,6 +46,8 @@
 void bases_set_sort_flags(zkp_ctx* ctx, uint64_t handle, const uint8_t* flags_host, size_t n);
 void bases_set_group(zkp_ctx* ctx, uint64_t owner, const uint8_t* member_flags_host, size_t n);
 void bases_set_filter_bit(zkp_ctx* ctx, uint64_t handle, int bit);
+void msm_plan_scratch(zkp_ctx* ctx, uint64_t handle, size_t n, int ws, int sort_src, int l1_src, int acc_into, bool defer,
+                      bool instrumented, bool batch_mode, LaneScratchPlan* plan);
 void msm_run_batch(zkp_ctx* ctx, uint64_t handle, size_t count, const size_t* offsets, const uint64_t* const* scalars_dev,
                    const size_t* ns, bool montgomery, uint64_t* out_xyz_host);
 void msm_run_multi(zkp_ctx* ctx, size_t count, const uint64_t* handles, const size_t* offsets,
@@ -74,6 +77,8 @@
 void groth16_fold_assemble(zkp_ctx* ctx, int curve, const void* gathered_dev, int world, const uint64_t* r,
                            const uint64_t* s, uint64_t* proof_out, uint8_t* inf_out);
 void groth16_pk_free(zkp_ctx* ctx, zkp_groth16_pk* pk);
+int groth16_reserve_lanes(zkp_ctx* ctx, zkp_groth16_pk* pk, int first, int count, bool batch_mode);
+void groth16_batch_stats(zkp_ctx* ctx, zkp_groth16_pk* pk, uint64_t info[6]);
 uint64_t groth16_domain_size(zkp_groth16_pk* pk);
 void groth16_pk_info(zkp_ctx* ctx, zkp_groth16_pk* pk, uint64_t info[8]);
 void bases_info(zkp_ctx* ctx, uint64_t handle, uint64_t info[5]);
diff --git a/ckb_zkp_amd/csrc/msm.hip b/ckb_zkp_amd/csrc/msm.hip
--- a/ckb_zkp_amd/csrc/msm.hip
+++ b/ckb_zkp_amd/csrc/msm.hip
@@ -242,6 +242,7 @@
 
 
 constexpr int SCAN_CHUNK = 2048;
+static size_t scan_tmp_bytes(size_t n) { return n ? ((n + SCAN_CHUNK - 1) / SCAN_CHUNK + 1) * 4 : 0; }
 __global__ __launch_bounds__(256) void scan_reduce_kernel(const uint32_t* __restrict__ in, size_t n,
                                                           uint32_t* __restrict__ sums) {
   ZKP_SORT_PRIO();
@@ -313,7 +314,7 @@
 static void exclusive_scan_u32(hipStream_t st, const uint32_t* in, uint32_t* out, size_t n, DevBuf& tmp) {
   if (n == 0) return;
   size_t chunks = (n + SCAN_CHUNK - 1) / SCAN_CHUNK;
-  uint32_t* sums = tmp.as<uint32_t>(chunks + 1);
+  uint32_t* sums = reinterpret_cast<uint32_t*>(tmp.get(scan_tmp_bytes(n)));
   hipLaunchKernelGGL(scan_reduce_kernel, dim3(chunks), dim3(256), 0, st, in, n, sums);
   hipLaunchKernelGGL(scan_sums_kernel, dim3(1), dim3(1024), 0, st, sums, chunks);
   hipLaunchKernelGGL(scan_apply_kernel, dim3(chunks), dim3(256), 0, st, in, n, sums, out);
@@ -679,6 +680,130 @@
   }
 }
 
+struct MsmShape {
+  uint32_t nb = 0;
+  int kbits = 0, H1 = 0, LB = 0;
+  uint32_t nbins1 = 0, tile = 0, nblocks = 0, max_tasks = 0;
+  size_t E = 0, hist_n = 0;
+  uint32_t seg_chunk = 0, seg_blocks = 0, var_n1 = 0;
+  size_t out = 0, vals = 0, keys2 = 0, sort_tmp = 0, offsets = 0, sched = 0, buckets = 0, partial = 0, redo = 0, tmp = 0,
+         scan_tmp = 0, scan_tmp2 = 0;
+};
+static int sort_h1_env() {
+  static const int v = [] { const char* e = getenv("ZKP_SORT_H1"); return e ? atoi(e) : 0; }();
+  return v;
+}
+static MsmShape msm_shape(const BasesEntry* be, size_t n, bool batch_mode) {
+  MsmShape s;
+  const size_t XB = be->vt->bucket_bytes;
+  s.out = 64 * 4 * sizeof(uint32_t);
+  if (n == 0) return s;
+  const int c = be->c, W = be->W, lgk = be->lgk;
+  s.kbits = (c - 1) + lgk;
+  s.nb = 1u << s.kbits;
+  s.E = n * (size_t)W;
+  int H1 = 10;
+  while (H1 < SORT_H1_MAX && (s.E >> H1) > SORT_BIN_TARGET) H1++;
+  if (sort_h1_env() > 0) H1 = std::min(SORT_H1_MAX, sort_h1_env());
+  H1 = std::min(H1, s.kbits);
+  if (s.kbits - H1 > SORT_L_MAX) H1 = s.kbits - SORT_L_MAX;
+  s.H1 = H1;
+  s.LB = s.kbits - H1;
+  s.nbins1 = 1u << H1;
+  s.tile = SORT_SCALARS;
+  while ((n + s.tile - 1) / s.tile > 1536) s.tile += 256;
+  s.nblocks = (uint32_t)((n + s.tile - 1) / s.tile);
+  s.hist_n = (size_t)s.nbins1 * s.nblocks + 1;
+  s.max_tasks = s.nb + (uint32_t)(s.E / be->cap) + 1;
+  s.vals = (s.E + 8) * 4;
+  s.keys2 = s.E * 8;
+  s.sort_tmp = 2 * s.hist_n * 4;
+  s.offsets = 2 * (size_t)s.nb * 4;
+  s.sched = ((size_t)2 * (s.nb + 2) + (size_t)8 * s.max_tasks + TM_WORDS + 8) * 4;
+  s.buckets = (size_t)2 * s.nb * XB + XB;
+  s.partial = (size_t)s.max_tasks * XB;
+  s.redo = ((size_t)s.max_tasks + 1) * 4;
+  s.scan_tmp = scan_tmp_bytes(s.hist_n);
+  s.scan_tmp2 = scan_tmp_bytes((size_t)s.nb + 1);
+  if (be->var) {
+    const uint32_t nb_w = 1u << (c - 1);
+    for (int l = 0; l < c - 1; l++) {
+      const uint32_t pw = nb_w >> (l + 1);
+      s.var_n1 += (uint32_t)(1 << lgk) * (pw / std::min<uint32_t>((uint32_t)SEG_CHUNK, pw));
+    }
+    s.tmp = ((size_t)s.var_n1 + 256 + 8) * XB;
+  } else {
+    s.seg_chunk = batch_mode ? SEG_CHUNK_BATCH : SEG_CHUNK;
+    uint32_t cnt = s.nb;
+    for (int l = 0; l < c - 1; l++) {
+      s.seg_blocks += (cnt / 2 + s.seg_chunk - 1) / s.seg_chunk;
+      cnt /= 2;
+    }
+    s.tmp = ((size_t)s.seg_blocks + 64) * XB;
+  }
+  return s;
+}
+
+struct MsmChunks {
+  bool on = false;
+  size_t nch = 1, first = 0, per_rest = 0;
+};
+static MsmChunks msm_chunks(const zkp_cfg& cfg, const BasesEntry* be, size_t n, int sort_src, int l1_src, bool instrumented,
+                            bool chained, bool batch_mode) {
+  MsmChunks k;
+  const size_t chunk_pts = (size_t)std::max<long long>(0, cfg.msm_chunk);
+  k.on = chunk_pts >= 1024 && n >= 2 * chunk_pts && be->group == 1 && !be->var && sort_src < 0 && l1_src < 0 &&
+         !be->group_flags && !instrumented && !chained && !batch_mode;
+  if (!k.on) return k;
+  const size_t nch0 = (n + chunk_pts - 1) / chunk_pts, per = ((n + nch0 - 1) / nch0 + 255) & ~(size_t)255;
+  static const size_t first_div = [] { const char* e = getenv("ZKP_MSM_CHUNK_FIRST"); long v = e ? atol(e) : 2; return (size_t)(v < 1 ? 1 : v); }();
+  const size_t first = first_div > 1 ? std::max<size_t>(((per / first_div) + 255) & ~(size_t)255, 1024) : 0;
+  const size_t rest = first && first < n ? n - first : n;
+  const size_t nrest = (rest + per - 1) / per;
+  k.per_rest = ((rest + nrest - 1) / nrest + 255) & ~(size_t)255;
+  k.first = first && first < n ? first : 0;
+  k.nch = (k.first ? 1 : 0) + (rest + k.per_rest - 1) / k.per_rest;
+  return k;
+}
+
+static void msm_plan_entry(const BasesEntry* be, size_t n, int ws_idx, int sort_src, int l1_src, int bucket_ws, bool batch_mode,
+                           LaneScratchPlan* plan) {
+  using B = MsmWorkspace;
+  const MsmShape sh = msm_shape(be, n, batch_mode);
+  plan->want(ws_idx, B::OUT, sh.out);
+  if (n == 0) return;
+  const bool reuse = sort_src >= 0, l1_reuse = !reuse && l1_src >= 0;
+  const int sw = reuse ? sort_src : ws_idx, lw = l1_reuse ? l1_src : sw;
+  plan->want(sw, B::VALS, sh.vals);
+  plan->want(lw, B::KEYS2, sh.keys2);
+  plan->want(lw, B::SORT_TMP, sh.sort_tmp);
+  plan->want(sw, B::OFFSETS, sh.offsets);
+  plan->want(sw, B::SCHED, sh.sched);
+  if (!reuse && !l1_reuse) plan->want(ws_idx, B::SCAN_TMP, sh.scan_tmp);
+  if (!reuse) plan->want(ws_idx, B::SCAN_TMP2, sh.scan_tmp2);
+  plan->want(bucket_ws >= 0 ? bucket_ws : ws_idx, B::BUCKETS, sh.buckets);
+  plan->want(ws_idx, B::PARTIAL, sh.partial);
+  plan->want(ws_idx, B::REDO, sh.redo);
+  plan->want(ws_idx, B::TMP, sh.tmp);
+}
+
+void msm_plan_scratch(zkp_ctx* ctx, uint64_t handle, size_t n, int ws_idx, int sort_src, int l1_src, int acc_into, bool defer,
+                      bool instrumented, bool batch_mode, LaneScratchPlan* plan) {
+  auto be = get_bases(ctx, handle);
+  const MsmChunks ck = msm_chunks(ctx->cfg, be.get(), n, sort_src, l1_src, instrumented, defer || acc_into >= 0, batch_mode);
+  if (!ck.on) {
+    msm_plan_entry(be.get(), n, ws_idx, sort_src, l1_src, acc_into, batch_mode, plan);
+    return;
+  }
+  const int wa = ws_idx, wb = ws_idx ^ 2;
+  size_t done = 0;
+  for (size_t k = 0; k < ck.nch; k++) {
+    const size_t len = std::min((k == 0 && ck.first) ? ck.first : ck.per_rest, n - done);
+    msm_plan_entry(be.get(), len, ((ck.nch - 1 - k) & 1) ? wb : wa, -1, -1, wa, batch_mode, plan);
+    done += len;
+  }
+}
+
 static void msm_run_entry(zkp_ctx* ctx, const BasesEntry* be, size_t offset, const uint64_t* scalars_dev, size_t n,
                           bool montgomery, uint64_t* out_xyz_host, void* out_dev_xyzz, float* ms_accumulate,
                           uint64_t* n_entries, int ws_idx, int sort_src, float* ms_scan, int l1_src = -1);
@@ -693,28 +818,21 @@
     }
   } chain_reset{ctx};
   auto be = get_bases(ctx, handle);
-  const size_t chunk_pts = (size_t)std::max<long long>(0, ctx->cfg.msm_chunk);
-  const bool chunkable = chunk_pts >= 1024 && n >= 2 * chunk_pts && be->group == 1 && !be->var && sort_src < 0 && l1_src < 0 &&
-                         !be->group_flags && !ctx->profiling && !ms_accumulate && !ms_scan && !n_entries &&
-                         !ctx->msm_defer_reduce && ctx->msm_acc_into < 0 && ctx->msm_bucket_ws < 0 && !ctx->batch_mode;
-  if (!chunkable) {
+  const MsmChunks ck = msm_chunks(ctx->cfg, be.get(), n, sort_src, l1_src, ctx->profiling || ms_accumulate || ms_scan || n_entries,
+                                  ctx->msm_defer_reduce || ctx->msm_acc_into >= 0 || ctx->msm_bucket_ws >= 0, ctx->batch_mode);
+  if (!ck.on) {
     msm_run_entry(ctx, be.get(), offset, scalars_dev, n, montgomery, out_xyz_host, out_dev_xyzz, ms_accumulate, n_entries,
                   ws_idx, sort_src, ms_scan, l1_src);
     return;
   }
-  const size_t nch0 = (n + chunk_pts - 1) / chunk_pts, per = ((n + nch0 - 1) / nch0 + 255) & ~(size_t)255;
-  static const size_t first_div = [] { const char* e = getenv("ZKP_MSM_CHUNK_FIRST"); long v = e ? atol(e) : 2; return (size_t)(v < 1 ? 1 : v); }();
-  const size_t first = first_div > 1 ? std::max<size_t>(((per / first_div) + 255) & ~(size_t)255, 1024) : 0;
-  const size_t rest = first && first < n ? n - first : n;
-  const size_t nrest = (rest + per - 1) / per, per_rest = ((rest + nrest - 1) / nrest + 255) & ~(size_t)255;
-  const size_t nch = (first && first < n ? 1 : 0) + (rest + per_rest - 1) / per_rest;
+  const size_t first = ck.first, per_rest = ck.per_rest, nch = ck.nch;
   const int wa = ws_idx, wb = ws_idx ^ 2;
   hipStream_t sa = wa == 0 ? ctx->cur->stream : ctx->cur->ws[wa].stream, sb = wb == 0 ? ctx->cur->stream : ctx->cur->ws[wb].stream;
   ZKP_HIP(hipEventRecord(ctx->cur->ws[wa].l1_done, sa));
   ZKP_HIP(hipStreamWaitEvent(sb, ctx->cur->ws[wa].l1_done, 0));
   size_t done = 0;
   for (size_t k = 0; k < nch; k++) {
-    const size_t len = std::min((k == 0 && first && first < n) ? first : per_rest, n - done);
+    const size_t len = std::min((k == 0 && first) ? first : per_rest, n - done);
     const bool last = k + 1 == nch;
     const int w = ((nch - 1 - k) & 1) ? wb : wa;
     ctx->msm_defer_reduce = !last;
@@ -779,7 +897,8 @@
   hipStream_t st = ws_idx == 0 ? ctx->cur->stream : ws.stream;
   const size_t XB = vt->bucket_bytes;
   const size_t jac_words = 3 * (size_t)vt->fN;
-  uint32_t* out_jac = ws.out.as<uint32_t>(64 * 4);
+  const MsmShape sh = msm_shape(be, n, ctx->batch_mode);
+  uint32_t* out_jac = reinterpret_cast<uint32_t*>(ws.out.get(sh.out));
   if (ms_accumulate) *ms_accumulate = 0.f;
   if (ms_scan) *ms_scan = 0.f;
   if (n_entries) *n_entries = 0;
@@ -791,31 +910,24 @@
     const int lgk = be->lgk, K = 1 << lgk;
     ZKP_REQUIRE(var == (lgk > 0), ZKP_ERR_BAD_ARG);
     const uint32_t nb_w = 1u << (c - 1);
-    const int kbits = (c - 1) + lgk;
-    const uint32_t nb = 1u << kbits;
-    const size_t E = n * (size_t)W;
+    const int kbits = sh.kbits;
+    const uint32_t nb = sh.nb;
+    const size_t E = sh.E;
     ZKP_REQUIRE(E < 2147483000ull, ZKP_ERR_BAD_ARG);
     const bool l1_reuse = !reuse && l1_src >= 0;
     MsmWorkspace& lw = l1_reuse ? ctx->cur->ws[l1_src] : sw;
-    uint32_t* vals = sw.vals.as<uint32_t>(E + 8);
-    uint64_t* kv = lw.keys2.as<uint64_t>(E);
+    uint32_t* vals = reinterpret_cast<uint32_t*>(sw.vals.get(sh.vals));
+    uint64_t* kv = reinterpret_cast<uint64_t*>(lw.keys2.get(sh.keys2));
     const uint32_t* sc = reinterpret_cast<const uint32_t*>(scalars_dev);
     const int mont = montgomery ? 1 : 0;
-    static const int h1_env = [] { const char* e = getenv("ZKP_SORT_H1"); return e ? atoi(e) : 0; }();
-    int H1 = 10;
-    while (H1 < SORT_H1_MAX && (E >> H1) > SORT_BIN_TARGET) H1++;
-    if (h1_env > 0) H1 = std::min(SORT_H1_MAX, h1_env);
-    H1 = std::min(H1, kbits);
-    if (kbits - H1 > SORT_L_MAX) H1 = kbits - SORT_L_MAX;
-    const int LB = kbits - H1;
-    const uint32_t nbins1 = 1u << H1;
-    uint32_t tile = SORT_SCALARS;
-    while ((n + tile - 1) / tile > 1536) tile += 256;
-    const uint32_t nblocks = (uint32_t)((n + tile - 1) / tile);
-    const size_t hist_n = (size_t)nbins1 * nblocks + 1;
-    uint32_t* hist = lw.sort_tmp.as<uint32_t>(2 * hist_n);
+    const int LB = sh.LB;
+    const uint32_t nbins1 = sh.nbins1;
+    const uint32_t tile = sh.tile;
+    const uint32_t nblocks = sh.nblocks;
+    const size_t hist_n = sh.hist_n;
+    uint32_t* hist = reinterpret_cast<uint32_t*>(lw.sort_tmp.get(sh.sort_tmp));
     uint32_t* offs = hist + hist_n;
-    uint32_t* start = sw.offsets.as<uint32_t>(2 * (size_t)nb);
+    uint32_t* start = reinterpret_cast<uint32_t*>(sw.offsets.get(sh.offsets));
     uint32_t* end = start + nb;
     const uint8_t* scan_inf = be->sort_inf && !ctx->profiling ? be->sort_inf : be->inf;
     if (reuse) {
@@ -879,8 +991,8 @@
       hipLaunchKernelGGL(sort_bin_kernel, dim3(nbins1), dim3(SORT_BIN_THREADS), ((size_t)4 << LB) + 4 * (size_t)SORT_BIN_STAGE, st,
                          kv, offs, nblocks, LB, vals, start, end, (l1_reuse || grp) ? be->filter_bit : -1);
     uint32_t* const sorted_vals = vals;
-    const uint32_t max_tasks = nb + (uint32_t)(E / be->cap) + 1;
-    uint32_t* sched = sw.sched.as<uint32_t>((size_t)2 * (nb + 2) + (size_t)8 * max_tasks + TM_WORDS + 8);
+    const uint32_t max_tasks = sh.max_tasks;
+    uint32_t* sched = reinterpret_cast<uint32_t*>(sw.sched.get(sh.sched));
     uint32_t* tcount = sched;
     uint32_t* toff = tcount + (nb + 2);
     uint32_t* task_start = toff + (nb + 2);
@@ -903,8 +1015,8 @@
       ctx->mark(st, ":sorted");
     }
     MsmWorkspace& bws = bucket_ws >= 0 ? ctx->cur->ws[bucket_ws] : ws;
-    char* buckets = reinterpret_cast<char*>(bws.buckets.get((size_t)2 * nb * XB + XB));
-    char* task_partial = reinterpret_cast<char*>(ws.partial.get((size_t)max_tasks * XB));
+    char* buckets = reinterpret_cast<char*>(bws.buckets.get(sh.buckets));
+    char* task_partial = reinterpret_cast<char*>(ws.partial.get(sh.partial));
     static const bool zero_all = getenv("ZKP_MEMSET_BUCKETS") && atoi(getenv("ZKP_MEMSET_BUCKETS")) != 0;
     const uint32_t init = into >= 0 ? 1u : 0u;
     if (init) {
@@ -918,7 +1030,7 @@
     static const uint32_t force_redo = getenv("ZKP_DEBUG_FORCE_REDO") && atoi(getenv("ZKP_DEBUG_FORCE_REDO")) != 0 ? 2u : 0u;
     ctx->mark(st, ":acc0");
     vt->accumulate(st, be->table, sorted_vals, desc, toff + nb, max_tasks, buckets, task_partial,
-                   ws.redo.as<uint32_t>((size_t)max_tasks + 1), init | force_redo);
+                   reinterpret_cast<uint32_t*>(ws.redo.get(sh.redo)), init | force_redo);
     ctx->mark(st, ":acc1");
     if (timed) {
       ZKP_HIP(hipEventRecord(ctx->ev3, st));
@@ -927,7 +1039,7 @@
     }
     static const int dbg = [] { const char* e = getenv("ZKP_DEBUG_MSM"); return e ? atoi(e) : 0; }();
     if (dbg) {
-      uint32_t* rep = ws.redo.as<uint32_t>((size_t)max_tasks + 1);
+      uint32_t* rep = reinterpret_cast<uint32_t*>(ws.redo.get(sh.redo));
       ZKP_HIP(hipStreamSynchronize(st));
       ZKP_HIP(hipMemsetAsync(rep, 0, 32, st));
       hipLaunchKernelGGL(sched_check_kernel, dim3(256), dim3(256), 0, st, toff, long_list, tmeta, nb, max_tasks, rep);
@@ -965,7 +1077,8 @@
         cnt /= 2;
       }
       const char* roots = buckets + (size_t)lvl_off * XB;
-      char* partial = reinterpret_cast<char*>(ws.tmp.get(((size_t)vp.n1 + 256 + 8) * XB));
+      ZKP_REQUIRE(vp.n1 == sh.var_n1, ZKP_ERR_BAD_ARG);
+      char* partial = reinterpret_cast<char*>(ws.tmp.get(sh.tmp));
       char* R = partial + (size_t)vp.n1 * XB;
       vt->segsum_desc(st, buckets, vp.d1.as<SegDesc>(vp.n1), vp.n1, partial);
       vt->segsum_desc(st, partial, vp.d2.as<SegDesc>(256), 256, R);
@@ -992,7 +1105,7 @@
     const int L = c - 1;
     SegPlan plan{};
     plan.L = L;
-    const uint32_t chunk = ctx->batch_mode ? SEG_CHUNK_BATCH : SEG_CHUNK;
+    const uint32_t chunk = sh.seg_chunk;
     plan.chunk = chunk;
     uint32_t lvl_off = 0, cnt = nb, blocks = 0;
     static const bool fuse_seg = !(getenv("ZKP_PAIR_TOP_FUSE_SEG") && atoi(getenv("ZKP_PAIR_TOP_FUSE_SEG")) == 0);
@@ -1029,7 +1142,8 @@
     }
     plan.first_block[L] = blocks;
     const char* root = buckets + (size_t)lvl_off * XB;
-    char* partial = reinterpret_cast<char*>(ws.tmp.get(((size_t)blocks + 64) * XB));
+    ZKP_REQUIRE(blocks == sh.seg_blocks, ZKP_ERR_BAD_ARG);
+    char* partial = reinterpret_cast<char*>(ws.tmp.get(sh.tmp));
     char* Obuf = partial + (size_t)blocks * XB;
     if (L > 0 && l_top >= 0) {
       SegPlan low = plan;
diff --git a/ckb_zkp_amd/csrc/ntt.hip b/ckb_zkp_amd/csrc/ntt.hip
--- a/ckb_zkp_amd/csrc/ntt.hip
+++ b/ckb_zkp_amd/csrc/ntt.hip
@@ -552,6 +552,15 @@
   return blk;
 }
 
+size_t ntt_scratch_bytes(int log_n, int count, bool fused) {
+  const size_t N = (size_t)1 << log_n;
+  if (fused || log_n == 0) return N * 32;
+  int S[8], np;
+  ntt_plan(log_n, S, &np);
+  const bool odd = (np & 1) && np > 1;
+  return (size_t)count * N * 32 * (odd ? 2 : 1);
+}
+
 template <class P>
 void ntt_run_t(zkp_ctx* ctx, int curve, uint32_t* const* data, int count, int log_n, int op) {
   ZKP_REQUIRE(log_n <= P::TWO_ADICITY, ZKP_ERR_DOMAIN_TOO_LARGE);
@@ -562,7 +571,7 @@
   int S[8], np;
   ntt_plan(log_n, S, &np);
   const bool odd = (np & 1) && np > 1;
-  uint32_t* scratch = ctx->cur->ntt_scratch.as<uint32_t>((size_t)count * N * 8 * (odd ? 2 : 1));
+  uint32_t* scratch = reinterpret_cast<uint32_t*>(ctx->cur->ntt_scratch.get(ntt_scratch_bytes(log_n, count, false)));
   uint32_t* scratch2 = scratch + (size_t)count * N * 8;
   const bool inverse = (op == ZKP_NTT_IFFT || op == ZKP_NTT_COSET_IFFT);
   bool in_scratch = false;
@@ -644,7 +653,7 @@
   uint32_t* pre = full_table<P>(ctx, t, &t.full_g_n, t.g_lo, t.g_hi_n, 0, 0, 0);
   if (!pre) return false;
   const size_t N = (size_t)1 << log_n;
-  uint32_t* scratch = ctx->cur->ntt_scratch.as<uint32_t>(N * 8);
+  uint32_t* scratch = reinterpret_cast<uint32_t*>(ctx->cur->ntt_scratch.get(ntt_scratch_bytes(log_n, 1, true)));
   int S[8], np;
   ntt_plan(log_n, S, &np);
   uint32_t* buf[2] = {data, scratch};
@@ -671,7 +680,7 @@
   uint32_t* post = full_table<P>(ctx, t, &t.full_gi, t.gi_lo, t.gi_hi, 0, 0, 0);
   if (!post) return nullptr;
   const size_t N = (size_t)1 << log_n;
-  uint32_t* scratch = ctx->cur->ntt_scratch.as<uint32_t>(N * 8);
+  uint32_t* scratch = reinterpret_cast<uint32_t*>(ctx->cur->ntt_scratch.get(ntt_scratch_bytes(log_n, 1, true)));
   int S[8], np;
   ntt_plan(log_n, S, &np);
   if (np < 2) return nullptr;
diff --git a/ckb_zkp_amd/groth16.py b/ckb_zkp_amd/groth16.py
--- a/ckb_zkp_amd/groth16.py
+++ b/ckb_zkp_amd/groth16.py
@@ -350,6 +350,12 @@
                 "l_reuses_a_sort": bool(info[6] & 2), "shared_level1_pass": bool(info[6] & 4),
                 "h_evaluation_form": bool(info[7] & 1), "c_folded_into_l": bool(info[7] & 2), "l_h_bucket_chained": bool(info[7] & 4)}
 
+    def batch_stats(self) -> dict:
+        info = (C.c_uint64 * 6)()
+        _lib.check(self.ctx.lib.zkp_groth16_batch_stats(self.ctx.h, self.h, info), "zkp_groth16_batch_stats")
+        return {"proofs_enqueued": int(info[0]), "allocs_in_last_batch": int(info[1]), "lanes_reserved": int(info[2]),
+                "bytes_reserved": int(info[3]), "reserved_at": {0: None, 1: "upload", 2: "batch"}[int(info[4])]}
+
     def free(self):
         if self.h:
             _lib.check(self.ctx.lib.zkp_groth16_pk_free(self.ctx.h, self.h), "zkp_groth16_pk_free")
diff --git a/include/zkp_accel.h b/include/zkp_accel.h
--- a/include/zkp_accel.h
+++ b/include/zkp_accel.h
@@ -177,6 +177,7 @@
 int32_t zkp_groth16_witness_map_dev(zkp_ctx* ctx, zkp_groth16_pk* pk, const uint64_t* z_dev, uint64_t* h_dev);
 int32_t zkp_groth16_domain_size(zkp_groth16_pk* pk, uint64_t* n);
 int32_t zkp_groth16_pk_info(zkp_ctx* ctx, zkp_groth16_pk* pk, uint64_t info[8]);
+int32_t zkp_groth16_batch_stats(zkp_ctx* ctx, zkp_groth16_pk* pk, uint64_t info[6]);
 
 int32_t zkp_groth16_prove(zkp_ctx* ctx, zkp_groth16_pk* pk, const uint64_t* z_host, const uint64_t* r,
                           const uint64_t* s, uint64_t* proof_out, uint8_t* inf_out);
diff --git a/rust/zkp-accel/src/ffi.rs b/rust/zkp-accel/src/ffi.rs
--- a/rust/zkp-accel/src/ffi.rs
+++ b/rust/zkp-accel/src/ffi.rs
@@ -250,6 +250,7 @@
     pub fn zkp_groth16_witness_map_dev(ctx: *mut zkp_ctx, pk: *mut zkp_groth16_pk, z_dev: *const u64, h_dev: *mut u64) -> i32;
     pub fn zkp_groth16_domain_size(pk: *mut zkp_groth16_pk, n: *mut u64) -> i32;
     pub fn zkp_groth16_pk_info(ctx: *mut zkp_ctx, pk: *mut zkp_groth16_pk, info: *mut u64) -> i32;
+    pub fn zkp_groth16_batch_stats(ctx: *mut zkp_ctx, pk: *mut zkp_groth16_pk, info: *mut u64) -> i32;
     pub fn zkp_groth16_prove(ctx: *mut zkp_ctx, pk: *mut zkp_groth16_pk, z_host: *const u64, r: *const u64, s: *const u64, proof_out: *mut u64, inf_out: *mut u8) -> i32;
     pub fn zkp_groth16_prove_dev(ctx: *mut zkp_ctx, pk: *mut zkp_groth16_pk, z_dev: *const u64, r: *const u64, s: *const u64, proof_out: *mut u64, inf_out: *mut u8) -> i32;
     pub fn zkp_groth16_prove_batch_dev(ctx: *mut zkp_ctx, pk: *mut zkp_groth16_pk, n: usize, z_dev: *const *const u64, r: *const u64, s: *const u64, proofs_out: *mut u64, inf_out: *mut u8) -> i32;
```

Measured after the change: 140.3 proofs/s, median of 2. No clear change (+0.2%).
